# IntelLabs/bayesian-torch

Hardware: AMD Instinct MI355X
Metric: MC-samples/sec (Bayesian-ResNet18, 224^2, bs=64) (higher is better)
Workload: dtype bf16

## Files before the change

### bayesian_torch_amd/_lib.py

```python
import ctypes
import os

_HERE = os.path.dirname(os.path.abspath(__file__))
_LIB = None

KIND_REPARAM, KIND_FLIPOUT = 0, 1
ACT_F32, ACT_BF16 = 0, 1
PREC_F32, PREC_BF16, PREC_BF16X3 = 0, 1, 2
PREC_CODE = {"f32": 0, "bf16": 1, "bf16x3": 2}
FLAG_TRANSPOSED, FLAG_KL_ACCUM, FLAG_ROWFUSE, FLAG_OUT_F32, FLAG_OUT_BF16, FLAG_GATHER, FLAG_SWAP_SIGNS, FLAG_CONCURRENT = 1, 2, 4, 8, 16, 32, 64, 128
FLAG_REVERSE = 256
E_UNSUPPORTED = -3
STREAM_EPS_W, STREAM_EPS_B, STREAM_SIGN_IN, STREAM_SIGN_OUT = 0, 1, 2, 3
ABI_VERSION = 9
FLAG_LANES_SHIFT = 16
FLAG_LANES_MASK = 0xff << FLAG_LANES_SHIFT
SAMPLE_SKIP_MU = 1


class BtxError(RuntimeError):
    pass


class Geom(ctypes.Structure):
    _fields_ = [(n, ctypes.c_int32) for n in (
        "NB", "D", "H", "W", "C", "N", "KD", "KH", "KW", "sd", "sh", "sw", "pd", "ph", "pw",
        "dd", "dh", "dw", "od", "oh", "ow", "groups")]


class Rng(ctypes.Structure):
    _fields_ = [("seed", ctypes.c_uint64), ("sample_idx", ctypes.c_uint32), ("layer_id", ctypes.c_uint32),
                ("sample_idx_dev", ctypes.c_void_p)]


class BnFuse(ctypes.Structure):
    _fields_ = [("residual", ctypes.c_void_p), ("relu", ctypes.c_int32), ("mask", ctypes.c_void_p), ("dres", ctypes.c_void_p)]


class Epilogue(ctypes.Structure):
    _fields_ = [("scale", ctypes.c_void_p), ("shift", ctypes.c_void_p), ("residual", ctypes.c_void_p),
                ("relu", ctypes.c_int32), ("pool", ctypes.c_int32)]


class Lanes(ctypes.Structure):
    _fields_ = [("n", ctypes.c_int32), ("x_stride", ctypes.c_int64), ("out_stride", ctypes.c_int64),
                ("res_stride", ctypes.c_int64)]


class PlanInfo(ctypes.Structure):
    _fields_ = [(n, ctypes.c_int32) for n in ("family", "ksplits", "kper", "kgroups", "wide", "tall", "par_major", "pool_band",
                                              "nwg", "lanes")] + [("ws_bytes", ctypes.c_uint64)]


FAMILIES = ("gather", "regstage", "dma", "gemm8", "patch", "taps", "taps2", "stem", "stem_pool")


class Noise(ctypes.Structure):
    _fields_ = [("eps_w", ctypes.c_void_p), ("eps_b", ctypes.c_void_p),
                ("sign_in", ctypes.c_void_p), ("sign_out", ctypes.c_void_p), ("sampled_w", ctypes.c_void_p)]


class SampleItem(ctypes.Structure):
    _fields_ = [("geom", ctypes.POINTER(Geom)), ("mu_w", ctypes.c_void_p), ("rho_w", ctypes.c_void_p),
                ("out", ctypes.c_void_p), ("kind", ctypes.c_int32), ("layer_id", ctypes.c_uint32),
                ("src_KW", ctypes.c_int32), ("src_C", ctypes.c_int32)]


class LstmLayer(ctypes.Structure):
    _fields_ = [("mu_w", ctypes.c_void_p), ("rho_w", ctypes.c_void_p), ("mu_b", ctypes.c_void_p), ("rho_b", ctypes.c_void_p),
                ("layer_id", ctypes.c_uint32), ("sample_idx", ctypes.c_uint32), ("sample_idx_dev", ctypes.c_void_p)]


class LstmGrads(ctypes.Structure):
    _fields_ = [("dmu_w", ctypes.c_void_p), ("drho_w", ctypes.c_void_p), ("dmu_b", ctypes.c_void_p), ("drho_b", ctypes.c_void_p)]


class KlItem(ctypes.Structure):
    _fields_ = [("mu", ctypes.c_void_p), ("rho", ctypes.c_void_p), ("prior_mu_t", ctypes.c_void_p),
                ("prior_sigma_t", ctypes.c_void_p), ("dmu", ctypes.c_void_p), ("drho", ctypes.c_void_p),
                ("prior_mu", ctypes.c_float), ("prior_sigma", ctypes.c_float), ("n", ctypes.c_size_t)]


class Q8Chain(ctypes.Structure):
    _fields_ = [(n, ctypes.c_float) for n in ("s_sigma", "s_mu", "s_eps", "inv_s_eps", "s_d", "inv_s_d", "inv_s_w")] + \
               [("bias_div", ctypes.c_double)]


class Q8Add(ctypes.Structure):
    _fields_ = [(n, ctypes.c_float) for n in ("s_a", "pre_a", "s_b", "pre_b", "inv_s")] + \
               [("zero_point", ctypes.c_int32), ("relu", ctypes.c_int32)]


class Q8Delta(ctypes.Structure):
    _fields_ = [("inv_s_eps", ctypes.c_float), ("mult", ctypes.c_float), ("mean_bias", ctypes.c_int32), ("pert_bias", ctypes.c_int32),
                ("div_mean", ctypes.c_double), ("div_pert", ctypes.c_double)]


class Q8Flipout(ctypes.Structure):
    _fields_ = [(n, ctypes.c_int32) for n in ("z_x", "z_xp", "z_mean", "z_pert", "z_p2", "sin_pos", "sin_neg", "sout_pos", "sout_neg")] + \
               [(n, ctypes.c_float) for n in ("mult_xp", "mult_mean", "mult_pert", "mult_p2", "out_scale")]


Q8_BIAS_NONE, Q8_BIAS_MU, Q8_BIAS_SIGMA_EPS = 0, 1, 2

EXPORTS = ("btx_abi_version", "btx_strerror", "btx_kl_workspace_bytes", "btx_kl_gauss", "btx_kl_model_workspace_bytes",
           "btx_kl_gauss_model", "btx_kl_gauss_model_bwd", "btx_contract_wgrad",
           "btx_contract_workspace_bytes", "btx_contract_fwd", "btx_contract_fwd_ex", "btx_contract_fwd_lanes", "btx_contract_pool_shape", "btx_contract_plan_info", "btx_out_shape", "btx_fill_eps", "btx_fill_sign", "btx_rho_grad",
           "btx_mc_packed_floats", "btx_mc_accumulate", "btx_mc_accumulate_lanes", "btx_sampled_w_bytes", "btx_sample_weights", "btx_sampled_w_bytes_lanes", "btx_sample_weights_lanes", "btx_rowfuse_pack", "btx_maxpool2d_cl", "btx_avgpool_global_cl",
           "btx_bn_workspace_bytes", "btx_bn_train_fwd", "btx_bn_train_bwd", "btx_dgrad_weights",
           "btx_wgrad_workspace_bytes", "btx_contract_wgrad_ws", "btx_maxpool2d_cl_train", "btx_maxpool2d_cl_bwd",
           "btx_lstm_workspace_bytes", "btx_lstm_fwd", "btx_lstm_train_saved_bytes", "btx_lstm_train_workspace_bytes",
           "btx_lstm_fwd_train", "btx_lstm_bwd",
           "btx_calib_workspace_bytes", "btx_avu_fwd", "btx_avu_bwd", "btx_eau_fwd", "btx_eau_bwd",
           "btx_q8_weight_row_bytes", "btx_q8_quantize_act", "btx_q8_sample_weights", "btx_q8_contract",
           "btx_q8_add", "btx_q8_contract_res", "btx_q8_maxpool2d_cl", "btx_q8_avgpool2d_cl",
           "btx_q8_sample_delta", "btx_q8_contract_flipout")


def lib_path():
    return os.environ.get("BTX_LIB") or os.path.join(_HERE, "libbtx.so")


def lib():
    global _LIB
    if _LIB is not None:
        return _LIB
    path = lib_path()
    if not os.path.exists(path):
        raise BtxError("libbtx.so not found at %s — build it with `python __graft_entry__.py build` "
                       "(hipcc --offload-arch=gfx950); there is no fallback path." % path)
    L = ctypes.CDLL(path)
    vp, sz, u32, i32, f32 = ctypes.c_void_p, ctypes.c_size_t, ctypes.c_uint32, ctypes.c_int, ctypes.c_float
    L.btx_abi_version.restype = i32
    L.btx_abi_version.argtypes = []
    L.btx_strerror.restype = ctypes.c_char_p
    L.btx_strerror.argtypes = [i32]
    L.btx_kl_workspace_bytes.restype = sz
    L.btx_kl_workspace_bytes.argtypes = [sz]
    L.btx_kl_gauss.restype = i32
    L.btx_kl_gauss.argtypes = [vp, vp, sz, vp, vp, f32, f32, vp, u32, vp, sz, vp]
    L.btx_kl_model_workspace_bytes.restype = sz
    L.btx_kl_model_workspace_bytes.argtypes = [i32]
    L.btx_kl_gauss_model.restype = i32
    L.btx_kl_gauss_model.argtypes = [ctypes.POINTER(KlItem), i32, vp, vp, sz, vp]
    L.btx_kl_gauss_model_bwd.restype = i32
    L.btx_kl_gauss_model_bwd.argtypes = [ctypes.POINTER(KlItem), i32, vp, vp]
    L.btx_contract_wgrad.restype = i32
    L.btx_contract_wgrad.argtypes = [i32, ctypes.POINTER(Geom), vp, vp, vp, vp, vp, vp, ctypes.POINTER(Rng),
                                     ctypes.POINTER(Noise), i32, u32, vp]
    L.btx_contract_wgrad_ws.restype = i32
    L.btx_contract_wgrad_ws.argtypes = [i32, ctypes.POINTER(Geom), vp, vp, vp, vp, vp, vp, ctypes.POINTER(Rng),
                                        ctypes.POINTER(Noise), i32, u32, vp, sz, vp, vp, vp]
    L.btx_wgrad_workspace_bytes.restype = sz
    L.btx_wgrad_workspace_bytes.argtypes = [i32, ctypes.POINTER(Geom), i32, u32]
    L.btx_contract_workspace_bytes.restype = sz
    L.btx_contract_workspace_bytes.argtypes = [ctypes.POINTER(Geom), i32, i32, i32, u32]
    L.btx_contract_fwd.restype = i32
    L.btx_contract_fwd.argtypes = [i32, ctypes.POINTER(Geom), vp, vp, vp, vp, vp, vp, ctypes.POINTER(Rng),
                                   ctypes.POINTER(Noise), i32, i32, u32, vp, sz, vp]
    L.btx_contract_fwd_ex.restype = i32
    L.btx_contract_fwd_ex.argtypes = L.btx_contract_fwd.argtypes + [ctypes.POINTER(Epilogue)]
    L.btx_contract_fwd_lanes.restype = i32
    L.btx_contract_fwd_lanes.argtypes = L.btx_contract_fwd_ex.argtypes + [ctypes.POINTER(Lanes)]
    L.btx_contract_plan_info.restype = i32
    L.btx_contract_plan_info.argtypes = [i32, ctypes.POINTER(Geom), i32, i32, u32, ctypes.POINTER(Epilogue), ctypes.POINTER(PlanInfo)]
    L.btx_contract_pool_shape.restype = i32
    L.btx_contract_pool_shape.argtypes = [ctypes.POINTER(Geom), i32, i32, u32] + [ctypes.POINTER(ctypes.c_int32)] * 2
    L.btx_out_shape.restype = i32
    L.btx_out_shape.argtypes = [ctypes.POINTER(Geom), u32] + [ctypes.POINTER(ctypes.c_int32)] * 3
    L.btx_fill_eps.restype = i32
    L.btx_fill_eps.argtypes = [vp, sz, ctypes.POINTER(Rng), u32, vp]
    L.btx_rho_grad.restype = i32
    L.btx_rho_grad.argtypes = [vp, vp, vp, sz, ctypes.POINTER(Rng), u32, vp]
    L.btx_fill_sign.restype = i32
    L.btx_fill_sign.argtypes = [vp, sz, ctypes.POINTER(Rng), u32, vp]
    L.btx_mc_packed_floats.restype = sz
    L.btx_mc_packed_floats.argtypes = [i32, i32]
    L.btx_sampled_w_bytes.restype = sz
    L.btx_sampled_w_bytes.argtypes = [ctypes.POINTER(Geom), i32, i32]
    L.btx_sample_weights.restype = i32
    L.btx_sample_weights.argtypes = [ctypes.POINTER(SampleItem), i32, ctypes.POINTER(Rng), i32, vp]
    L.btx_sampled_w_bytes_lanes.restype = sz
    L.btx_sampled_w_bytes_lanes.argtypes = [ctypes.POINTER(Geom), i32, i32, i32]
    L.btx_sample_weights_lanes.restype = i32
    L.btx_sample_weights_lanes.argtypes = [ctypes.POINTER(SampleItem), i32, ctypes.POINTER(Rng), i32, vp, i32, u32]
    L.btx_rowfuse_pack.restype = i32
    L.btx_rowfuse_pack.argtypes = [vp, i32, ctypes.POINTER(ctypes.c_int64), i32, i32, i32, i32, vp, i32, i32, i32, i32, i32,
                                   i32, vp]
    L.btx_maxpool2d_cl.restype = i32
    L.btx_maxpool2d_cl.argtypes = [vp, vp, i32, i32, i32, i32, i32, i32, i32, i32, vp]
    L.btx_maxpool2d_cl_train.restype = i32
    L.btx_maxpool2d_cl_train.argtypes = [vp, vp, vp, i32, i32, i32, i32, i32, i32, i32, i32, vp]
    L.btx_maxpool2d_cl_bwd.restype = i32
    L.btx_maxpool2d_cl_bwd.argtypes = [vp, vp, vp, i32, i32, i32, i32, i32, i32, i32, i32, vp]
    L.btx_avgpool_global_cl.restype = i32
    L.btx_avgpool_global_cl.argtypes = [vp, vp, i32, i32, i32, i32, vp]
    L.btx_mc_accumulate.restype = i32
    L.btx_mc_accumulate.argtypes = [vp, i32, i32, i32, f32, vp, vp]
# ... 70 lines not shown
```

### bayesian_torch_amd/csrc/btx_api.hip

```cpp
#include <hip/hip_runtime.h>
#include <math.h>
#include <string.h>
#include "../../include/btx.h"
#include <stdlib.h>
#include "btx_contract.h"
#include "btx_rng.h"
#include "btx_presample.h"

using namespace btx;

static int contract_fwd_impl(int kind, const BtxGeom* g, const void* x, const float* mu_w, const float* rho_w,
                             const float* mu_b, const float* rho_b, void* out, const BtxRng* rng, const BtxNoise* noise,
                             int act_dtype, int prec, uint32_t flags, void* ws, size_t ws_bytes, void* stream,
                             const BtxEpilogue* ep, const BtxLanes* ln) {
  if (!g || !x || !mu_w || !rho_w || !out || !rng) return BTX_E_NULL;
  const int lanes = ln ? ln->n : 1;
  if ((mu_b == nullptr) != (rho_b == nullptr)) return BTX_E_NULL;
  const uintptr_t al = (uintptr_t)x | (uintptr_t)mu_w | (uintptr_t)rho_w | (uintptr_t)out |
                       (uintptr_t)(noise && noise->eps_w ? noise->eps_w : nullptr);
  FwdSel sel;
  int rc = select_fwd(kind, g, act_dtype, prec, flags, (al & 15) != 0, noise, ep, &sel);
  if (rc) return rc;
  const Plan& pl = sel.pl;
  const void* sampled_w = (noise && noise->sampled_w) ? noise->sampled_w : nullptr;
  if (sel.need && (!ws || ws_bytes < sel.need)) return BTX_E_WORKSPACE;
  if (sel.need && (((uintptr_t)ws) & 15)) return BTX_E_ALIGN;

  ContractParams p;
  memset(&p, 0, sizeof(p));
  p.x = x; p.mu = mu_w; p.rho = rho_w; p.mu_b = mu_b; p.rho_b = rho_b; p.out = out;
  p.partial = pl.ksplits > 1 ? (float*)ws : nullptr;
  p.lanes = lanes; p.lane_nwg = pl.nwg; p.fd_lane_nwg = make_fastdiv((uint32_t)(pl.nwg > 0 ? pl.nwg : 1));
  if (lanes > 1) {
    p.lane_x = ln->x_stride; p.lane_out = ln->out_stride; p.lane_res = ln->res_stride;
    p.lane_partial = (long long)(plan_ws(pl, g, 1));
  }
  if (noise) {
    p.eps_w = noise->eps_w; p.eps_b = noise->eps_b;
    p.sign_in = noise->sign_in; p.sign_out = noise->sign_out;
  }
  p.NB = g->NB; p.D = g->D; p.H = g->H; p.W = g->W; p.C = g->C; p.Cg = pl.Cg;
  p.Do = pl.Do; p.Ho = pl.Ho; p.Wo = pl.Wo; p.N = g->N; p.Ng = pl.Ng;
  p.KD = g->KD; p.KH = g->KH; p.KW = g->KW;
  p.sd = g->sd; p.sh = g->sh; p.sw = g->sw; p.pd = g->pd; p.ph = g->ph; p.pw = g->pw;
  p.dd = g->dd; p.dh = g->dh; p.dw = g->dw;
  p.M = pl.M; p.K = pl.K;
  p.mtiles = pl.mtiles; p.ntiles = pl.ntiles; p.groups = g->groups; p.ksplits = pl.ksplits; p.kper = pl.kper;
  p.transposed = (flags & BTX_FLAG_TRANSPOSED) ? 1 : 0;
  p.pointwise = (!p.transposed && g->KD == 1 && g->KH == 1 && g->KW == 1 && g->sd == 1 && g->sh == 1 && g->sw == 1 &&
                 g->pd == 0 && g->ph == 0 && g->pw == 0) ? 1 : 0;
  p.out_bf16 = sel.out_bf16;
  if (ep) { p.ep_scale = ep->scale; p.ep_shift = ep->shift; p.ep_res = ep->residual; p.ep_relu = ep->relu; }
  if (flags & BTX_FLAG_ROWFUSE) {
    p.Cg = g->KW * g->C;
    p.KW = 1;
    p.sign_unaligned = 1;
  }
  p.fd_Cg = make_fastdiv((uint32_t)p.Cg); p.fd_KW = make_fastdiv((uint32_t)p.KW); p.fd_KH = make_fastdiv((uint32_t)p.KH);
  p.seed_lo = (uint32_t)rng->seed; p.seed_hi = (uint32_t)(rng->seed >> 32);
  p.sample = rng->sample_idx; p.layer = rng->layer_id;
  p.sample_ptr = rng->sample_idx_dev;
  p.fd_sd = make_fastdiv((uint32_t)g->sd); p.fd_sh = make_fastdiv((uint32_t)g->sh); p.fd_sw = make_fastdiv((uint32_t)g->sw);
  if (sel.par_major) {
    p.par_major = 1; p.par_Hh = pl.Ho / 2; p.par_Wh = pl.Wo / 2; p.par_Mq = g->NB * p.par_Hh * p.par_Wh; p.par_Mqp = sel.par_mqp;
    p.fd_par_Mqp = make_fastdiv((uint32_t)p.par_Mqp); p.fd_par_Hh = make_fastdiv((uint32_t)p.par_Hh);
    p.fd_par_Wh = make_fastdiv((uint32_t)p.par_Wh);
  }
  p.swap_signs = (flags & BTX_FLAG_SWAP_SIGNS) ? 1 : 0;
  p.reverse = (flags & BTX_FLAG_REVERSE) ? 1 : 0;
  sign_keys(rng, p.swap_signs ? BTX_STREAM_SIGN_OUT : BTX_STREAM_SIGN_IN, &p.kin_a, &p.kin_b);
  sign_keys(rng, p.swap_signs ? BTX_STREAM_SIGN_IN : BTX_STREAM_SIGN_OUT, &p.kout_a, &p.kout_b);
  {
    const long long in_elems = (long long)g->NB * g->D * g->H * g->W * g->C;
    const long long xb = in_elems * (act_dtype == BTX_ACT_BF16 ? 2 : 4), wb = (long long)g->N * pl.K * 4;
    p.x_bytes = xb < 0xffffffffLL ? (uint32_t)xb : 0xffffffffu;
    p.w_bytes = wb < 0xffffffffLL ? (uint32_t)wb : 0xffffffffu;
  }

  p.fd_inner = make_fastdiv((uint32_t)(pl.ntiles * g->groups * pl.ksplits)); p.fd_ksplits = make_fastdiv((uint32_t)pl.ksplits);
  p.fd_ntiles = make_fastdiv((uint32_t)pl.ntiles); p.fd_rtiles = make_fastdiv(1u);
  p.fd_mtiles = make_fastdiv((uint32_t)(pl.mtiles > 0 ? pl.mtiles : 1));
  {
    const double w_b = (prec == BTX_PREC_BF16 ? 2.0 : 4.0) * (double)g->N * pl.K * (kind == BTX_KIND_FLIPOUT ? 2 : 1);
    p.wg_order = (uses_tiles(sel.family) && pl.mtiles > 1 && w_b >= WG_MAJOR_MIB * 1048576.0) ? 1 : 0;
  }
  p.fd_Wo = make_fastdiv((uint32_t)pl.Wo); p.fd_Ho = make_fastdiv((uint32_t)pl.Ho); p.fd_Do = make_fastdiv((uint32_t)pl.Do);
  if (uses_tiles(sel.family)) {
    p.wt = sampled_w ? (void*)sampled_w : (void*)((unsigned char*)ws + sel.wt_off);
    p.wt_ready = sampled_w ? 1 : 0;
    p.wt_bytes = (uint32_t)sel.wt_all;
    p.wt_delta_off = (uint32_t)sel.wt_one;
    p.lane_wt = (long long)sel.wt_one;
    p.lane_wt_delta = (kind == BTX_KIND_FLIPOUT) ? 1 : 0;
  }
  hipStream_t st = (hipStream_t)stream;
  typedef int (*LaunchFn)(int, const ContractParams&, int, hipStream_t);
  auto launch = [&](LaunchFn f32, LaunchFn bf16, LaunchFn x3) {
    return (prec == BTX_PREC_BF16 ? bf16 : prec == BTX_PREC_BF16X3 ? x3 : f32)(kind, p, pl.nwg * lanes, st);
  };
  switch (sel.family) {
    case BTX_FAMILY_STEM_POOL: {
      const StemPoolPlan& spp = sel.spp;
// ... 79 lines not shown
    case BTX_E_UNSUPPORTED: return "btx: unsupported configuration";
    case BTX_E_WORKSPACE: return "btx: workspace too small";
    case BTX_E_DTYPE: return "btx: unknown dtype / precision code";
    case BTX_E_ALIGN: return "btx: pointer not 16-byte aligned";
    default: return code > 0 ? hipGetErrorString((hipError_t)code) : "btx: unknown error";
  }
}

int btx_contract_fwd(int kind, const BtxGeom* g, const void* x, const float* mu_w, const float* rho_w,
                     const float* mu_b, const float* rho_b, void* out, const BtxRng* rng, const BtxNoise* noise,
                     int act_dtype, int prec, uint32_t flags, void* ws, size_t ws_bytes, void* stream) {
  return btx_contract_fwd_ex(kind, g, x, mu_w, rho_w, mu_b, rho_b, out, rng, noise, act_dtype, prec, flags, ws,
                             ws_bytes, stream, nullptr);
}

int btx_contract_fwd_ex(int kind, const BtxGeom* g, const void* x, const float* mu_w, const float* rho_w,
                        const float* mu_b, const float* rho_b, void* out, const BtxRng* rng, const BtxNoise* noise,
                        int act_dtype, int prec, uint32_t flags, void* ws, size_t ws_bytes, void* stream,
                        const BtxEpilogue* ep) {
  return contract_fwd_impl(kind, g, x, mu_w, rho_w, mu_b, rho_b, out, rng, noise, act_dtype, prec,
                           flags & ~BTX_FLAG_LANES_MASK, ws, ws_bytes, stream, ep, nullptr);
}

int btx_contract_fwd_lanes(int kind, const BtxGeom* g, const void* x, const float* mu_w, const float* rho_w,
                           const float* mu_b, const float* rho_b, void* out, const BtxRng* rng, const BtxNoise* noise,
                           int act_dtype, int prec, uint32_t flags, void* ws, size_t ws_bytes, void* stream,
                           const BtxEpilogue* ep, const BtxLanes* lanes) {
  if (!lanes) return BTX_E_NULL;
  if (lanes->n < 1 || lanes->n > 255) return BTX_E_SHAPE;
  if ((lanes->x_stride | lanes->out_stride | lanes->res_stride) & 15) return BTX_E_ALIGN;
  if (noise && lanes->n > 1 && (noise->eps_w || noise->eps_b || noise->sign_in || noise->sign_out)) return BTX_E_UNSUPPORTED;
  return contract_fwd_impl(kind, g, x, mu_w, rho_w, mu_b, rho_b, out, rng, noise, act_dtype, prec,
                           (flags & ~BTX_FLAG_LANES_MASK) | BTX_FLAG_LANES(lanes->n), ws, ws_bytes, stream, ep, lanes);
}

int btx_sample_weights(const BtxSampleItem* items, int n_items, const BtxRng* rng, int prec, void* stream) {
  return btx_sample_weights_lanes(items, n_items, rng, prec, stream, 1, 0);
}

int btx_sample_weights_lanes(const BtxSampleItem* items, int n_items, const BtxRng* rng, int prec, void* stream, int lanes,
                             uint32_t sflags) {
  if (!items || !rng) return BTX_E_NULL;
  if (lanes < 1 || lanes > 255) return BTX_E_SHAPE;
  const uint64_t seed = rng->seed;
  const uint32_t sample_idx = rng->sample_idx;
  if (n_items <= 0) return n_items == 0 ? 0 : BTX_E_SHAPE;
  if (prec != BTX_PREC_F32 && prec != BTX_PREC_BF16 && prec != BTX_PREC_BF16X3) return BTX_E_DTYPE;
  for (int base = 0; base < n_items; base += PRESAMPLE_MAX_ITEMS) {
    PresampleBatch b;
    memset(&b, 0, sizeof(b));
    b.n = n_items - base < PRESAMPLE_MAX_ITEMS ? n_items - base : PRESAMPLE_MAX_ITEMS;
    b.seed_lo = (uint32_t)seed; b.seed_hi = (uint32_t)(seed >> 32); b.sample = sample_idx; b.sample_ptr = rng->sample_idx_dev;
    b.lanes = lanes; b.skip_mu = (sflags & BTX_SAMPLE_SKIP_MU) ? 1 : 0;
    uint32_t blocks = 0;
    for (int i = 0; i < b.n; ++i) {
      const BtxSampleItem& s = items[base + i];
      if (!s.geom || !s.mu_w || !s.rho_w || !s.out) return BTX_E_NULL;
      if (s.kind != BTX_KIND_REPARAM && s.kind != BTX_KIND_FLIPOUT) return BTX_E_UNSUPPORTED;
      const bool remap = s.src_C != 0 || s.src_KW != 0;
      if ((((uintptr_t)s.out) & 15) || (!remap && (((uintptr_t)s.mu_w | (uintptr_t)s.rho_w) & 15))) return BTX_E_ALIGN;
      Plan pl;
      int rc = make_plan(s.geom, prec, 0, DBM, &pl);
      if (rc) return rc;
      if (pl.K % (prec == BTX_PREC_BF16 ? 8 : 4)) return BTX_E_UNSUPPORTED;
      size_t one = 0;
      if (patch_wt_bytes(pl, s.geom, s.kind, prec, &one, lanes) >= 0xfff00000ULL) return BTX_E_UNSUPPORTED;
// ... 29 lines not shown
```

### bayesian_torch_amd/csrc/btx_contract.h

```cpp
#pragma once
#include <hip/hip_runtime.h>
#include <stdint.h>
#include "btx_rng.h"
#include "btx_plan.h"

typedef __attribute__((ext_vector_type(8))) __bf16 bf16x8;
typedef __attribute__((ext_vector_type(4))) __bf16 bf16x4;
typedef __attribute__((ext_vector_type(4))) float f32x4;
typedef __attribute__((ext_vector_type(8))) float f32x8;
typedef __attribute__((ext_vector_type(16))) float f32x16;
typedef __attribute__((ext_vector_type(4))) uint32_t u32x4;
typedef __attribute__((ext_vector_type(2))) uint32_t u32x2;

namespace btx {

constexpr int NTHREADS = 512;
constexpr int ACTS_OFF = 0;
constexpr int SIGN_OFF = NG * BM * 16;
constexpr int WMU_OFF = SIGN_OFF + NG * BM * 4;
constexpr int WDL_OFF = WMU_OFF + NG * BN * 16;
constexpr int STAGE_BYTES = WDL_OFF + NG * BN * 16;
constexpr int LDS_BYTES = 2 * STAGE_BYTES;

struct FastDiv {
// ... 48 lines not shown
  const float* ep_scale;
  const float* ep_shift;
  const void* ep_res;
  int ep_relu;
  int out_bf16;
  int sign_unaligned;
  uint32_t x_bytes, w_bytes;
  int pt_G, pt_R, pt_Rp, pt_Wp, pt_PP, pt_NI, pt_rtiles;
  FastDiv fd_Wo, fd_Ho, fd_Do, fd_ptWp, fd_ptRp, fd_ptR;
  FastDiv fd_inner, fd_ksplits, fd_ntiles, fd_Cg, fd_KW, fd_KH, fd_rtiles;
  FastDiv fd_mtiles;
  int swap_signs;
  int par_major, par_Mq, par_Mqp, par_Hh, par_Wh;
  FastDiv fd_par_Mqp, fd_par_Hh, fd_par_Wh;
  FastDiv fd_sd, fd_sh, fd_sw;
  int wg_order;
  int pt_nw, pt_astage, pt_lds;
  int pt_kg;
  int pt_lds_g;
  int pt_taps;
  int pt_wide;
  int sp_Hq, sp_Wq;
  int st_sbytes;
  void* wt;
  uint32_t wt_bytes, wt_delta_off;
  int wt_ready;
  int pt_tall, pt_P, pt_Wt, pt_ncs;
  FastDiv fd_P, fd_Wt, fd_ncs;
  int lanes, lane_nwg;
  FastDiv fd_lane_nwg;
  long long lane_x, lane_out, lane_res, lane_wt, lane_partial;
  int lane_wt_delta;
  int reverse;
};

__device__ __forceinline__ uint32_t sample_word_scalar(const uint32_t* ptr) {
  return *(const __attribute__((address_space(4))) uint32_t*)(uintptr_t)ptr;
}

__device__ __forceinline__ int xcd_logical() {
  const int nwg = gridDim.x, L = blockIdx.x;
  const int q = nwg >> 3, r = nwg & 7, xcd = L & 7, slot = L >> 3;
  return (xcd < r ? xcd * (q + 1) : r * (q + 1) + (xcd - r) * q) + slot;
}

__device__ __forceinline__ ContractParams lane_view(const ContractParams& q, int& logical) {
  ContractParams p = q;
  if (q.reverse) logical = (int)gridDim.x - 1 - logical;
  if (q.lanes > 1) {
    uint32_t lane, loc;
    fdivmod((uint32_t)logical, q.fd_lane_nwg, (uint32_t)q.lane_nwg, lane, loc);
    logical = (int)loc;
    const long long l = (long long)lane;
    p.x = (const unsigned char*)q.x + l * q.lane_x;
    p.out = (unsigned char*)q.out + l * q.lane_out;
    if (q.ep_res) p.ep_res = (const unsigned char*)q.ep_res + l * q.lane_res;
    if (q.wt) {
      if (q.lane_wt_delta) p.wt_delta_off = q.wt_delta_off + (uint32_t)(l * q.lane_wt);
      else p.wt = (unsigned char*)q.wt + l * q.lane_wt;
    }
    if (q.partial) p.partial = (float*)((unsigned char*)q.partial + l * q.lane_partial);
    if (q.sample_ptr) p.sample_ptr = q.sample_ptr + lane;
    p.sample = q.sample + lane;
  }
  return p;
}
// ... 601 lines not shown
      for (int r = 0; r < nv; ++r)
        for (int s = 0; s < ksplits; ++s) a[r] += partial[(long long)s * total + i + r];
    }
    for (int r = 0; r < nv; ++r) {
      const int col = (int)((i + r) % N);
      float v = a[r];
      v = __builtin_fmaf(v, scale ? scale[col] : 1.f, shift ? shift[col] : 0.f);
      if (res) v += (float)res[i + r];
      if (relu) v = v > 0.f ? v : 0.f;
      if (relu == 2) v = v < 6.f ? v : 6.f;
      a[r] = v;
    }
    if (nv == 4) {
      if constexpr (sizeof(ACT) == 4) *(f32x4*)(out + i) = (f32x4){a[0], a[1], a[2], a[3]};
      else *(bf16x4*)(out + i) = __builtin_convertvector((f32x4){a[0], a[1], a[2], a[3]}, bf16x4);
    } else {
      for (int r = 0; r < nv; ++r) out[i + r] = (ACT)a[r];
    }
  }
}

int launch_contract_f32(int kind, int act_bf16, bool gen, const ContractParams& p, int nwg, hipStream_t st);
int launch_contract_bf16(int kind, int act_bf16, bool gen, const ContractParams& p, int nwg, hipStream_t st);
int launch_contract_dma_f32(int kind, const ContractParams& p, int nwg, hipStream_t st);
int launch_contract_dma_bf16(int kind, const ContractParams& p, int nwg, hipStream_t st);
int launch_contract_patch_f32(int kind, const ContractParams& p, int nwg, hipStream_t st);
int launch_contract_stem_f32(int kind, const ContractParams& p, int nwg, hipStream_t st);
int launch_contract_stem_bf16(int kind, const ContractParams& p, int nwg, hipStream_t st);
int launch_stem_pool_bf16(int kind, const ContractParams& p, int nwg, hipStream_t st);
struct PresampleBatch;
int launch_presample_batch_f32(const PresampleBatch& b, hipStream_t st);
int launch_presample_batch_bf16(const PresampleBatch& b, hipStream_t st);
int launch_contract_patch_bf16(int kind, const ContractParams& p, int nwg, hipStream_t st);
int launch_contract_patch_x3(int kind, const ContractParams& p, int nwg, hipStream_t st);
int launch_contract_stem_x3(int kind, const ContractParams& p, int nwg, hipStream_t st);
int launch_contract_dma_x3(int kind, const ContractParams& p, int nwg, hipStream_t st);
int launch_contract_gemm8_bf16(int kind, const ContractParams& p, int nwg, hipStream_t st);
int launch_contract_gemm8_f32(int kind, const ContractParams& p, int nwg, hipStream_t st);
int launch_contract_gemm8_x3(int kind, const ContractParams& p, int nwg, hipStream_t st);
int launch_presample_batch_x3(const PresampleBatch& b, hipStream_t st);

template <int PREC>
static int launch_contract_impl(int kind, int act_bf16, bool gen, const ContractParams& p, int nwg, hipStream_t st) {
#define BTX_LAUNCH(ACT, KIND, GENF)                                                                              \
  do {                                                                                                            \
    auto kfn = contract_kernel<PREC, ACT, KIND, GENF>;                                                            \
    static bool attr_done = false;                                                                                \
    if (!attr_done) {                                                                                             \
      hipError_t e = hipFuncSetAttribute((const void*)kfn, hipFuncAttributeMaxDynamicSharedMemorySize, LDS_BYTES); \
      if (e != hipSuccess) return (int)e;                                                                         \
      attr_done = true;                                                                                           \
    }                                                                                                             \
    hipLaunchKernelGGL(kfn, dim3(nwg), dim3(NTHREADS), LDS_BYTES, st, p);                                         \
  } while (0)
  if (!act_bf16) {
    if (kind == 0) { if (gen) BTX_LAUNCH(float, 0, true); else BTX_LAUNCH(float, 0, false); }
    else           { if (gen) BTX_LAUNCH(float, 1, true); else BTX_LAUNCH(float, 1, false); }
  } else {
    if (kind == 0) { if (gen) BTX_LAUNCH(__bf16, 0, true); else BTX_LAUNCH(__bf16, 0, false); }
    else           { if (gen) BTX_LAUNCH(__bf16, 1, true); else BTX_LAUNCH(__bf16, 1, false); }
  }
#undef BTX_LAUNCH
  return (int)hipGetLastError();
}

}
// ... 1 lines not shown
```

### bayesian_torch_amd/csrc/btx_contract_patch.h

```cpp
#pragma once
#include <type_traits>
#include "btx_contract.h"
#include "btx_contract_dma.h"
#include "btx_epilogue.h"
#include "btx_presample.h"
#include "btx_mma.h"
#include "btx_contract_taps.h"
#include "btx_contract_taps2.h"

namespace btx {



template <int PREC, int KIND, int NW, int MI>
__global__ __launch_bounds__(64 * NW, (MI == 4) ? 1 : 2) void contract_patch_kernel(const ContractParams) {
  BTX_SECTION_PARAMS(p, logical);
  const RngLive rl = rng_live<KIND>(p);
  constexpr int NT = 64 * NW;
  constexpr int WPX = 32 * MI;
  constexpr int MAXNI = (MI == 4) ? 16 : PT_MAXNI;
  constexpr int SJ = (MI == 4) ? 4 : 2;
  using ACT = typename std::conditional<PREC == 1, __bf16, float>::type;
  constexpr int G = (PREC == 1) ? 8 : 4;
  constexpr int BK = NG * G;
// ... 196 lines not shown
    BTX_SECTION_PARAMS(pe, logical2);
    const int nimg = min(pe.pt_G, pe.NB - img0), nrow = min(pe.pt_R, pe.Ho - row0);
    const int nvalid = nimg * nrow * pe.Wo;
    const uint32_t m0 = (uint32_t)(img0 * pe.Ho + row0) * (uint32_t)pe.Wo;
    if constexpr (MI == 2) {
      staged_epilogue<KIND, NW>(pe, rl, accm, accd, smem, tid, wave, lane, ntile, group, split, m0, nvalid);
    } else {
#pragma unroll
      for (int hf = 0; hf < MI / 2; ++hf) {
        __builtin_amdgcn_sched_barrier(0);
        staged_epilogue<KIND, NW>(pe, rl, reinterpret_cast<const f32x16(&)[2][2]>(accm[2 * hf]),
                                  reinterpret_cast<const f32x16(&)[2][2]>(accd[2 * hf]), smem, tid, wave, lane, ntile,
                                  group, split, m0, nvalid, wave * (MI / 2) + hf, hf == 0);
      }
    }
  }
}

template <int PREC>
static int launch_contract_patch_impl(int kind, const ContractParams& p, int nwg, hipStream_t st) {
#define BTX_LAUNCH_PT(KIND, NW, MI)                                                                                 \
  do {                                                                                                            \
    auto kfn = contract_patch_kernel<PREC, KIND, NW, MI>;                                                           \
    static bool attr_done = false;                                                                                \
    if (!attr_done) {                                                                                             \
      hipError_t e = hipFuncSetAttribute((const void*)kfn, hipFuncAttributeMaxDynamicSharedMemorySize, 163840);   \
      if (e != hipSuccess) return (int)e;                                                                         \
      attr_done = true;                                                                                           \
    }                                                                                                             \
    hipLaunchKernelGGL(kfn, dim3(nwg), dim3(64 * NW), p.pt_lds, st, p);                                           \
  } while (0)
  int rc = launch_presample_impl<PREC>(kind, p, st);
  if (rc) return rc;
  if (p.pt_taps == 332) {
#define BTX_LAUNCH_T2(KIND, ...)                                                                                  \
  do {                                                                                                            \
    auto kfn = contract_taps2_kernel<PREC, KIND, ##__VA_ARGS__>;                                                  \
    static bool attr_done = false;                                                                                \
    if (!attr_done) {                                                                                             \
      hipError_t e = hipFuncSetAttribute((const void*)kfn, hipFuncAttributeMaxDynamicSharedMemorySize, 163840);   \
      if (e != hipSuccess) return (int)e;                                                                         \
      attr_done = true;                                                                                           \
    }                                                                                                             \
    hipLaunchKernelGGL(kfn, dim3(nwg), dim3(256), p.pt_lds, st, p);                                               \
  } while (0)
    if constexpr (PREC == 1) {
      if (p.pt_wide && kind == 0) {
        BTX_LAUNCH_T2(0, true);
        return (int)hipGetLastError();
      }
    }
    if (kind == 0) BTX_LAUNCH_T2(0); else BTX_LAUNCH_T2(1);
#undef BTX_LAUNCH_T2
    return (int)hipGetLastError();
  }
  if (p.pt_taps == 33) {
#define BTX_LAUNCH_TP(KIND, KG, ...)                                                                               \
  do {                                                                                                            \
    auto kfn = contract_taps_kernel<PREC, KIND, 3, 3, KG, ##__VA_ARGS__>;                                           \
    static bool attr_done = false;                                                                                \
    if (!attr_done) {                                                                                             \
      hipError_t e = hipFuncSetAttribute((const void*)kfn, hipFuncAttributeMaxDynamicSharedMemorySize, 163840);   \
      if (e != hipSuccess) return (int)e;                                                                         \
      attr_done = true;                                                                                           \
    }                                                                                                             \
    hipLaunchKernelGGL(kfn, dim3(nwg), dim3(256 * KG), p.pt_lds, st, p);                                          \
// ... 22 lines not shown
```

### bayesian_torch_amd/csrc/btx_contract_taps.h

```cpp
#pragma once
#include <type_traits>
#include "btx_contract.h"
#include "btx_contract_dma.h"
#include "btx_epilogue.h"
#include "btx_mma.h"

namespace btx {

__device__ __forceinline__ void dma16s(__amdgpu_buffer_rsrc_t rsrc, uint32_t voff, uint32_t soff,
                                       unsigned char* lds_wave_base) {
  __builtin_amdgcn_raw_ptr_buffer_load_lds(rsrc, (__attribute__((address_space(3))) void*)lds_wave_base, 16, voff, soff,
                                           0, 0);
}

template <int N>
__device__ __forceinline__ void end_stage() {
  asm volatile("s_waitcnt vmcnt(%0)\n\ts_waitcnt lgkmcnt(0)\n\ts_barrier" ::"n"(N) : "memory");
}

template <int I, int N, class F>
__device__ __forceinline__ void static_for(F&& f) {
  if constexpr (I < N) {
    f(std::integral_constant<int, I>{});
    static_for<I + 1, N>(f);
  }
}

constexpr int TP_MAXNI = 6;

template <int T>
constexpr int tp_pieces(int t) {
  constexpr int PST = T - 3;
  constexpr int PPS = (TP_MAXNI + PST - 1) / PST;
  if (t < 0) t += T;
  if (t >= PST) return 0;
  int n = 0;
  for (int i = 0; i < PPS; ++i)
    if (t + PST * i < TP_MAXNI) ++n;
  return n;
}

template <int PREC, int KIND, int KH, int KW, int KG, bool WIDE = false>
__global__ __launch_bounds__(256 * KG, 2) void contract_taps_kernel(const ContractParams) {
  static_assert(!WIDE || (PREC == 1 && KG == 1 && KIND == 0), "wide tile: bf16 Reparameterization, one K-group");
  constexpr int K2 = (KIND == 1 || WIDE) ? 1 : 0;
  BTX_SECTION_PARAMS(p, logical);
  constexpr int NW = 4, NT = 256, MI = 2, T = KH * KW;
  static_assert(T >= 5 && T <= 32, "tap-unrolled kernel: 5..32 taps");
  constexpr int MAXNI = TP_MAXNI;
  constexpr int PST = T - 3;
  constexpr int WOPS = K2 ? 2 : 1;
  using ACT = typename std::conditional<PREC == 1, __bf16, float>::type;
  constexpr int G = (PREC == 1) ? 8 : 4;
  constexpr int BK = NG * G;
  constexpr int ESZ = (int)sizeof(ACT);
  extern __shared__ __attribute__((aligned(16))) unsigned char smem_all[];

  uint32_t smp = p.sample;
  if (p.sample_ptr) smp = sample_word_scalar(p.sample_ptr);

  const int tid = threadIdx.x & 255;
  const int lane = tid & 63;
  const int l31 = lane & 31;
  const int h = lane >> 5;
  const int wave_all = __builtin_amdgcn_readfirstlane((int)(threadIdx.x >> 6));
  const int wave = wave_all & 3;
  const int kg = (KG == 1) ? 0 : (wave_all >> 2);
  unsigned char* const smem = smem_all + kg * p.pt_lds_g;

  uint32_t u_mtile, u_rem, u_split, u_ntile, u_group, u_t;
  const uint32_t ntg = (uint32_t)(WIDE ? p.ntiles >> 1 : p.ntiles);
  if (p.wg_order) fdivmod((uint32_t)logical, p.fd_mtiles, (uint32_t)p.mtiles, u_rem, u_mtile);
  else fdivmod((uint32_t)logical, p.fd_inner, ntg * (uint32_t)(p.groups * p.ksplits), u_mtile, u_rem);
  fdivmod(u_rem, p.fd_ksplits, (uint32_t)p.ksplits, u_t, u_split);
  fdivmod(u_t, p.fd_ntiles, ntg, u_group, u_ntile);
  const int mtile = (int)u_mtile, split = (int)u_split, ntile = (int)u_ntile, group = (int)u_group;

  const bool tall = p.pt_tall != 0;
  uint32_t u_ig, u_rt;
  if (tall) fdivmod((uint32_t)mtile, p.fd_ncs, (uint32_t)p.pt_ncs, u_rt, u_ig);
  else fdivmod((uint32_t)mtile, p.fd_rtiles, (uint32_t)p.pt_rtiles, u_ig, u_rt);
  const int img0 = tall ? 0 : (int)u_ig * p.pt_G, row0 = (int)u_rt * p.pt_R, col0 = tall ? (int)u_ig * p.pt_Wt : 0;
  auto patch_src = [&](int q, bool& ok) __attribute__((always_inline)) -> uint32_t {
    uint32_t ut, upc, ugi, upr;
    fdivmod((uint32_t)q, p.fd_ptWp, (uint32_t)p.pt_Wp, ut, upc);
    int img, ih, iw;
    if (tall) {
      fdivmod((uint32_t)row0 + ut, p.fd_P, (uint32_t)p.pt_P, ugi, upr);
      img = (int)ugi; ih = (int)upr - p.ph; iw = col0 + (int)upc - p.pw;
      ok = (int)ut < p.pt_Rp;
    } else {
      fdivmod(ut, p.fd_ptRp, (uint32_t)p.pt_Rp, ugi, upr);
      img = img0 + (int)ugi; ih = row0 + (int)upr - p.ph; iw = (int)upc - p.pw;
      ok = true;
    }
    ok = ok && img < p.NB && (unsigned)ih < (unsigned)p.H && (unsigned)iw < (unsigned)p.W;
    return (uint32_t)((img * p.H + ih) * p.W + iw);
  };
  const int ncb_total = p.Cg / BK;
  const int cb_per = p.kper / BK;
  const int cb0 = split * cb_per + kg * (cb_per / KG);
  const int ncb = (KG == 1) ? min(ncb_total, cb0 + cb_per) - cb0 : cb_per / KG;
  const int a_stage = p.pt_astage, s_stage = p.pt_astage >> 4;
  const int PT_A_OFF = 0, PT_S_OFF = 2 * a_stage, PT_W_OFF = 2 * a_stage + 2 * s_stage;
  const int PT_X_OFF = PT_W_OFF + PT_WD * DW_STAGE;

  const __amdgpu_buffer_rsrc_t x_rsrc = __builtin_amdgcn_make_buffer_rsrc((void*)p.x, 0, p.x_bytes, 0x00020000);
  const __amdgpu_buffer_rsrc_t wt_rsrc = __builtin_amdgcn_make_buffer_rsrc((void*)p.wt, 0, p.wt_bytes, 0x00020000);

  const uint32_t w_voff = (uint32_t)lane * 16u + (uint32_t)wave * 1024u;
  const uint32_t w_sbase = (uint32_t)(group * p.ntiles + (WIDE ? 2 * ntile : ntile)) * (uint32_t)(p.K / G) * 1024u;
  const uint32_t w_second = WIDE ? (uint32_t)(p.K / G) * 1024u : p.wt_delta_off;
  const uint32_t CgG = (uint32_t)(p.Cg / G);
  const int w_lds = PT_W_OFF + wave * 1024;
  int wslot = 0;
  auto issue_w = [&](uint32_t tap, uint32_t cb, int slot) __attribute__((always_inline)) {
    const uint32_t soff = w_sbase + (tap * CgG + cb * (uint32_t)NG) * 1024u;
    unsigned char* ld = smem + w_lds + slot * DW_STAGE;
    dma16s(wt_rsrc, w_voff, soff, ld);
    if constexpr (K2) dma16s(wt_rsrc, w_voff, soff + w_second, ld + 4096);
  };
  if (ncb > 0) issue_w(0u, (uint32_t)cb0, 0);

  uint32_t sg_off[2];
  bool sg_ok[2];
  uint32_t* const pix_tab = (uint32_t*)(smem + PT_S_OFF + s_stage);
#pragma unroll
  for (int j = 0; j < 2; ++j) {
    const int q = tid + NT * j;
    sg_ok[j] = q < p.pt_PP;
    bool inside;
    const uint32_t ipix = patch_src(sg_ok[j] ? q : 0, inside);
    sg_off[j] = ipix * (uint32_t)p.C + (uint32_t)(group * p.Cg);
    if (q * 4 < s_stage) pix_tab[q] = (sg_ok[j] && inside) ? sg_off[j] : 0xffffffffu;
    if (p.sign_in)
      sg_ok[j] = sg_ok[j] && inside;
  }
  asm volatile("s_waitcnt lgkmcnt(0)\n\ts_barrier" ::: "memory");

  const int g_lane = (lane & 3) ^ ((lane >> 4) & 3);
  uint32_t pp_boff[MAXNI];
  uint32_t pmask = 0;
  uint32_t pp_e[MAXNI];
#pragma unroll
  for (int j = 0; j < MAXNI; ++j) {
    const int q = 16 * (wave + NW * j) + (lane >> 2);
    pp_e[j] = pix_tab[q < p.pt_PP ? q : 0];
  }
#pragma unroll
  for (int j = 0; j < MAXNI; ++j) {
    const int q = 16 * (wave + NW * j) + (lane >> 2);
    uint32_t bo = DMA_OOB;
    if (j < p.pt_NI && q < p.pt_PP) {
      const uint32_t e = pp_e[j];
      if (e != 0xffffffffu) bo = (e + (uint32_t)(G * g_lane)) * (uint32_t)ESZ;
    }
    pp_boff[j] = bo;
    if (j < p.pt_NI && 16 * (wave + NW * j) < p.pt_PP) {
      pmask |= 1u << j;
      if (ncb > 0)
        dma16(x_rsrc, bo == DMA_OOB ? DMA_OOB : bo + (uint32_t)(cb0 * BK * ESZ), smem + PT_A_OFF + (wave + NW * j) * 1024);
    }
  }
  pmask = __builtin_amdgcn_readfirstlane(pmask);
  if (ncb > 0) {
    issue_w(1u, (uint32_t)cb0, 1);
    issue_w(2u, (uint32_t)cb0, 2);
  }

  RngLive rl = {smp, p.kin_a, p.kin_b, p.kout_a, p.kout_b};
  if (p.sample_ptr || p.lanes > 1) {
    rl.sample = __builtin_amdgcn_readfirstlane(smp);
    if constexpr (KIND == 1) {
      const uint32_t si = p.swap_signs ? 3u : 2u, so = p.swap_signs ? 2u : 3u;
      const BtxPhilox4 ki = btx_philox4x32_10(0u, rl.sample, p.layer, si, p.seed_lo, p.seed_hi);
      const BtxPhilox4 ko = btx_philox4x32_10(0u, rl.sample, p.layer, so, p.seed_lo, p.seed_hi);
      rl.kin_a = __builtin_amdgcn_readfirstlane(ki.x[0]); rl.kin_b = __builtin_amdgcn_readfirstlane(ki.x[1]);
      rl.kout_a = __builtin_amdgcn_readfirstlane(ko.x[0]); rl.kout_b = __builtin_amdgcn_readfirstlane(ko.x[1]);
    }
  }

  auto write_signs = [&](int slot, int cb) __attribute__((always_inline)) {
    if constexpr (KIND == 1) {
      unsigned char* ss = smem + PT_S_OFF + slot * s_stage;
#pragma unroll
      for (int j = 0; j < 2; ++j) {
        if (sg_ok[j]) {
          const uint32_t off = sg_off[j] + (uint32_t)(cb * BK);
          uint32_t w;
          if (p.sign_in) w = sign_word_explicit(p.sign_in, off, p.x_bytes / (uint32_t)ESZ);
          else w = btx_sign_word(off >> 5, rl.kin_a, rl.kin_b);
          if constexpr (G == 4) w <<= 8 * ((off >> 4) & 1);
          *(uint32_t*)(ss + (tid + NT * j) * 4) = w;
        }
      }
    }
  };

  int q0[MI];
#pragma unroll
  for (int mi = 0; mi < MI; ++mi) {
    const int pl = wave * 64 + mi * 32 + l31;
    uint32_t ut, uc, ugi, ur;
    if (tall) {
      fdivmod((uint32_t)pl, p.fd_Wt, (uint32_t)p.pt_Wt, ur, uc);
      q0[mi] = ((int)ur < p.pt_R) ? (int)ur * p.pt_Wp + (int)uc : 0;
    } else {
      fdivmod((uint32_t)pl, p.fd_Wo, (uint32_t)p.Wo, ut, uc);
      fdivmod(ut, p.fd_ptR, (uint32_t)p.pt_R, ugi, ur);
      const int c = (int)uc, r = (int)ur, gi = (int)ugi;
      const bool ok = (gi < p.pt_G) && (img0 + gi < p.NB) && (row0 + r < p.Ho);
      q0[mi] = ok ? (gi * p.pt_Rp + r) * p.pt_Wp + c : 0;
    }
  }
  const int row_step = p.dh * p.pt_Wp;

  constexpr bool ZI = (PREC == 1 && KG == 1);
  f32x16 accm[MI][2], accd[MI][2];
  auto clear_acc = [&](int a0) __attribute__((always_inline)) {
#pragma unroll
    for (int a = 0; a < MI; ++a)
#pragma unroll
      for (int b = 0; b < 2; ++b)
#pragma unroll
        for (int r = 0; r < 16; ++r)
          if (a >= a0) { accm[a][b][r] = 0.f; accd[a][b][r] = 0.f; }
  };
  if (!ZI || ncb <= 0) clear_acc(0);

  using Frag = StageFragT<MI>;
  auto load_frag = [&](Frag& f, int aslot, int toffv, int wsl, auto mia_tag) __attribute__((always_inline)) {
    constexpr int MIA = decltype(mia_tag)::value;
    const unsigned char* as = smem + PT_A_OFF + aslot * a_stage;
    const unsigned char* ss = smem + PT_S_OFF + aslot * s_stage;
    const unsigned char* ws = smem + PT_W_OFF + wsl * DW_STAGE;
    int q[MI];
#pragma unroll
    for (int mi = 0; mi < MI; ++mi) q[mi] = q0[mi] + toffv;
#pragma unroll
    for (int kk = 0; kk < NG / 2; ++kk) {
      const int row = 2 * kk + h;
#pragma unroll
      for (int mi = 0; mi < MIA; ++mi) f.a[kk][mi] = *(const u32x4*)(as + q[mi] * 64 + ((row ^ ((q[mi] >> 2) & 3)) * 16));
#pragma unroll
      for (int ni = 0; ni < 2; ++ni) f.wm[kk][ni] = *(const u32x4*)(ws + (row * BN + ni * 32 + l31) * 16);
    }
    if constexpr (KIND == 1) {
#pragma unroll
      for (int mi = 0; mi < MIA; ++mi) f.sw[mi] = *(const uint32_t*)(ss + q[mi] * 4);
    }
  };

  if (ncb > 0) {
    write_signs(0, cb0);
    asm volatile("s_waitcnt vmcnt(%0)\n\ts_waitcnt lgkmcnt(0)\n\ts_barrier" ::"n"(KG == 1 ? WOPS : 2 * WOPS) : "memory");
    Frag fa, fb;
    const int nvalid_px = tall ? p.pt_R * p.pt_Wt : min(p.pt_G, p.NB - img0) * min(p.pt_R, p.Ho - row0) * p.Wo;
    const bool mi1_dead = wave * 64 + 32 >= nvalid_px;
    auto kloop = [&](auto mia_tag) __attribute__((always_inline)) {
    constexpr int MIA = decltype(mia_tag)::value;
    if constexpr (KG == 1) load_frag(fa, 0, 0, 0, mia_tag);
    auto block = [&](auto par_tag, auto first_tag, int cbi, bool last) __attribute__((always_inline)) {
      constexpr int PAR = decltype(par_tag)::value;
      constexpr bool FIRST = decltype(first_tag)::value;
      static_for<0, T>([&](auto t_tag) __attribute__((always_inline)) {
        constexpr int t = decltype(t_tag)::value;
        constexpr int sp = (PAR * T + t) & 1;
        Frag& cur = (KG == 1 && sp) ? fb : fa;
        Frag& nxt = (KG == 1 && sp) ? fa : fb;
        asm volatile("" : "+v"(q0[0]), "+v"(q0[1]));
        constexpr int t3 = (t + 3) % T, c3 = (t + 3) / T;
        if constexpr (c3 == 0) {
          issue_w((uint32_t)t3, (uint32_t)(cb0 + cbi), (wslot + 3) & 3);
        } else {
          if (!last) issue_w((uint32_t)t3, (uint32_t)(cb0 + cbi + 1), (wslot + 3) & 3);
        }
        constexpr int KP = tp_pieces<T>(t);
        if constexpr (t < PST) {
          if (!last) {
            const uint32_t cboff = (uint32_t)((cb0 + cbi + 1) * BK * ESZ);
#pragma unroll
            for (int i = 0; i < KP; ++i) {
              const int j = t + PST * i;
              const uint32_t bo = pp_boff[j];
              unsigned char* dst = ((pmask >> j) & 1u) ? smem + PT_A_OFF + (PAR ^ 1) * a_stage + (wave + NW * j) * 1024
                                                        : smem + PT_X_OFF;
              dma16(x_rsrc, bo == DMA_OOB ? DMA_OOB : bo + cboff, dst);
            }
            if constexpr (t == 0) write_signs(PAR ^ 1, cb0 + cbi + 1);
          }
        }
        DeltaFrag df;
        if constexpr (KG == 1) {
          load_delta<K2>(df, smem + PT_W_OFF + wslot * DW_STAGE, l31, h);
          constexpr int t1 = (t + 1) % T, c1 = (t + 1) / T;
          load_frag(nxt, PAR ^ c1, (t1 / KW) * row_step + (t1 % KW) * p.dw, (wslot + 1) & 3, mia_tag);
          if constexpr (FIRST && t == 0) stage_mma<PREC, K2, MI, MIA, true, KIND == 1>(cur, df, accm, accd, l31, h);
          else stage_mma<PREC, K2, MI, MIA, false, KIND == 1>(cur, df, accm, accd, l31, h);
          if (!last) end_stage<WOPS + KP>();
          else end_stage<(c3 == 0) ? WOPS : 0>();
        } else {
          load_delta<KIND>(df, smem + PT_W_OFF + wslot * DW_STAGE, l31, h);
          load_frag(cur, PAR, (t / KW) * row_step + (t % KW) * p.dw, wslot, mia_tag);
          __builtin_amdgcn_sched_barrier(0);
          asm volatile("s_barrier" ::: "memory");
          __builtin_amdgcn_sched_barrier(0);
          stage_mma<PREC, KIND, MI, MIA>(cur, df, accm, accd, l31, h);
          __builtin_amdgcn_sched_barrier(0);
          if (!last) {
            end_stage<2 * WOPS + KP + tp_pieces<T>(t - 1) + tp_pieces<T>(t - 2)>();
          } else {
            constexpr int a_ = (t + 3 < T) ? 1 : 0, b_ = (t == 0) ? 1 : ((t + 2 < T) ? 1 : 0);
            end_stage<WOPS * (a_ + b_)>();
          }
        }
        wslot = (wslot + 1) & 3;
      });
    };
    if (KG == 2 && kg == 1) asm volatile("s_barrier" ::: "memory");
    using P0 = std::integral_constant<int, 0>;
    using P1 = std::integral_constant<int, 1>;
    if constexpr (ZI) {
      if constexpr (MIA < MI) clear_acc(MIA);
      block(P0{}, std::true_type{}, 0, ncb == 1);
      int cbi = 1;
      for (; cbi + 2 <= ncb; cbi += 2) {
        block(P1{}, std::false_type{}, cbi, false);
        block(P0{}, std::false_type{}, cbi + 1, cbi + 2 == ncb);
      }
      if (cbi < ncb) block(P1{}, std::false_type{}, cbi, true);
    } else {
      int cbi = 0;
      for (; cbi + 2 <= ncb; cbi += 2) {
        block(P0{}, std::false_type{}, cbi, false);
        block(P1{}, std::false_type{}, cbi + 1, cbi + 2 == ncb);
      }
      if (cbi < ncb) block(P0{}, std::false_type{}, cbi, true);
    }
    if (KG == 2 && kg == 0) asm volatile("s_barrier" ::: "memory");
    };
    if (mi1_dead) kloop(std::integral_constant<int, 1>{});
    else kloop(std::integral_constant<int, 2>{});
  }

  {
    BTX_SECTION_PARAMS(pe, logical2);
    const int nimg = min(pe.pt_G, pe.NB - img0), nrow = min(pe.pt_R, pe.Ho - row0);
    const int nvalid = nimg * nrow * pe.Wo;
    const uint32_t m0 = (uint32_t)(img0 * pe.Ho + row0) * (uint32_t)pe.Wo;
    const PixTall pmt = {pe, row0, col0};
    if constexpr (KG == 1) {
      if constexpr (WIDE) {
        float* const ba0 = (float*)(smem + NW * PT_EP_WAVE);
        float* const ba1 = ba0 + 4 * BN;
        {
          const bool has_bias = (split == 0) && (pe.mu_b != nullptr);
          const bool has_aff = (pe.ksplits == 1) && ((pe.ep_scale != nullptr) || (pe.ep_shift != nullptr));
          if (has_bias || has_aff) {
            if (tid < 64) ep_fill_constants<0>(pe, rl, ba0, tid, 2 * ntile, group, has_bias, has_aff);
            else if (tid < 128) ep_fill_constants<0>(pe, rl, ba1, tid - 64, 2 * ntile + 1, group, has_bias, has_aff);
          }
          __syncthreads();
        }
        if (tall) {
          staged_epilogue_pm<0, NW, PixTall>(pe, rl, accm, accm, smem, tid, wave, lane, 2 * ntile, group, split, pmt, -1, true, ba0);
          staged_epilogue_pm<0, NW, PixTall>(pe, rl, accd, accd, smem, tid, wave, lane, 2 * ntile + 1, group, split, pmt, -1, true, ba1);
        } else {
          staged_epilogue<0, NW>(pe, rl, accm, accm, smem, tid, wave, lane, 2 * ntile, group, split, m0, nvalid, -1, true, ba0);
          staged_epilogue<0, NW>(pe, rl, accd, accd, smem, tid, wave, lane, 2 * ntile + 1, group, split, m0, nvalid, -1, true, ba1);
        }
      } else
      if (tall) staged_epilogue_pm<KIND, NW, PixTall>(pe, rl, accm, accd, smem, tid, wave, lane, ntile, group, split, pmt);
      else staged_epilogue<KIND, NW>(pe, rl, accm, accd, smem, tid, wave, lane, ntile, group, split, m0, nvalid);
    } else {
      float* ba_lds = (float*)(smem_all + 131072);
      const bool to_partial = pe.ksplits > 1;
      const bool has_bias = (split == 0) && (pe.mu_b != nullptr);
      const bool has_aff = !to_partial && ((pe.ep_scale != nullptr) || (pe.ep_shift != nullptr));
      if (kg == 1) {
#pragma unroll
        for (int mi = 0; mi < MI; ++mi)
#pragma unroll
          for (int ni = 0; ni < 2; ++ni)
// ... 44 lines not shown
```

### bayesian_torch_amd/csrc/btx_contract_taps2.h

```cpp
#pragma once
#include <type_traits>
#include "btx_contract.h"
#include "btx_contract_dma.h"
#include "btx_contract_taps.h"
#include "btx_epilogue.h"
#include "btx_mma.h"

namespace btx {

constexpr int T2_MAXNI = 5;
constexpr int T2_WD = 3;
constexpr int T2_T = 9;

constexpr int t2_seq(int s) { return s < 4 ? 0 : (s == 4 ? 1 : (s < 7 ? 2 : 3)); }
constexpr int t2_tap(int s) {
  return s == 0 ? 0 : s == 1 ? 2 : s == 2 ? 6 : s == 3 ? 8 : s == 4 ? 4 : s == 5 ? 1 : s == 6 ? 7 : s == 7 ? 3 : 5;
}
constexpr int t2_a(int k) { return (k == 0 || k == 2) ? 1 : 0; }
constexpr int t2_b(int k) { return (k == 0 || k == 3) ? 1 : 0; }
constexpr int t2_np(int s) { return (s == 0 || s == 5 || s == 7) ? 3 : ((s == 1 || s == 6 || s == 8) ? 2 : (s == 4 ? 5 : 0)); }
constexpr int t2_p0(int s) { return (s == 1 || s == 6 || s == 8) ? 3 : 0; }
constexpr int t2_fseq(int s) { return s < 2 ? 2 : (s == 4 ? 3 : (s < 7 ? 4 : 5)); }

template <int PREC, int KIND, bool WIDE = false>
__global__ __launch_bounds__(256, 2) void contract_taps2_kernel(const ContractParams) {
  static_assert(!WIDE || (PREC == 1 && KIND == 0), "wide tile: bf16 Reparameterization");
  BTX_SECTION_PARAMS(p, logical);
  constexpr int NW = 4, NT = 256, MI = 2, T = T2_T, MAXNI = T2_MAXNI, WD = T2_WD;
  constexpr int K2 = (KIND == 1 || WIDE) ? 1 : 0;
  constexpr int WOPS = K2 ? 2 : 1;
  using ACT = typename std::conditional<PREC == 1, __bf16, float>::type;
  constexpr int G = (PREC == 1) ? 8 : 4;
  constexpr int BK = NG * G;
  constexpr int ESZ = (int)sizeof(ACT);
  extern __shared__ __attribute__((aligned(16))) unsigned char smem[];

  uint32_t smp = p.sample;
  if (p.sample_ptr) smp = sample_word_scalar(p.sample_ptr);

  const int tid = threadIdx.x;
  const int lane = tid & 63;
  const int l31 = lane & 31;
  const int h = lane >> 5;
  const int wave = __builtin_amdgcn_readfirstlane(tid >> 6);

  uint32_t u_mtile, u_rem, u_split, u_ntile, u_group, u_t;
  const uint32_t ntg = (uint32_t)(WIDE ? p.ntiles >> 1 : p.ntiles);
  if (p.wg_order) fdivmod((uint32_t)logical, p.fd_mtiles, (uint32_t)p.mtiles, u_rem, u_mtile);
  else fdivmod((uint32_t)logical, p.fd_inner, ntg * (uint32_t)(p.groups * p.ksplits), u_mtile, u_rem);
  fdivmod(u_rem, p.fd_ksplits, (uint32_t)p.ksplits, u_t, u_split);
  fdivmod(u_t, p.fd_ntiles, ntg, u_group, u_ntile);
  const int mtile = (int)u_mtile, split = (int)u_split, ntile = (int)u_ntile, group = (int)u_group;

  uint32_t u_ig, u_rt;
  fdivmod((uint32_t)mtile, p.fd_rtiles, (uint32_t)p.pt_rtiles, u_ig, u_rt);
  const int img0 = (int)u_ig * p.pt_G, row0 = (int)u_rt * p.pt_R;
  const int ncb_total = p.Cg / BK;
  const int cb_per = p.kper / BK;
  const int cb0 = split * cb_per;
  const int ncb = min(ncb_total, cb0 + cb_per) - cb0;
  const int a_stage = p.pt_astage, s_stage = p.pt_astage >> 4;
  const int PT_A_OFF = 0, PT_S_OFF = 3 * a_stage, PT_W_OFF = 3 * a_stage + 3 * s_stage;
  const int PT_X_OFF = PT_W_OFF + WD * DW_STAGE;

  const __amdgpu_buffer_rsrc_t x_rsrc = __builtin_amdgcn_make_buffer_rsrc((void*)p.x, 0, p.x_bytes, 0x00020000);
  const __amdgpu_buffer_rsrc_t wt_rsrc = __builtin_amdgcn_make_buffer_rsrc((void*)p.wt, 0, p.wt_bytes, 0x00020000);

  const uint32_t w_voff = (uint32_t)lane * 16u + (uint32_t)wave * 1024u;
  const uint32_t w_sbase = (uint32_t)(group * p.ntiles + (WIDE ? 2 * ntile : ntile)) * (uint32_t)(p.K / G) * 1024u;
  const uint32_t w_second = WIDE ? (uint32_t)(p.K / G) * 1024u : p.wt_delta_off;
  const uint32_t CgG = (uint32_t)(p.Cg / G);
  const int w_lds = PT_W_OFF + wave * 1024;
  int wslot = 0;
  auto issue_w = [&](uint32_t tap, uint32_t cb, int slot) __attribute__((always_inline)) {
    const uint32_t soff = w_sbase + (tap * CgG + cb * (uint32_t)NG) * 1024u;
    unsigned char* ld = smem + w_lds + slot * DW_STAGE;
    dma16s(wt_rsrc, w_voff, soff, ld);
    if constexpr (K2) dma16s(wt_rsrc, w_voff, soff + w_second, ld + 4096);
  };
  if (ncb > 0) issue_w((uint32_t)t2_tap(0), (uint32_t)cb0, 0);

  const int g_lane = (lane & 3) ^ ((lane >> 4) & 3);
  uint32_t pp_base[MAXNI];
  uint32_t pvalid = 0, pmask = 0;
#pragma unroll
  for (int j = 0; j < MAXNI; ++j) {
    const int q = 16 * (wave + NW * j) + (lane >> 2);
    uint32_t bo = 0;
    if (j < p.pt_NI && q < p.pt_PP) {
      uint32_t ut, ujj, ugi, ui;
      fdivmod((uint32_t)q, p.fd_ptWp, (uint32_t)p.pt_Wp, ut, ujj);
      fdivmod(ut, p.fd_ptRp, (uint32_t)p.pt_Rp, ugi, ui);
      const int img = img0 + (int)ugi, ih0 = 2 * (row0 + (int)ui), iw0 = 2 * (int)ujj;
      bo = ((uint32_t)((img * p.H + ih0) * p.W + iw0) * (uint32_t)p.C + (uint32_t)(group * p.Cg + G * g_lane)) * (uint32_t)ESZ;
// ... 24 lines not shown
  };

  RngLive rl = {smp, p.kin_a, p.kin_b, p.kout_a, p.kout_b};
  if (p.sample_ptr || p.lanes > 1) {
    rl.sample = __builtin_amdgcn_readfirstlane(smp);
    if constexpr (KIND == 1) {
      const uint32_t si = p.swap_signs ? 3u : 2u, so = p.swap_signs ? 2u : 3u;
      const BtxPhilox4 ki = btx_philox4x32_10(0u, rl.sample, p.layer, si, p.seed_lo, p.seed_hi);
      const BtxPhilox4 ko = btx_philox4x32_10(0u, rl.sample, p.layer, so, p.seed_lo, p.seed_hi);
      rl.kin_a = __builtin_amdgcn_readfirstlane(ki.x[0]); rl.kin_b = __builtin_amdgcn_readfirstlane(ki.x[1]);
      rl.kout_a = __builtin_amdgcn_readfirstlane(ko.x[0]); rl.kout_b = __builtin_amdgcn_readfirstlane(ko.x[1]);
    }
  }
  uint32_t sg_base[2];
  uint32_t sg_v = 0;
#pragma unroll
  for (int j = 0; j < 2; ++j) {
    const int q = tid + NT * j;
    const int qq = q < p.pt_PP ? q : 0;
    uint32_t ut, ujj, ugi, ui;
    fdivmod((uint32_t)qq, p.fd_ptWp, (uint32_t)p.pt_Wp, ut, ujj);
    fdivmod(ut, p.fd_ptRp, (uint32_t)p.pt_Rp, ugi, ui);
    const int img = img0 + (int)ugi, ih0 = 2 * (row0 + (int)ui), iw0 = 2 * (int)ujj;
    sg_base[j] = (uint32_t)((img * p.H + ih0) * p.W + iw0) * (uint32_t)p.C + (uint32_t)(group * p.Cg);
    if (q < p.pt_PP && img < p.NB) {
#pragma unroll
      for (int a = 0; a < 2; ++a)
#pragma unroll
        for (int b = 0; b < 2; ++b)
          if ((unsigned)(ih0 - a) < (unsigned)p.H && (unsigned)(iw0 - b) < (unsigned)p.W) sg_v |= 1u << (4 * j + 2 * a + b);
    }
  }
  auto write_signs = [&](int a, int b, int cb, int sslot_off) __attribute__((always_inline)) {
    if constexpr (KIND == 1) {
      unsigned char* ss = smem + PT_S_OFF + sslot_off;
#pragma unroll
      for (int j = 0; j < 2; ++j) {
        if ((sg_v >> (4 * j + 2 * a + b)) & 1u) {
          const uint32_t off = sg_base[j] - (uint32_t)((a * p.W + b) * p.C) + (uint32_t)(cb * BK);
          uint32_t w;
          if (p.sign_in) w = sign_word_explicit(p.sign_in, off, p.x_bytes / (uint32_t)ESZ);
          else w = btx_sign_word(off >> 5, rl.kin_a, rl.kin_b);
          if constexpr (G == 4) w <<= 8 * ((off >> 4) & 1);
          *(uint32_t*)(ss + (tid + NT * j) * 4) = w;
        }
      }
    }
  };

  int q0[MI];
#pragma unroll
  for (int mi = 0; mi < MI; ++mi) {
    const int pl = wave * 64 + mi * 32 + l31;
    uint32_t ut, uc, ugi, ur;
    fdivmod((uint32_t)pl, p.fd_Wo, (uint32_t)p.Wo, ut, uc);
    fdivmod(ut, p.fd_ptR, (uint32_t)p.pt_R, ugi, ur);
    const int c = (int)uc, r = (int)ur, gi = (int)ugi;
    const bool ok = (gi < p.pt_G) && (img0 + gi < p.NB) && (row0 + r < p.Ho);
    q0[mi] = ok ? (gi * p.pt_Rp + r) * p.pt_Wp + c : 0;
  }
  const int Wp = p.pt_Wp;

  f32x16 accm[MI][2], accd[MI][2];
#pragma unroll
  for (int a = 0; a < MI; ++a)
#pragma unroll
    for (int b = 0; b < 2; ++b)
#pragma unroll
      for (int r = 0; r < 16; ++r) { accm[a][b][r] = 0.f; accd[a][b][r] = 0.f; }

  using Frag = StageFragT<MI>;
  auto load_frag = [&](Frag& f, int aoff, int soff, int toffv, int wsl, auto mia_tag) __attribute__((always_inline)) {
    constexpr int MIA = decltype(mia_tag)::value;
    const unsigned char* as = smem + PT_A_OFF + aoff;
    const unsigned char* ss = smem + PT_S_OFF + soff;
    const unsigned char* ws = smem + PT_W_OFF + wsl * DW_STAGE;
    int q[MI];
#pragma unroll
    for (int mi = 0; mi < MI; ++mi) q[mi] = q0[mi] + toffv;
#pragma unroll
    for (int kk = 0; kk < NG / 2; ++kk) {
      const int row = 2 * kk + h;
#pragma unroll
      for (int mi = 0; mi < MIA; ++mi) f.a[kk][mi] = *(const u32x4*)(as + q[mi] * 64 + ((row ^ ((q[mi] >> 2) & 3)) * 16));
#pragma unroll
      for (int ni = 0; ni < 2; ++ni) f.wm[kk][ni] = *(const u32x4*)(ws + (row * BN + ni * 32 + l31) * 16);
    }
    if constexpr (KIND == 1) {
#pragma unroll
      for (int mi = 0; mi < MIA; ++mi) f.sw[mi] = *(const uint32_t*)(ss + q[mi] * 4);
    }
  };

  if (ncb > 0) {
    int sl0 = 0, sl1 = 1, sl2 = 2;
    issue_plane(0, MAXNI, 1, 1, cb0, sl0 * a_stage);
    issue_w((uint32_t)t2_tap(1), (uint32_t)cb0, 1);
    issue_plane(0, MAXNI, 0, 0, cb0, sl1 * a_stage);
    write_signs(1, 1, cb0, sl0 * s_stage);
    write_signs(0, 0, cb0, sl1 * s_stage);
    asm volatile("s_waitcnt vmcnt(%0)\n\ts_waitcnt lgkmcnt(0)\n\ts_barrier" ::"n"(MAXNI + WOPS) : "memory");
    Frag fa;
    const int nvalid_px = min(p.pt_G, p.NB - img0) * min(p.pt_R, p.Ho - row0) * p.Wo;
    const bool mi1_dead = wave * 64 + 32 >= nvalid_px;
    auto kloop = [&](auto mia_tag) __attribute__((always_inline)) {
      constexpr int MIA = decltype(mia_tag)::value;
      auto block = [&](int cbi, bool last) __attribute__((always_inline)) {
        static_for<0, T>([&](auto t_tag) __attribute__((always_inline)) {
          constexpr int s = decltype(t_tag)::value;
          asm volatile("" : "+v"(q0[0]), "+v"(q0[1]), "+v"(pvalid), "+v"(sg_v), "+v"(sg_base[0]), "+v"(sg_base[1]));
          asm volatile("" : "+v"(pp_base[0]), "+v"(pp_base[1]), "+v"(pp_base[2]), "+v"(pp_base[3]), "+v"(pp_base[4]));
          auto slot_of = [&](int k) __attribute__((always_inline)) { return (k % 3) == 0 ? sl0 : ((k % 3) == 1 ? sl1 : sl2); };
          constexpr int s2 = (s + 2) % T, c2 = (s + 2) / T;
          if constexpr (c2 == 0) issue_w((uint32_t)t2_tap(s2), (uint32_t)(cb0 + cbi), (wslot + 2) % WD);
          else { if (!last) issue_w((uint32_t)t2_tap(s2), (uint32_t)(cb0 + cbi + 1), (wslot + 2) % WD); }
          constexpr int NP = t2_np(s);
          if constexpr (NP > 0) {
            constexpr int FS = t2_fseq(s), FK = FS % 4, FC = FS / 4;
            if (FC == 0 || !last) {
              const int so = slot_of(FS);
              issue_plane(t2_p0(s), NP, t2_a(FK), t2_b(FK), cb0 + cbi + FC, so * a_stage);
              if constexpr (t2_p0(s) == 0) write_signs(t2_a(FK), t2_b(FK), cb0 + cbi + FC, so * s_stage);
            }
          }
          DeltaFrag df;
          load_delta<K2>(df, smem + PT_W_OFF + wslot * DW_STAGE, l31, h);
          {
            constexpr int TP = t2_tap(s);
            const int so = slot_of(t2_seq(s));
            load_frag(fa, so * a_stage, so * s_stage, ((TP / 3) == 2 ? Wp : 0) + ((TP % 3) == 2 ? 1 : 0), wslot, mia_tag);
          }
          stage_mma<PREC, K2, MI, MIA, false, KIND == 1>(fa, df, accm, accd, l31, h);
          if (!last) end_stage<WOPS + NP>();
          else end_stage<((s + 2 < T) ? WOPS : 0) + ((t2_fseq(s) < 4) ? NP : 0)>();
          wslot = (wslot + 1) % WD;
        });
        const int t0 = sl0; sl0 = sl1; sl1 = sl2; sl2 = t0;
      };
      for (int cbi = 0; cbi + 1 < ncb; ++cbi) block(cbi, false);
      block(ncb - 1, true);
    };
    if (mi1_dead) kloop(std::integral_constant<int, 1>{});
    else kloop(std::integral_constant<int, 2>{});
  }

  {
    BTX_SECTION_PARAMS(pe, logical2);
    const int nimg = min(pe.pt_G, pe.NB - img0), nrow = min(pe.pt_R, pe.Ho - row0);
    const int nvalid = nimg * nrow * pe.Wo;
    const uint32_t m0 = (uint32_t)(img0 * pe.Ho + row0) * (uint32_t)pe.Wo;
    if constexpr (WIDE) {
      float* const ba0 = (float*)(smem + NW * PT_EP_WAVE);
      float* const ba1 = ba0 + 4 * BN;
      const bool has_bias = (split == 0) && (pe.mu_b != nullptr);
      const bool has_aff = (pe.ksplits == 1) && ((pe.ep_scale != nullptr) || (pe.ep_shift != nullptr));
      if (has_bias || has_aff) {
        if (tid < 64) ep_fill_constants<0>(pe, rl, ba0, tid, 2 * ntile, group, has_bias, has_aff);
        else if (tid < 128) ep_fill_constants<0>(pe, rl, ba1, tid - 64, 2 * ntile + 1, group, has_bias, has_aff);
      }
      __syncthreads();
      staged_epilogue<0, NW>(pe, rl, accm, accm, smem, tid, wave, lane, 2 * ntile, group, split, m0, nvalid, -1, true, ba0);
      staged_epilogue<0, NW>(pe, rl, accd, accd, smem, tid, wave, lane, 2 * ntile + 1, group, split, m0, nvalid, -1, true, ba1);
    } else
    staged_epilogue<KIND, NW>(pe, rl, accm, accd, smem, tid, wave, lane, ntile, group, split, m0, nvalid);
  }
}

}
```

### bayesian_torch_amd/csrc/btx_epilogue.h

```cpp
#pragma once
#include <type_traits>
#include "btx_contract.h"

namespace btx {

template <int I, int N, class F>
__device__ __forceinline__ void static_for_ep(F&& f) {
  if constexpr (I < N) {
    f(std::integral_constant<int, I>{});
    static_for_ep<I + 1, N>(f);
  }
}

struct EpRaw {
  float mu, rho, eps, sc, sh;
};
__device__ __forceinline__ EpRaw ep_load_constants(const ContractParams& p, int t, int ntile, int group, bool has_bias,
                                                   bool has_aff) {
  EpRaw r = {0.f, 0.f, 0.f, 1.f, 0.f};
  if (t < BN) {
    const int col = ntile * BN + t;
    const int gcol = group * p.Ng + (col < p.Ng ? col : 0);
    if (has_bias && col < p.Ng) {
      r.mu = p.mu_b[gcol];
// ... 75 lines not shown
    fdivmod((uint32_t)pl, p.fd_Wt, (uint32_t)p.pt_Wt, r, c);
    fdivmod((uint32_t)row0 + r, p.fd_P, (uint32_t)p.pt_P, img, oh);
    const int ow = col0 + (int)c;
    ok = (int)r < p.pt_R && (int)oh < p.Ho && (int)img < p.NB && ow < p.Wo;
    return ok ? ((img * (uint32_t)p.Ho + oh) * (uint32_t)p.Wo + (uint32_t)ow) : 0u;
  }
  __device__ __forceinline__ uint32_t first() const { return 0u; }
  struct Walk {
    const ContractParams& p;
    int r, c, oh, img, col0;
    __device__ __forceinline__ uint32_t get(bool& ok) const {
      const int ow = col0 + c;
      ok = r < p.pt_R && oh < p.Ho && img < p.NB && ow < p.Wo;
      return ok ? (uint32_t)((img * p.Ho + oh) * p.Wo + ow) : 0u;
    }
    __device__ __forceinline__ void step8() {
      c += 8;
#pragma unroll
      for (int i = 0; i < 2; ++i)
        if (c >= p.pt_Wt) { c -= p.pt_Wt; ++r; if (++oh >= p.pt_P) { oh -= p.pt_P; ++img; } }
    }
  };
  __device__ __forceinline__ Walk walk(int pl) const {
    uint32_t r, c, img, oh;
    fdivmod((uint32_t)pl, p.fd_Wt, (uint32_t)p.pt_Wt, r, c);
    fdivmod((uint32_t)row0 + r, p.fd_P, (uint32_t)p.pt_P, img, oh);
    return Walk{p, (int)r, (int)c, (int)oh, (int)img, col0};
  }
};

struct EpNoHook {
  __device__ __forceinline__ void operator()() const {}
};
template <int KIND, int NW, class PM = PixContig, bool RES_PRE = false, class HOOK = EpNoHook>
__device__ __forceinline__ void staged_epilogue_pm(const ContractParams& p, const RngLive& rl, const f32x16 (&accm)[2][2],
                                                   const f32x16 (&accd)[2][2], unsigned char* smem, int tid, int wave,
                                                   int lane, int ntile, int group, int split, const PM& pm,
                                                   int pwave = -1, bool first = true,
                                                   float* ba_ext = nullptr, const HOOK& hook = HOOK{},
                                                   const uint32_t* wsh_ext = nullptr) {
  if (pwave < 0) pwave = wave;
  constexpr int EP_ROW = PT_EP_ROW;
  constexpr int EP_WAVE = PT_EP_WAVE;
  const int l31 = lane & 31, h = lane >> 5;
  const bool to_partial = p.ksplits > 1;
  const bool has_bias = (split == 0) && (p.mu_b != nullptr);
  const bool has_aff = !to_partial && ((p.ep_scale != nullptr) || (p.ep_shift != nullptr));
  const bool has_ba = has_bias || has_aff;
  float* ba_lds = ba_ext ? ba_ext : (float*)(smem + NW * EP_WAVE);
  if (has_ba && first && !ba_ext) {
    ep_fill_constants<KIND>(p, rl, ba_lds, tid, ntile, group, has_bias, has_aff);
    __syncthreads();
  }
  unsigned char* ep = smem + wave * EP_WAVE;

  constexpr bool BUFIO = RES_PRE && std::is_same<PM, PixContig>::value;
  u32x4 rpre[8];
  auto io_off = [&](int lane_) __attribute__((always_inline)) -> uint32_t {
    return ((pm.first() + (uint32_t)(pwave * 64 + (lane_ >> 3))) * (uint32_t)p.N + (uint32_t)(group * p.Ng + ntile * BN + (lane_ & 7) * 8)) * 2u;
  };
  const uint32_t io_step = 8u * (uint32_t)p.N * 2u, io_bytes = (uint32_t)p.M * (uint32_t)p.N * 2u;
  if constexpr (RES_PRE) {
    const bool all_vec = ((p.N & 7) == 0) && (((group * p.Ng) & 7) == 0) && (ntile * BN + BN <= p.Ng);
    if (all_vec && !to_partial && p.ep_res != nullptr && p.out_bf16 && p.ep_relu != 2) {
      if constexpr (BUFIO) {
        const __amdgpu_buffer_rsrc_t res_rsrc = __builtin_amdgcn_make_buffer_rsrc((void*)p.ep_res, 0, io_bytes, 0x00020000);
        const uint32_t io_voff = io_off(lane);
#pragma unroll
        for (int i = 0; i < 8; ++i) rpre[i] = __builtin_amdgcn_raw_buffer_load_b128(res_rsrc, io_voff, io_step * (uint32_t)i, 0);
      } else {
        const uint32_t cbase = (uint32_t)(group * p.Ng + ntile * BN + (lane & 7) * 8);
        auto wk = pm.walk(pwave * 64 + (lane >> 3));
#pragma unroll
// ... 127 lines not shown
    const bool all_vec = ((p.N & 7) == 0) && (((group * p.Ng) & 7) == 0) && (ntile * BN + BN <= p.Ng) && p.ep_relu != 2;
    const bool res = !to_partial && p.ep_res != nullptr, relu = !to_partial && p.ep_relu;
    const bool relu6 = relu && p.ep_relu == 2;
    auto fast = [&](auto outk_tag, auto res_tag, auto relu_tag) __attribute__((always_inline)) {
      constexpr int OUTK = decltype(outk_tag)::value;
      constexpr bool RES = decltype(res_tag)::value, RELU = decltype(relu_tag)::value;
      auto wk = pm.walk(pwave * 64 + (lane >> 3));
      int lane_s2 = lane;
      asm volatile("" : "+v"(lane_s2));
      const uint32_t io_voff = BUFIO ? io_off(lane_s2) : 0u;
      constexpr int NP = RES_PRE ? 8 : 4;
#pragma unroll
      for (int hf = 0; hf < 8 / NP; ++hf) {
        uint32_t idx[NP];
        bool pk[NP];
        u32x4 r0[NP], r1[NP];
#pragma unroll
        for (int i = 0; i < NP; ++i) {
          if constexpr (BUFIO && OUTK == 1) {
            pk[i] = true; idx[i] = 0;
            if constexpr (RES) r0[i] = rpre[hf * NP + i];
            continue;
          }
          const uint32_t gp = wk.get(pk[i]);
          wk.step8();
          idx[i] = gp * (uint32_t)p.N + cbase;
          if constexpr (RES) {
            const uint32_t li = pk[i] ? idx[i] : cbase + pm.first() * (uint32_t)p.N;
            if constexpr (OUTK == 1 && RES_PRE) r0[i] = rpre[hf * NP + i];
            else if constexpr (OUTK == 1) r0[i] = *(const u32x4*)((const __bf16*)p.ep_res + li);
            else { r0[i] = *(const u32x4*)((const float*)p.ep_res + li); r1[i] = *(const u32x4*)((const float*)p.ep_res + li + 4); }
          }
        }
        f32x4 lo[NP], hi[NP];
#pragma unroll
        for (int i = 0; i < NP; ++i) {
          const int pix = (hf * NP + i) * 8 + (lane >> 3);
          lo[i] = *(const f32x4*)(ep + pix * EP_ROW + cg * 32);
          hi[i] = *(const f32x4*)(ep + pix * EP_ROW + cg * 32 + 16);
        }
#pragma unroll
        for (int i = 0; i < NP; ++i) {
          float v[8] = {lo[i][0], lo[i][1], lo[i][2], lo[i][3], hi[i][0], hi[i][1], hi[i][2], hi[i][3]};
          if constexpr (RES) {
            if constexpr (OUTK == 1) {
#pragma unroll
              for (int j = 0; j < 4; ++j) { v[2 * j] += u2f(r0[i][j] << 16); v[2 * j + 1] += u2f(r0[i][j] & 0xffff0000u); }
            } else {
#pragma unroll
              for (int j = 0; j < 4; ++j) { v[j] += u2f(r0[i][j]); v[4 + j] += u2f(r1[i][j]); }
            }
          }
          if constexpr (RELU) {
#pragma unroll
            for (int j = 0; j < 8; ++j) v[j] = fmaxf(v[j], 0.f);
          }
          if constexpr (OUTK == 1 && !BUFIO) {
            const f32x4 x0 = {v[0], v[1], v[2], v[3]}, x1 = {v[4], v[5], v[6], v[7]};
            const u32x2 p0 = __builtin_bit_cast(u32x2, __builtin_convertvector(x0, bf16x4));
            const u32x2 p1 = __builtin_bit_cast(u32x2, __builtin_convertvector(x1, bf16x4));
            const __amdgpu_buffer_rsrc_t out_rsrc = __builtin_amdgcn_make_buffer_rsrc((void*)p.out, 0, io_bytes, 0x00020000);
            __builtin_amdgcn_raw_buffer_store_b128((u32x4){p0[0], p0[1], p1[0], p1[1]}, out_rsrc, pk[i] ? idx[i] * 2u : 0xfffffff0u, 0, 0);
          } else
          if (pk[i]) {
            if constexpr (OUTK == 0) {
              float* dst = p.partial + (size_t)split * p.M * p.N + idx[i];
              *(f32x4*)dst = (f32x4){v[0], v[1], v[2], v[3]};
              *(f32x4*)(dst + 4) = (f32x4){v[4], v[5], v[6], v[7]};
            } else if constexpr (OUTK == 1) {
              const f32x4 x0 = {v[0], v[1], v[2], v[3]}, x1 = {v[4], v[5], v[6], v[7]};
              const u32x2 p0 = __builtin_bit_cast(u32x2, __builtin_convertvector(x0, bf16x4));
              const u32x2 p1 = __builtin_bit_cast(u32x2, __builtin_convertvector(x1, bf16x4));
              if constexpr (BUFIO) {
                const __amdgpu_buffer_rsrc_t out_rsrc = __builtin_amdgcn_make_buffer_rsrc((void*)p.out, 0, io_bytes, 0x00020000);
                __builtin_amdgcn_raw_buffer_store_b128((u32x4){p0[0], p0[1], p1[0], p1[1]}, out_rsrc, io_voff,
                                                       io_step * (uint32_t)(hf * NP + i), 0);
              } else {
                *(u32x4*)((__bf16*)p.out + idx[i]) = (u32x4){p0[0], p0[1], p1[0], p1[1]};
              }
            } else {
              float* dst = (float*)p.out + idx[i];
              *(f32x4*)dst = (f32x4){v[0], v[1], v[2], v[3]};
              *(f32x4*)(dst + 4) = (f32x4){v[4], v[5], v[6], v[7]};
            }
          }
        }
      }
    };
    using T = std::true_type;
    using F = std::false_type;
    if (all_vec) {
      if (to_partial) fast(std::integral_constant<int, 0>{}, F{}, F{});
      else if (p.out_bf16) {
        if (res) { if (relu) fast(std::integral_constant<int, 1>{}, T{}, T{}); else fast(std::integral_constant<int, 1>{}, T{}, F{}); }
        else { if (relu) fast(std::integral_constant<int, 1>{}, F{}, T{}); else fast(std::integral_constant<int, 1>{}, F{}, F{}); }
      } else {
        if (res) { if (relu) fast(std::integral_constant<int, 2>{}, T{}, T{}); else fast(std::integral_constant<int, 2>{}, T{}, F{}); }
        else { if (relu) fast(std::integral_constant<int, 2>{}, F{}, T{}); else fast(std::integral_constant<int, 2>{}, F{}, F{}); }
      }
    } else {
      auto wk = pm.walk(pwave * 64 + (lane >> 3));
#pragma unroll 1
      for (int r8 = 0; r8 < 8; ++r8) {
        const int pix = r8 * 8 + (lane >> 3);
        bool pok;
        const uint32_t gp = wk.get(pok);
        wk.step8();
        if (pok && nv > 0) {
          const uint32_t idx = gp * (uint32_t)p.N + cbase;
          const float* row = (const float*)(ep + pix * EP_ROW + cg * 32);
#pragma unroll 1
          for (int j = 0; j < nv; ++j) {
            float y = row[j];
            if (to_partial) { p.partial[(size_t)split * p.M * p.N + idx + j] = y; continue; }
            if (res) y += p.out_bf16 ? (float)((const __bf16*)p.ep_res)[idx + j] : ((const float*)p.ep_res)[idx + j];
            if (relu) y = fmaxf(y, 0.f);
            if (relu6) y = fminf(y, 6.f);
            if (p.out_bf16) ((__bf16*)p.out)[idx + j] = (__bf16)y;
            else ((float*)p.out)[idx + j] = y;
          }
        }
      }
    }
  }
}

template <int KIND, int NW, bool RES_PRE = false>
__device__ __forceinline__ void staged_epilogue(const ContractParams& p, const RngLive& rl, const f32x16 (&accm)[2][2],
                                                const f32x16 (&accd)[2][2], unsigned char* smem, int tid, int wave,
                                                int lane, int ntile, int group, int split, uint32_t m0, int nvalid,
                                                int pwave = -1, bool first = true, float* ba_ext = nullptr) {
  const PixContig pm = {m0, nvalid};
  staged_epilogue_pm<KIND, NW, PixContig, RES_PRE>(p, rl, accm, accd, smem, tid, wave, lane, ntile, group, split, pm, pwave, first,
                                                   ba_ext);
}

}
```

### bayesian_torch_amd/csrc/btx_mma.h

```cpp
#pragma once
#include "btx_contract.h"

namespace btx {

typedef __attribute__((ext_vector_type(2))) float f32x2;
typedef __attribute__((ext_vector_type(2))) __bf16 bf16x2;

__device__ __forceinline__ void split_bf16_pair(uint32_t x0, uint32_t x1, uint32_t& hi, uint32_t& lo) {
#pragma clang fp contract(off)
  const f32x2 v = {u2f(x0), u2f(x1)};
  hi = __builtin_bit_cast(uint32_t, __builtin_convertvector(v, bf16x2));
  const f32x2 r = {v[0] - u2f(hi << 16), v[1] - u2f(hi & 0xffff0000u)};
  lo = __builtin_bit_cast(uint32_t, __builtin_convertvector(r, bf16x2));
}
__device__ __forceinline__ void split_bf16_granules(const u32x4& g0, const u32x4& g1, u32x4& hi, u32x4& lo) {
  uint32_t h_, l_;
  split_bf16_pair(g0[0], g0[1], h_, l_); hi[0] = h_; lo[0] = l_;
  split_bf16_pair(g0[2], g0[3], h_, l_); hi[1] = h_; lo[1] = l_;
  split_bf16_pair(g1[0], g1[1], h_, l_); hi[2] = h_; lo[2] = l_;
  split_bf16_pair(g1[2], g1[3], h_, l_); hi[3] = h_; lo[3] = l_;
}
__device__ __forceinline__ f32x16 mfma3(const u32x4& wh, const u32x4& wl, const u32x4& ah, const u32x4& al, f32x16 c) {
  c = __builtin_amdgcn_mfma_f32_32x32x16_bf16(__builtin_bit_cast(bf16x8, wl), __builtin_bit_cast(bf16x8, ah), c, 0, 0, 0);
  c = __builtin_amdgcn_mfma_f32_32x32x16_bf16(__builtin_bit_cast(bf16x8, wh), __builtin_bit_cast(bf16x8, al), c, 0, 0, 0);
  return __builtin_amdgcn_mfma_f32_32x32x16_bf16(__builtin_bit_cast(bf16x8, wh), __builtin_bit_cast(bf16x8, ah), c, 0, 0, 0);
}

template <int MI>
struct StageFragT {
  u32x4 a[NG / 2][MI], wm[NG / 2][2];
  uint32_t sw[MI];
};
using StageFrag = StageFragT<2>;

struct DeltaFrag {
  u32x4 w[NG / 2][2];
};
template <int KIND>
__device__ __forceinline__ void load_delta(DeltaFrag& d, const unsigned char* ws, int l31, int h) {
  if constexpr (KIND == 1) {
#pragma unroll
    for (int kk = 0; kk < NG / 2; ++kk)
#pragma unroll
      for (int ni = 0; ni < 2; ++ni)
        d.w[kk][ni] = *(const u32x4*)(ws + NG * BN * 16 + ((2 * kk + h) * BN + ni * 32 + l31) * 16);
  }
}

template <int PREC, int KIND, int MI = 2, int MIA = MI, bool ZERO = false, bool MASK = true>
__device__ __forceinline__ void stage_mma(StageFragT<MI>& f, const DeltaFrag& dfrag, f32x16 (&accm)[MI][2],
                                          f32x16 (&accd)[MI][2], int l31, int h) {
    const u32x4 (&wd)[NG / 2][2] = dfrag.w;
    if constexpr (PREC == 2) {
      static_assert(NG == 4, "split-bf16: one 32x32x16 K-step per 16-k stage");
      u32x4 ah[MI], al[MI];
#pragma unroll
      for (int mi = 0; mi < MIA; ++mi) split_bf16_granules(f.a[0][mi], f.a[1][mi], ah[mi], al[mi]);
#pragma unroll
      for (int ni = 0; ni < 2; ++ni) {
        const u32x4 wh = {f.wm[0][ni][0], f.wm[0][ni][1], f.wm[1][ni][0], f.wm[1][ni][1]};
        const u32x4 wl = {f.wm[0][ni][2], f.wm[0][ni][3], f.wm[1][ni][2], f.wm[1][ni][3]};
#pragma unroll
        for (int mi = 0; mi < MIA; ++mi) accm[mi][ni] = mfma3(wh, wl, ah[mi], al[mi], accm[mi][ni]);
      }
      if constexpr (KIND == 1) {
#pragma unroll
        for (int mi = 0; mi < MIA; ++mi) {
#pragma unroll
          for (int r = 0; r < 4; ++r) {
            const uint32_t m = (f.sw[mi] << (2 * ((r >> 1) * 2 + h) + (r & 1))) & 0x80008000u;
            ah[mi][r] ^= m;
            al[mi][r] ^= m;
          }
        }
#pragma unroll
        for (int ni = 0; ni < 2; ++ni) {
          const u32x4 dh = {wd[0][ni][0], wd[0][ni][1], wd[1][ni][0], wd[1][ni][1]};
          const u32x4 dl = {wd[0][ni][2], wd[0][ni][3], wd[1][ni][2], wd[1][ni][3]};
#pragma unroll
          for (int mi = 0; mi < MIA; ++mi) accd[mi][ni] = mfma3(dh, dl, ah[mi], al[mi], accd[mi][ni]);
        }
      }
      return;
    }
#pragma unroll
// ... 68 lines not shown
```

### bayesian_torch_amd/csrc/btx_plan.cpp

```cpp
#include <string.h>
#include "btx_plan.h"

namespace btx {

static inline long long plan_lanes(uint32_t flags) {
  const long long n = (flags >> BTX_FLAG_LANES_SHIFT) & 0xffu;
  return n > 1 ? n : 1;
}

static inline bool throughput_plan(uint32_t flags) { return (flags & BTX_FLAG_CONCURRENT) || plan_lanes(flags) > 1; }

static int split_k(long long base1, int units, int unit_cost, int max_split, bool full_splits, bool throughput, bool short_exit) {
  int ks = 1;
  long long best = -1;
  for (int c = 1; c <= max_split; ++c) {
    if (full_splits && units % c) continue;
    const int per = (units + c - 1) / c;
    const long long rounds = (base1 * c + SLOTS - 1) / SLOTS;
    const long long cost = rounds * (per * unit_cost + 4) + (c > 1 ? 1 : 0);
    if (best < 0 || cost < best) { best = cost; ks = c; }
    if (throughput && (base1 * c >= 64 || (short_exit && base1 * c >= 16 && per <= 16))) { ks = c; break; }
  }
  return ks;
}
// ... 72 lines not shown
    if (Rp * Wp > ppcap) return false;
    G = tp / (Ho * Wo);
    if (G > ppcap / (Rp * Wp)) G = ppcap / (Rp * Wp);
    if (G > g->NB) G = g->NB;
    if (G < 1) return false;
  } else {
    int rmax = tp / Wo;
    const int rfit = ppcap / Wp - halo_r;
    if (rfit < rmax) rmax = rfit;
    if (rmax > Ho) rmax = Ho;
    if (rmax < 1) return false;
    const int nrt = (Ho + rmax - 1) / rmax;
    R = (Ho + nrt - 1) / nrt;
    auto mfma_tiles = [&](int r) {
      long long n = 0;
      for (int row = 0; row < Ho; row += r) n += ((long long)((Ho - row < r) ? Ho - row : r) * Wo + 31) / 32;
      return n;
    };
    if (rmax > R && (Ho % rmax == 0 || 2 * (Ho % rmax) >= rmax) && mfma_tiles(rmax) < mfma_tiles(R)) R = rmax;
  }
  pt->G = G; pt->R = R; pt->Rp = R + halo_r; pt->Wp = Wp; pt->PP = G * pt->Rp * Wp;
  pt->rtiles = (Ho + R - 1) / R;
  return pt->PP <= ppcap && G * R * Wo <= tp;
}


static bool patch_base_ok(const BtxGeom* g, int act_dtype, int prec, uint32_t flags, Plan* pl, PatchPlan* pt) {
  if (flags & (BTX_FLAG_TRANSPOSED | BTX_FLAG_ROWFUSE)) return false;
  pt->wide = 0;
  if (make_plan(g, prec, flags, DBM, pl)) return false;
  if (!dma_shape_ok(g, act_dtype, prec, *pl)) return false;
  return g->D == 1 && g->KD == 1 && pl->Do == 1;
}
static bool patch_lds(PatchPlan* pt, int slots, int wd, int max_ni) {
  const int pieces = (pt->PP + 15) / 16;
  pt->NI = (pieces + pt->nw - 1) / pt->nw;
  if (pt->NI > max_ni) return false;
  pt->astage = pieces * 1024;
  int lds = slots * pt->astage + slots * (pt->astage / 16) + wd * 8192 + 1024;
  const int ep = pt->nw * PT_EP_WAVE + 1024;
  if (lds < ep) lds = ep;
  if (lds > (pt->nw == 4 ? 81920 : 163840)) return false;
  pt->lds = lds;
  pt->lds_g = (lds + 15) & ~15;
  return true;
}
static void wide_tile(const BtxGeom* g, int kind, int act_dtype, int prec, uint32_t flags, const Plan& pl, PatchPlan* pt) {
  if (kind == BTX_KIND_REPARAM && prec == BTX_PREC_BF16 && act_dtype == BTX_ACT_BF16 && (pl.Ng % 128) == 0 &&
      (long long)pl.mtiles * (pl.ntiles / 2) * g->groups * plan_lanes(flags) >= SLOTS) {
    pt->wide = 1;
    if (pt->lds < pt->nw * PT_EP_WAVE + 2048) {
      pt->lds = pt->nw * PT_EP_WAVE + 2048;
      pt->lds_g = (pt->lds + 15) & ~15;
    }
  }
}
static long long patch_base1(const BtxGeom* g, const Plan& pl, const PatchPlan& pt) {
  return (long long)pl.mtiles * (pt.wide ? pl.ntiles / 2 : pl.ntiles) * g->groups;
}
static bool patch_split_k(const BtxGeom* g, int prec, uint32_t flags, int T, Plan* pl, const PatchPlan& pt) {
  const int bk = NG * (prec == BTX_PREC_BF16 ? 8 : 4);
  const int units = pl->Cg / bk / pt.kg;
  const long long base1 = patch_base1(g, *pl, pt);
  const long long base1n = throughput_plan(flags) ? (long long)pl->mtiles * pl->ntiles * g->groups : base1;
  int max_ks = 1;
  while (max_ks < units && max_ks < 32 && (units + max_ks) / (max_ks + 1) * T >= 4) ++max_ks;
  const int ks = split_k(base1n, units, T, max_ks, pt.kg == 2, throughput_plan(flags), false);
  const int per = (units + ks - 1) / ks;
  pl->kper = per * pt.kg * bk;
  pl->ksplits = (units + per - 1) / per;
  const long long nwg = base1 * pl->ksplits;
  if (nwg > 0x7fffffffLL) return false;
  pl->nwg = (int)nwg;
  return true;
}

static bool make_patch_plan(const BtxGeom* g, int act_dtype, int prec, uint32_t flags, Plan* pl, PatchPlan* pt, int kind = -1) {
  if (!patch_base_ok(g, act_dtype, prec, flags, pl, pt) || g->sh != 1 || g->sw != 1) return false;
  const int T = g->KH * g->KW;
  if (T < 2 || T > 64) return false;
  pt->tall = 0; pt->P = 1; pt->Wt = 1; pt->ncs = 1;
  if (patch_tile(g, *pl, 256, 352, pt)) pt->nw = 4;
  else if (patch_tile(g, *pl, 512, 960, pt)) pt->nw = 8;
  else return false;
  if (pt->nw == 4 && g->KH == 3 && g->KW == 3) {
    const long long mt_old = (long long)((g->NB + pt->G - 1) / pt->G) * pt->rtiles;
    const double eff_old = (double)pl->M / ((double)mt_old * 256.0);
    PatchPlan tp = *pt;
    const double eff_tall = tall_tile(g, *pl, 256, 352, &tp);
    if (eff_tall > eff_old * TALL_MIN_GAIN) *pt = tp;
  }
  if (!patch_lds(pt, 2, PT_WD, PT_MAXNI)) return false;
  pl->mtiles = pt->tall ? pt->rtiles * pt->ncs : ((g->NB + pt->G - 1) / pt->G) * pt->rtiles;
  pt->taps = (pt->nw == 4 && pt->NI <= 6 && g->KH == 3 && g->KW == 3) ? 33 : 0;
  if (pt->taps == 33) wide_tile(g, kind, act_dtype, prec, flags, *pl, pt);
  const int ncb = pl->Cg / (NG * (prec == BTX_PREC_BF16 ? 8 : 4));
  pt->kg = (pt->taps && !throughput_plan(flags) && patch_base1(g, *pl, *pt) * plan_lanes(flags) <= 256 && ncb >= 2 && (ncb % 2) == 0 &&
            2 * pt->lds_g <= 163840) ? 2 : 1;
  if (!patch_split_k(g, prec, flags, T, pl, *pt)) return false;
  if (pt->kg == 2) pt->lds = 2 * pt->lds_g;
  return true;
}

static bool make_patch2_plan(const BtxGeom* g, int act_dtype, int prec, uint32_t flags, Plan* pl, PatchPlan* pt, int kind = -1) {
  if (!patch_base_ok(g, act_dtype, prec, flags, pl, pt)) return false;
  if (g->KH != 3 || g->KW != 3 || g->sh != 2 || g->sw != 2 || g->ph != 1 || g->pw != 1 || g->dh != 1 || g->dw != 1) return false;
  BtxGeom gp = *g;
  gp.KH = 2; gp.KW = 2;
  if (!patch_tile(&gp, *pl, 256, 272, pt)) return false;
  pt->nw = 4;
  pt->tall = 0; pt->P = 1; pt->Wt = 1; pt->ncs = 1;
  if (!patch_lds(pt, 3, 3, 5)) return false;
  pl->mtiles = ((g->NB + pt->G - 1) / pt->G) * pt->rtiles;
  wide_tile(g, kind, act_dtype, prec, flags, *pl, pt);
  pt->taps = 332;
  pt->kg = 1;
  return patch_split_k(g, prec, flags, 9, pl, *pt);
}

static bool make_stem_plan(const BtxGeom* g, int act_dtype, int prec, const Plan& pl, StemPlan* st) {
  if (g->D != 1 || g->KD != 1 || pl.Do != 1 || g->groups != 1) return false;
  const int esz = (act_dtype == BTX_ACT_BF16) ? 2 : 4;
  const int bk = NG * (prec == BTX_PREC_BF16 ? 8 : 4);
  if ((g->KW * g->C) % bk || pl.K % bk) return false;
  const long long rowB = (long long)g->W * g->C * esz;
  for (int nw = 4; nw <= 8; nw += 4) {
    const int tp = 64 * nw;
    if (pl.Wo > tp) continue;
    int R = tp / pl.Wo;
    if (R > pl.Ho) R = pl.Ho;
    const long long cap = (nw == 4 ? 81920 : 163840) - PT_WD * 8192;
    for (; R >= 1; --R) {
      const long long Rp = (long long)(R - 1) * g->sh + g->KH;
      const long long pb = Rp * rowB;
      const long long astage = (pb + 1023) / 1024 * 1024;
      const long long sbytes = ((pb / esz + 31) / 32 + 3) * 4;
      const long long sb16 = (sbytes + 15) / 16 * 16;
      if (astage + sb16 > cap) continue;
      long long lds = astage + sb16 + PT_WD * 8192;
      const long long ep = (long long)nw * PT_EP_WAVE + 1024;
      if (lds < ep) lds = ep;
      st->R = R; st->Rp = (int)Rp; st->rtiles = (pl.Ho + R - 1) / R; st->nw = nw; st->astage = (int)astage;
      st->sbytes = (int)sb16; st->lds = (int)lds; st->patch_bytes = (int)pb;
      const long long nwg = (long long)g->NB * st->rtiles * pl.ntiles;
      if (nwg > 0x7fffffffLL) return false;
      st->nwg = (int)nwg;
      return true;
    }
  }
  return false;
// ... 10 lines not shown
  const int Hq = (pl.Ho - 1) / 2 + 1, Wq = (pl.Wo - 1) / 2 + 1;
  const long long rowB = (long long)g->W * g->C * 2;
  const long long Rp = (long long)g->sh + g->KH;
  const long long pb = Rp * rowB;
  const long long astage = (pb + 1023) / 1024 * 1024;
  const long long sbytes = ((pb / 2 + 31) / 32 + 3) * 4;
  const long long sb16 = (sbytes + 127) / 128 * 128;
  const long long lds = (long long)nstages * 8192 + 3 * astage + 2 * sb16 + 3LL * pl.Wo * 128 + 1024 + 64;
  if (lds > 163840) return false;
  const long long units = (long long)g->NB * pl.ntiles;
  long long PB = ((long long)Hq * units * (lanes > 1 ? lanes : 1)) / 256;
  if (PB < 4) PB = 4;
  if (PB > Hq) PB = Hq;
  const int bands = (Hq + (int)PB - 1) / (int)PB;
  const long long nwg = units * bands;
  if (nwg > 0x7fffffffLL) return false;
  sp->PB = (int)PB; sp->bands = bands; sp->Rp = (int)Rp; sp->astage = (int)astage; sp->sbytes = (int)sb16;
  sp->lds = (int)lds; sp->patch_bytes = (int)pb; sp->nwg = (int)nwg; sp->Hq = Hq; sp->Wq = Wq;
  return true;
}

size_t patch_wt_bytes(const Plan& pl, const BtxGeom* g, int kind, int prec, size_t* one, int lanes) {
  const size_t arr = (size_t)g->groups * pl.ntiles * 64 * (size_t)pl.K * (prec == BTX_PREC_BF16 ? 2 : 4);
  if (one) *one = arr;
  return arr * (size_t)(kind == BTX_KIND_FLIPOUT ? 1 + lanes : lanes);
}
static size_t pad256(size_t v) { return (v + 255) & ~(size_t)255; }

size_t plan_ws(const Plan& pl, const BtxGeom* g, int lanes) {
  return pl.ksplits > 1 ? (size_t)lanes * (size_t)pl.ksplits * (size_t)pl.M * (size_t)g->N * sizeof(float) : 0;
}

int select_fwd(int kind, const BtxGeom* g, int act_dtype, int prec, uint32_t flags, bool unaligned, const BtxNoise* noise,
               const BtxEpilogue* ep, FwdSel* s) {
  if (kind != BTX_KIND_REPARAM && kind != BTX_KIND_FLIPOUT) return BTX_E_UNSUPPORTED;
  if (act_dtype != BTX_ACT_F32 && act_dtype != BTX_ACT_BF16) return BTX_E_DTYPE;
  memset(s, 0, sizeof(*s));
  const int lanes = (int)plan_lanes(flags);
  Plan& pl = s->pl;
  int rc = make_plan(g, prec, flags, BM, &pl);
  if (rc) return rc;

  const int G = (prec == BTX_PREC_BF16) ? 8 : 4;
  const bool explicit_kloop = (flags & BTX_FLAG_GATHER) != 0;
  const bool gen = (pl.Cg % G != 0) || unaligned || explicit_kloop;
  const bool rowfuse = (flags & BTX_FLAG_ROWFUSE) != 0;
  bool dma = !gen && dma_shape_ok(g, act_dtype, prec, pl);
  {
    const bool pointwise_geom = !(flags & BTX_FLAG_TRANSPOSED) && g->KD == 1 && g->KH == 1 && g->KW == 1 && g->sd == 1 && g->sh == 1 &&
                                g->sw == 1 && g->pd == 0 && g->ph == 0 && g->pw == 0;
    if (dma && !rowfuse && pointwise_geom && lanes == 1 && !(flags & BTX_FLAG_CONCURRENT) && pl.M <= 256 && prec != BTX_PREC_BF16X3 &&
        !(noise && (noise->sampled_w || noise->eps_w || noise->sign_in || noise->sign_out)) &&
        !(flags & (BTX_FLAG_OUT_F32 | BTX_FLAG_OUT_BF16)))
      dma = false;
  }
  if (rowfuse) {
    const int esz = (act_dtype == BTX_ACT_BF16) ? 2 : 4;
    const int bk = NG * G;
    const bool ok = !unaligned && !explicit_kloop && !(noise && noise->sign_in) && (prec == BTX_PREC_BF16) == (act_dtype == BTX_ACT_BF16) &&
                    g->groups == 1 && g->dw == 1 && g->pw == 0 && !(flags & BTX_FLAG_TRANSPOSED) &&
                    ((g->KW * g->C) % bk == 0) && ((g->sw * g->C * esz) % 16 == 0) && ((g->W * g->C * esz) % 16 == 0) &&
                    (g->C % G == 0 || G % g->C == 0);
    if (!ok) return BTX_E_UNSUPPORTED;
    dma = true;
  }
  if (dma) {
    rc = make_plan(g, prec, flags, 256, &pl);
// ... 63 lines not shown
      }
    }
  }
  size_t need = plan_ws(pl, g, lanes);
  size_t wt_off = 0, wt_one = 0, wt_all = 0;
  const void* sampled_w = (noise && noise->sampled_w) ? noise->sampled_w : nullptr;
  if (sampled_w && (((uintptr_t)sampled_w) & 15)) return BTX_E_ALIGN;
  if (dma) {
    wt_off = pad256(need);
    wt_all = patch_wt_bytes(pl, g, kind, prec, &wt_one, lanes);
    if (sampled_w && wt_all < 0xfff00000ULL) wt_off = need;
    if (wt_off + wt_all >= 0xfff00000ULL) {
      if (rowfuse || (flags & (BTX_FLAG_OUT_F32 | BTX_FLAG_OUT_BF16)) || lanes > 1) return BTX_E_UNSUPPORTED;
      dma = false;
      rc = make_plan(g, prec, flags, BM, &pl);
      if (rc) return rc;
      need = plan_ws(pl, g, lanes);
    } else if (!sampled_w) {
      need = wt_off + wt_all;
    }
  }
  if ((long long)pl.nwg * lanes > 0x7fffffffLL) return BTX_E_UNSUPPORTED;
  if (!dma) s->family = gen ? BTX_FAMILY_GATHER : BTX_FAMILY_REGSTAGE;
  else if (want_pool) s->family = BTX_FAMILY_STEM_POOL;
  else if (stem) s->family = BTX_FAMILY_STEM;
  else if (patch) s->family = pt.taps == 33 ? BTX_FAMILY_TAPS : pt.taps == 332 ? BTX_FAMILY_TAPS2 : BTX_FAMILY_PATCH;
  else s->family = gemm8 ? BTX_FAMILY_GEMM8 : BTX_FAMILY_DMA;
  s->par_major = (par_major && s->family == BTX_FAMILY_DMA) ? 1 : 0;
  s->par_mqp = par_mqp; s->g8_pairs = g8_pairs; s->out_bf16 = out_bf16;
  s->stp = stp; s->spp = spp;
  if (dma && patch) s->pt = pt;
  else s->pt.kg = 1;
  s->need = need; s->wt_off = wt_off; s->wt_one = wt_one; s->wt_all = wt_all;
  return 0;
}

}

using namespace btx;

extern "C" {

int btx_out_shape(const BtxGeom* g, uint32_t flags, int32_t* Do, int32_t* Ho, int32_t* Wo) {
  if (!g || !Do || !Ho || !Wo) return BTX_E_NULL;
  if (g->NB <= 0 || g->D <= 0 || g->H <= 0 || g->W <= 0 || g->C <= 0 || g->N <= 0 || g->KD <= 0 || g->KH <= 0 ||
      g->KW <= 0 || g->sd <= 0 || g->sh <= 0 || g->sw <= 0 || g->dd <= 0 || g->dh <= 0 || g->dw <= 0 ||
      g->pd < 0 || g->ph < 0 || g->pw < 0 || g->groups <= 0)
    return BTX_E_SHAPE;
  if (g->C % g->groups || g->N % g->groups) return BTX_E_SHAPE;
  if (flags & BTX_FLAG_TRANSPOSED) {
    *Do = (g->D - 1) * g->sd - 2 * g->pd + g->dd * (g->KD - 1) + g->od + 1;
    *Ho = (g->H - 1) * g->sh - 2 * g->ph + g->dh * (g->KH - 1) + g->oh + 1;
    *Wo = (g->W - 1) * g->sw - 2 * g->pw + g->dw * (g->KW - 1) + g->ow + 1;
  } else {
    *Do = (g->D + 2 * g->pd - g->dd * (g->KD - 1) - 1) / g->sd + 1;
    *Ho = (g->H + 2 * g->ph - g->dh * (g->KH - 1) - 1) / g->sh + 1;
    *Wo = (g->W + 2 * g->pw - g->dw * (g->KW - 1) - 1) / g->sw + 1;
  }
  if (*Do <= 0 || *Ho <= 0 || *Wo <= 0) return BTX_E_SHAPE;
  return 0;
}

int btx_contract_pool_shape(const BtxGeom* g, int act_dtype, int prec, uint32_t flags, int32_t* Hq, int32_t* Wq) {
  if (!g || !(flags & BTX_FLAG_ROWFUSE) || (flags & (BTX_FLAG_TRANSPOSED | BTX_FLAG_OUT_F32 | BTX_FLAG_SWAP_SIGNS | BTX_FLAG_GATHER)))
    return 0;
  Plan sp;
// ... 1 lines not shown
  StemPoolPlan spp;
  if (make_plan(g, prec, flags, DBM, &sp) || !make_stem_plan(g, act_dtype, prec, sp, &stp) ||
      !make_stem_pool_plan(g, act_dtype, prec, sp, &spp))
    return 0;
  if (Hq) *Hq = spp.Hq;
  if (Wq) *Wq = spp.Wq;
  return 1;
}

size_t btx_contract_workspace_bytes(const BtxGeom* g, int kind, int act_dtype, int prec, uint32_t flags) {
  Plan a, b;
  if (!g || make_plan(g, prec, flags, BM, &a) || make_plan(g, prec, flags, DBM, &b)) return 0;
  (void)kind;
  const int lanes = (int)plan_lanes(flags);
  auto with_tiles = [&](const Plan& pl) {
    return pad256(plan_ws(pl, g, lanes)) + patch_wt_bytes(pl, g, BTX_KIND_FLIPOUT, prec, nullptr, lanes);
  };
  auto raise = [](size_t& w, size_t v) { if (v > w) w = v; };
  size_t wa = plan_ws(a, g, lanes);
  raise(wa, with_tiles(b));
  Plan b4;
  if (!make_plan(g, prec, flags, 256, &b4)) raise(wa, with_tiles(b4));
  Plan c;
  PatchPlan pt;
  if (make_patch_plan(g, act_dtype, prec, flags, &c, &pt) || make_patch2_plan(g, act_dtype, prec, flags, &c, &pt)) {
    raise(wa, with_tiles(c));
    if ((make_patch_plan(g, act_dtype, prec, flags, &c, &pt, BTX_KIND_REPARAM) ||
         make_patch2_plan(g, act_dtype, prec, flags, &c, &pt, BTX_KIND_REPARAM)) && pt.wide)
      raise(wa, with_tiles(c));
  }
  return wa;
}

int btx_contract_plan_info(int kind, const BtxGeom* g, int act_dtype, int prec, uint32_t flags, const BtxEpilogue* ep,
                           BtxPlanInfo* out) {
  if (!g || !out) return BTX_E_NULL;
  memset(out, 0, sizeof(*out));
  FwdSel s;
  const int rc = select_fwd(kind, g, act_dtype, prec, flags, false, nullptr, ep, &s);
  if (rc) return rc;
  out->family = s.family;
  out->ksplits = s.pl.ksplits;
  out->kper = s.pl.kper;
  out->kgroups = s.pt.kg;
  out->wide = s.pt.wide;
  out->tall = s.pt.tall;
  out->par_major = s.par_major;
  out->pool_band = s.spp.PB;
  out->nwg = s.pl.nwg;
  out->lanes = (int32_t)plan_lanes(flags);
  out->ws_bytes = (uint64_t)s.need;
  return 0;
}

size_t btx_sampled_w_bytes(const BtxGeom* g, int kind, int prec) { return btx_sampled_w_bytes_lanes(g, kind, prec, 1); }

size_t btx_sampled_w_bytes_lanes(const BtxGeom* g, int kind, int prec, int lanes) {
  Plan pl;
  if (!g || lanes < 1 || lanes > 255 || make_plan(g, prec, 0, DBM, &pl)) return 0;
  size_t one = 0;
  const size_t tiles = patch_wt_bytes(pl, g, kind, prec, &one, lanes);
  return tiles + (kind == BTX_KIND_FLIPOUT ? one * (prec == BTX_PREC_BF16 ? 2 : 1) : 0);
}

}
```

### bayesian_torch_amd/csrc/btx_plan.h

```cpp
#pragma once
#include <stddef.h>
#include <stdint.h>
#include "../../include/btx.h"

namespace btx {

constexpr int BM = 256;
constexpr int BN = 64;
constexpr int NG = 4;
constexpr int DBM = 512;

constexpr int PT_WD = 4;
constexpr int PT_EP_ROW = 272;
constexpr int PT_EP_WAVE = 64 * PT_EP_ROW;
constexpr int PT_MAXNI = 8;

constexpr long long SLOTS = 256;
constexpr double TALL_MIN_GAIN = 1.15;
constexpr int GEMM8_MIN_K = 128;
constexpr double WG_MAJOR_MIB = 3.0;

struct Plan {
  int Do, Ho, Wo, Cg, Ng, M, K, mtiles, ntiles, ksplits, kper, nwg;
};

struct PatchPlan {
  int G, R, Rp, Wp, PP, NI, rtiles, nw, astage, lds;
  int taps, kg, lds_g;
  int wide;
  int tall, P, Wt, ncs;
};

struct StemPlan {
  int R, Rp, rtiles, nw, astage, sbytes, lds, patch_bytes, nwg;
};

struct StemPoolPlan {
  int PB, bands, Rp, astage, sbytes, lds, patch_bytes, nwg, Hq, Wq;
};

struct FwdSel {
  int family;
  Plan pl;
  int par_major;
  int par_mqp, g8_pairs, out_bf16;
  StemPlan stp;
  StemPoolPlan spp;
  PatchPlan pt;
  size_t need, wt_off, wt_one, wt_all;
};
static inline bool uses_tiles(int family) { return family >= BTX_FAMILY_DMA; }

int select_fwd(int kind, const BtxGeom* g, int act_dtype, int prec, uint32_t flags, bool unaligned, const BtxNoise* noise,
               const BtxEpilogue* ep, FwdSel* s);

int make_plan(const BtxGeom* g, int prec, uint32_t flags, int bm, Plan* pl);
size_t plan_ws(const Plan& pl, const BtxGeom* g, int lanes = 1);
size_t patch_wt_bytes(const Plan& pl, const BtxGeom* g, int kind, int prec, size_t* one, int lanes = 1);

}
```

### bayesian_torch_amd/functional.py

```python
import ctypes
import os

import torch
import torch.nn.functional as F

from . import _lib
from . import rng as _rng

_PRECISION = os.environ.get("BTX_PRECISION", "f32")
PRECISIONS = ("f32", "bf16", "bf16x3")


def set_precision(prec):
    global _PRECISION
    if prec not in PRECISIONS:
        raise ValueError("precision must be one of %s" % (PRECISIONS,))
    _PRECISION = prec


def get_precision():
    return _PRECISION


_ALT_ORDER = True
# ... 200 lines not shown
    r = _lib.Rng(int(seed), int(sample_idx) & 0xFFFFFFFF, 0, sample_dev.data_ptr() if sample_dev is not None else None)
    _lib.check(L.btx_sample_weights_lanes(arr, len(items), ctypes.byref(r), prec_c, stream, int(lanes),
                                          _lib.SAMPLE_SKIP_MU if skip_mu else 0))
    return outs


_REFUSED_CACHE = {}


def _lanes_refused(kind, op, nb, spatial, dtype, out_dtype, prec_c, extra_flags, lanes):
    flags = (_lib.FLAG_TRANSPOSED if op.transposed else 0) | extra_flags | (lanes << _lib.FLAG_LANES_SHIFT)
    if out_dtype is not None and out_dtype != dtype:
        flags |= _lib.FLAG_OUT_BF16 if out_dtype == torch.bfloat16 else _lib.FLAG_OUT_F32
    act = _lib.ACT_BF16 if dtype == torch.bfloat16 else _lib.ACT_F32
    key = (id(op), nb, spatial, kind, act, prec_c, flags)
    hit = _REFUSED_CACHE.get(key)
    if hit is None or hit[1] is not op:
        L = _lib.lib()
        g = _lib.Geom()
        g.NB, (g.D, g.H, g.W), g.C, g.N = nb, spatial, op.in_channels, op.out_channels
        g.KD, g.KH, g.KW = op.kernel
        g.sd, g.sh, g.sw = op.stride
        g.pd, g.ph, g.pw = op.padding
        g.dd, g.dh, g.dw = op.dilation
        g.od, g.oh, g.ow = op.output_padding
        g.groups = op.groups
        info = _lib.PlanInfo()
        rc = L.btx_contract_plan_info(kind, ctypes.byref(g), act, prec_c, flags, None, ctypes.byref(info))
        if len(_REFUSED_CACHE) > 4096:
            _REFUSED_CACHE.clear()
        hit = _REFUSED_CACHE[key] = (rc == _lib.E_UNSUPPORTED and
                                     L.btx_contract_plan_info(kind, ctypes.byref(g), act, prec_c, flags & ~_lib.FLAG_LANES_MASK,
                                                              None, ctypes.byref(info)) == 0, op)
    return hit[0]


def act_code(act):
    if isinstance(act, str):
        codes = {"none": 0, "relu": 1, "relu6": 2}
        if act not in codes:
            raise ValueError("epilogue activation must be one of %s, got %r" % (sorted(codes), act))
        return codes[act]
    if act is None or isinstance(act, bool):
        return int(bool(act))
    if act in (0, 1, 2):
        return int(act)
    raise ValueError("epilogue activation code must be 0, 1 or 2, got %r" % (act,))


def apply_act_aten(out, act):
    code = act_code(act)
    if code == 1:
        return torch.relu(out)
    if code == 2:
        return torch.clamp(out, 0.0, 6.0)
    return out


def contract_hip(kind, x, mu_p, rho_p, mu_b, rho_b, op, seed, sample_idx, layer_id, prec=None, noise=None,
                 extra_flags=0, out_dtype=None, epilogue=None, sampled_w=None, sample_dev=None, lanes=1, lane_batch=None,
                 self_sampling_weights=None):
    L = _lib.lib()
    if not x.is_cuda:
        raise _lib.BtxError("contract_hip needs a CUDA (ROCm) tensor")
    if x.dtype == torch.float32:
        act = _lib.ACT_F32
# ... 99 lines not shown
            t = _sign_to_int8_cl(noise["sign_in"].to(x.device), op)
            keep.append(t); nz.sign_in = t.data_ptr()
        if noise.get("sign_out") is not None:
            so = noise["sign_out"].to(x.device)
            if op.nd == 0:
                so = so.reshape(-1, op.out_channels)
            t = _sign_to_int8_cl(so, op)
            keep.append(t); nz.sign_out = t.data_ptr()
    ev0 = None
    if _LAUNCH_LOG is not None:
        ev0 = torch.cuda.Event(enable_timing=True)
        ev0.record(torch.cuda.current_stream(x.device))
    ep = None
    if epilogue is not None:
        ep = _lib.Epilogue()
        for name in ("scale", "shift"):
            t = epilogue.get(name)
            if t is not None:
                if t.dtype != torch.float32 or t.numel() != op.out_channels or not t.is_contiguous():
                    raise ValueError("epilogue %s must be a contiguous float32 [out_channels] tensor" % name)
                keep.append(t)
                setattr(ep, name, t.data_ptr())
        res = epilogue.get("residual")
        if res is not None:
            if op.nd == 0:
                res = res.reshape(-1, op.out_channels)
            rp, _, _, _ = _to_channels_last(res, OpDesc(op.nd, op.out_channels, op.out_channels))
            if rp.dtype != out.dtype or rp.numel() != out.numel():
                raise ValueError("epilogue residual must match the output shape and dtype")
            keep.append(rp)
            ep.residual = rp.data_ptr()
        ep.relu = act_code(epilogue.get("relu"))
        ep.pool = 1 if epilogue.get("pool") else 0
    args = (kind, ctypes.byref(g), xp.data_ptr(), mu_p.data_ptr(), rho_p.data_ptr(),
            mu_b.data_ptr() if mu_b is not None else None, rho_b.data_ptr() if rho_b is not None else None,
            out.data_ptr(), ctypes.byref(r), ctypes.byref(nz) if nz is not None else None,
            act, prec_c, flags | rev, ws.data_ptr() if ws is not None else None,
            ws.numel() if ws is not None else 0, stream, ctypes.byref(ep) if ep is not None else None)
    if lanes > 1:
        ln = _lib.Lanes()
        ln.n = lanes
        ln.x_stride = 0 if x_shared else (xp.numel() // lanes) * xp.element_size()
        ln.out_stride = (out.numel() // lanes) * out.element_size()
        ln.res_stride = ln.out_stride
        rc = L.btx_contract_fwd_lanes(*args, ctypes.byref(ln))
    else:
        rc = L.btx_contract_fwd_ex(*args)
    if rc == _lib.E_UNSUPPORTED and ep is not None and ep.relu == 2:
        ep.relu = 1
        rc = L.btx_contract_fwd_lanes(*args, ctypes.byref(ln)) if lanes > 1 else L.btx_contract_fwd_ex(*args)
        _lib.check(rc)
        out.clamp_(max=6.0)
    _lib.check(rc)
    if ev0 is not None:
        ev1 = torch.cuda.Event(enable_timing=True)
        ev1.record(torch.cuda.current_stream(x.device))
        m_rows = nb_out * out_sp[0] * out_sp[1] * out_sp[2]
        k_red = op.kernel[0] * op.kernel[1] * op.kernel[2] * (op.in_channels // op.groups)
        flops = 2.0 * m_rows * op.out_channels * k_red * (2 if kind == _lib.KIND_FLIPOUT else 1)
        tag = "%s/%s/%s k%dx%dx%d cin%d cout%d M%d" % ("flipout" if kind else "reparam", prec,
                                                     "bf16" if act == _lib.ACT_BF16 else "f32", op.kernel[0],
                                                     op.kernel[1], op.kernel[2], op.in_channels, op.out_channels, m_rows)
        _LAUNCH_LOG.append((tag, flops, ev0, ev1))
    if op.nd == 0 and x_shared:
        res = out.reshape((lanes * x.shape[0],) + tuple(x.shape[1:-1]) + (op.out_channels,))
    else:
        res = restore(out, out_sp)
    return res.contiguous() if (_OUT_LAYOUT == "contiguous" and op.nd > 0) else res


WGRAD_ATOMICS = False


def wgrad_hip(kind, x, dy, op, seed, sample_idx, layer_id, w_shape, signs=None, swap=False, bias=False, rowfuse=None,
              _flags=0, raw=False, sample_dev=None, rho_flat=None):
    L = _lib.lib()
    if op.transposed:
        raise _lib.BtxError("wgrad_hip wants the plain-convolution geometry (exchange x and dy for transposed layers)")
    if rowfuse is not None:
        plan, fop = rowfuse, rowfuse["op"]
        xin = rowfuse_input(x, plan, dy.dtype)
# ... 483 lines not shown
```

### bayesian_torch_amd/layers/base_variational_layer.py

```python
import collections
import warnings
from itertools import repeat

import torch
import torch.nn as nn
from torch.nn import Parameter

from .. import _lib
from .. import functional as BF
from .. import rng as _rng

_BACKEND = "auto"


def set_backend(name):
    global _BACKEND
    if name not in ("auto", "hip", "torch"):
        raise ValueError("backend must be auto|hip|torch")
    _BACKEND = name


def get_kernel_size(x, n):
    if isinstance(x, collections.abc.Iterable):
        return tuple(x)
# ... 264 lines not shown
        else:
            tag, op, src = ("plain",), op0, ()
        if src and op0.transposed:
            return None
        if op0.nd == 0 and (self.precision or prec) != "bf16x3" and self._lanes()[0] == 1 and not BF._CONCURRENT:
            rows = 1
            for v in shape[:-1]:
                rows *= int(v)
            if rows <= 256:
                return None
        bk = 32 if (self.precision or prec) == "bf16" else 16
        cg = op.in_channels // op.groups
        if plan is None and cg % bk != 0:
            return None
        kind = _lib.KIND_FLIPOUT if self._family == "flipout" else _lib.KIND_REPARAM
        key = (_rng.seed(), self._sample_key(sample_idx), self._btx_layer_id, self.precision or prec, tag)
        return key, (kind, op, mu_p, rho_p, self._btx_layer_id) + tuple(src)

    def _lanes(self):
        return self.__dict__.get("_btx_lanes", 1), self.__dict__.get("_btx_lane_batch")

    def _sample_key(self, sample_idx):
        sdev = getattr(self, "_btx_sample_dev", None)
        n = self.__dict__.get("_btx_lanes", 1)
        return ("dev", sdev.data_ptr(), n) if sdev is not None else (int(sample_idx), n)

    def _take_presampled(self, sample_idx, prec, tag):
        pre = self.__dict__.get("_btx_pre")
        self.__dict__["_btx_pre"] = None
        if pre is not None and pre[0] == (_rng.seed(), self._sample_key(sample_idx), self._btx_layer_id, prec, tag):
            return pre[1]
        return None

    def _forward_hip(self, x, noise=None, sample_idx=None, epilogue=None, gather=False):
        if self._op.nd > 0 and x.dim() == self._op.nd + 1:
            if epilogue is not None and epilogue.get("residual") is not None:
                epilogue = dict(epilogue, residual=epilogue["residual"].unsqueeze(0))
            return self._forward_hip(x.unsqueeze(0), noise, sample_idx, epilogue, gather).squeeze(0)
        mu, rho = self._w()
        mu_p, rho_p = BF.gemm_major_view(mu, self._op), BF.gemm_major_view(rho, self._op)
        lanes, lane_batch = self._lanes()
        if lanes > 1 and noise is not None:
            raise _lib.BtxError("explicit noise is single-sample: clear the sample lanes first (rng.set_sample_lanes)")
        if sample_idx is None:
            sample_idx = self._btx_sample
            self.__dict__["_btx_sample"] = sample_idx + lanes
        kind = _lib.KIND_FLIPOUT if self._family == "flipout" else _lib.KIND_REPARAM
        mb = self.mu_bias.detach() if self.mu_bias is not None else None
        rb = self.rho_bias.detach() if self.rho_bias is not None else None
        op = self._op
        self.__dict__["_btx_last_xshape"] = tuple(x.shape)
        plan = self._rowfuse_plan(x) if noise is None else None
        if plan is not None:
            prec = self.precision or BF.get_precision()
            pre = self._take_presampled(sample_idx, prec, ("rowfuse", plan["cp"], plan["kwp"]))
            mu_f, rho_f = BF.rowfuse_weights(mu_p, rho_p, plan) if pre is None else (mu_p, rho_p)
            xin = self._rowfuse_packed(x, plan, torch.bfloat16 if prec == "bf16" else torch.float32)
            fo = plan["op"].out_spatial((1, plan["Hp"], plan["Wp"]))
            if epilogue is not None and epilogue.get("residual") is not None and fo[2] != plan["Wo"]:
                raise _lib.BtxError("residual epilogue is not available for this row-fused stem geometry")
            out = BF.contract_hip(kind, xin, mu_f, rho_f, mb, rb, plan["op"], _rng.seed(), sample_idx,
                                  self._btx_layer_id, prec=prec, extra_flags=_lib.FLAG_ROWFUSE, out_dtype=x.dtype,
                                  epilogue=epilogue, sampled_w=pre, sample_dev=getattr(self, "_btx_sample_dev", None),
                                  lanes=lanes, lane_batch=lane_batch,
                                  self_sampling_weights=(lambda: BF.rowfuse_weights(mu_p, rho_p, plan)) if pre is not None else None)
            if epilogue is not None and epilogue.get("pool"):
                return out
            return out[:, :, :plan["Ho"], :plan["Wo"]]
        if epilogue is not None and epilogue.get("pool"):
            raise _lib.BtxError("the fused max-pool needs the row-fused stem path (pool_fusable)")
        if self._btx_cpad is not None and noise is None:
            extra = self._btx_cpad - op.in_channels
            x = BF.pad_channels(x, op, extra)
            mu_p = torch.nn.functional.pad(mu_p, (0, extra))
            rho_p = torch.nn.functional.pad(rho_p, (0, extra))
            op = self._op_pad
        pre = None
        if noise is None:
            tag = ("cpad", self._btx_cpad) if self._btx_cpad is not None else ("plain",)
            pre = self._take_presampled(sample_idx, self.precision or BF.get_precision(), tag)
        return BF.contract_hip(kind, x, mu_p, rho_p, mb, rb, op, _rng.seed(), sample_idx,
                               self._btx_layer_id, prec=self.precision, noise=noise, epilogue=epilogue, sampled_w=pre,
                               sample_dev=getattr(self, "_btx_sample_dev", None),
                               extra_flags=_lib.FLAG_GATHER if gather else 0, lanes=lanes, lane_batch=lane_batch)

    def _rowfuse_packed(self, x, plan, dtype):
        store = self.__dict__.get("_btx_static_x")
        if store is None or store is False:
            return BF.rowfuse_input(x, plan, dtype)
        key = (x.data_ptr(), tuple(x.shape), x.dtype, dtype)
        st = store.get(id(self))
        if st is None or st[0] != key:
            if torch.cuda.is_current_stream_capturing():
                raise _lib.BtxError("static_input: the stem input must be packed before the capture starts")
            st = (key, BF.rowfuse_input(x, plan, dtype))
            store[id(self)] = st
        return st[1]

    def _static_repack(self, x, store):
        st = store.get(id(self))
        if st is None or st[0][0] != x.data_ptr():
            return
        plan = self._rowfuse_plan(x)
        st[1].copy_(BF.rowfuse_input(x, plan, st[1].dtype))

    def pool_fusable(self, x):
        if not self._use_hip(x) or x.dtype != torch.bfloat16 or (self.precision or BF.get_precision()) != "bf16":
            return False
        plan = self._rowfuse_plan(x)
        if plan is None:
            return False
        fo = plan["op"].out_spatial((1, plan["Hp"], plan["Wp"]))
        if (fo[1], fo[2]) != (plan["Ho"], plan["Wo"]):
            return False
        return BF.contract_pool_ok(plan["op"], x.shape[0], (1, plan["Hp"], plan["Wp"]), torch.bfloat16, "bf16",
                                   _lib.FLAG_ROWFUSE)

    def forward_fused(self, x, scale=None, shift=None, residual=None, relu=False, pool=False, act=None):
        relu = BF.act_code(act if act is not None else relu)
        if self._use_hip(x) and not self._needs_grad(x):
            return self._forward_hip(x, epilogue=dict(scale=scale, shift=shift, residual=residual, relu=relu, pool=pool))
        if pool:
            raise _lib.BtxError("forward_fused(pool=True) is an inference-only GPU path (pool_fusable)")
        out = self.forward(x, return_kl=False) if self._use_hip(x) else self._forward_aten(x, False)
        shape = (1, -1) + (1,) * self._op.nd if self._op.nd else (1, -1)
        if scale is not None:
            out = out * scale.view(shape).to(out.dtype)
        if shift is not None:
            out = out + shift.view(shape).to(out.dtype)
        if residual is not None:
            out = out + residual
        return BF.apply_act_aten(out, relu)

    def _rowfuse_plan(self, x):
        if self._op.nd != 2 or self._op.in_channels > 4 or not x.is_cuda:
            return None
        cache = self.__dict__.setdefault("_btx_plans", {})
        key = tuple(x.shape)
        if key not in cache:
            if len(cache) > 64:
                cache.clear()
            cache[key] = BF.rowfuse_plan(self._op, key)
        return cache[key]

    def materialize_noise(self, sample_idx, x_shape=None, out_shape=None, x_dtype=None, signs=True, sample_dev=None):
        mu, _ = self._w()
        op, seed, lid = self._op, _rng.seed(), self._btx_layer_id
        cin, cpad = op.in_channels, self._btx_cpad
        if sample_dev is not None and signs and self._family == "flipout" and x_shape is not None:
            raise _lib.BtxError("sign tensors of padded layouts need a host-side sample index: this layer cannot run in a captured step")
        _fill_eps = BF.fill_eps_hip
        if sample_dev is not None:
            _fill_eps = lambda n, dev, sd, si, li, st: BF.fill_eps_hip(n, dev, sd, si, li, st, sample_dev=sample_dev)
        plan = None
# ... 295 lines not shown
```

### bayesian_torch_amd/models/fuse.py

```python
import types

import torch
import torch.nn as nn


STEM_POOL_FUSION = True


def fold_bn(bn):
    with torch.no_grad():
        w = bn.weight.float() if bn.weight is not None else torch.ones_like(bn.running_var, dtype=torch.float32)
        b = bn.bias.float() if bn.bias is not None else torch.zeros_like(bn.running_var, dtype=torch.float32)
        scale = w / torch.sqrt(bn.running_var.float() + bn.eps)
        shift = b - bn.running_mean.float() * scale
    return scale.contiguous(), shift.contiguous()


def _is_var(m):
    return hasattr(m, "forward_fused")


def _is_q8(m):
    return getattr(m, "_btx_q8", False)


def _is_lstm(m):
    return hasattr(m, "fused_sequence") and hasattr(m, "ih") and hasattr(m, "hh")


def _out(o):
    return o[0] if isinstance(o, tuple) else o


def _textbook_block(m, x):
    y = torch.relu(m.bn1(_out(m.conv1(x))))
    y = m.bn2(_out(m.conv2(y)))
    if hasattr(m, "conv3") and hasattr(m, "bn3"):
        y = m.bn3(_out(m.conv3(torch.relu(y))))
    idt = x if m.downsample is None else m.downsample(x)
# ... 66 lines not shown
            import warnings
            warnings.warn("bayesian_torch_amd.models.fuse: %s has a ResNet's attributes but not its forward: stem / head left unfused"
                          % type(model).__name__)
    object.__setattr__(model, "_btx_textbook", bool(ok))
    return bool(ok)


class _Folded:

    def __init__(self, conv, bn):
        self.conv, self.bn = conv, bn
        self._key, self._ss = None, None

    def _scale_shift(self):
        bn = self.bn
        ts = [t for t in (bn.weight, bn.bias, bn.running_mean, bn.running_var) if t is not None]
        key = tuple((t.data_ptr(), t._version) for t in ts)
        if key != self._key:
            self._ss, self._key = fold_bn(bn), key
        return self._ss

    def __call__(self, x, residual=None, relu=False, pool=False):
        scale, shift = self._scale_shift()
        return self.conv.forward_fused(x, scale, shift, residual, relu, pool=pool)


def _downsample(self, x):
    f = self.__dict__.get("_fds")
    if f is not None:
        return f(x)
    return x if self.downsample is None else self.downsample(x)


def _basic_forward(self, x):
    idt = _downsample(self, x)
    y = self._f1(x, None, True)
    return self._f2(y, idt, True)


def _bottleneck_forward(self, x):
    idt = _downsample(self, x)
    y = self._f1(x, None, True)
    y = self._f2(y, None, True)
    return self._f3(y, idt, True)


def fuse_resnet(model):
    n = 0
    for m in model.modules():
        names = [k for k in ("conv1", "bn1", "conv2", "bn2") if hasattr(m, k)]
        if (len(names) == 4 and hasattr(m, "downsample") and _is_var(m.conv1) and _is_var(m.conv2)
                and ("_f1" in m.__dict__ or block_is_textbook(m))):
            object.__setattr__(m, "_f1", _Folded(m.conv1, m.bn1))
            object.__setattr__(m, "_f2", _Folded(m.conv2, m.bn2))
            if hasattr(m, "conv3") and _is_var(m.conv3):
                object.__setattr__(m, "_f3", _Folded(m.conv3, m.bn3))
                m.forward = types.MethodType(_bottleneck_forward, m)
            else:
                m.forward = types.MethodType(_basic_forward, m)
            ds = m.downsample
            if isinstance(ds, nn.Sequential) and len(ds) == 2 and _is_var(ds[0]) and isinstance(ds[1], nn.BatchNorm2d):
                object.__setattr__(m, "_fds", _Folded(ds[0], ds[1]))
            n += 1
    if (hasattr(model, "conv1") and hasattr(model, "bn1") and hasattr(model, "maxpool") and _is_var(model.conv1)
            and ("_stem" in model.__dict__ or resnet_is_textbook(model))):
        object.__setattr__(model, "_stem", _Folded(model.conv1, model.bn1))

        def pool(mp, y):
            ints = all(isinstance(v, int) for v in (mp.kernel_size, mp.stride, mp.padding, mp.dilation))
            if (y.is_cuda and isinstance(mp, nn.MaxPool2d) and ints and mp.dilation == 1 and not mp.ceil_mode
# ... 469 lines not shown
```

### include/btx.h

```cpp
#ifndef BTX_H_
#define BTX_H_

#include <stddef.h>
#include <stdint.h>

#ifdef __cplusplus
extern "C" {
#endif

#define BTX_ABI_VERSION 9

#define BTX_E_NULL        (-1)
#define BTX_E_SHAPE       (-2)
#define BTX_E_UNSUPPORTED (-3)
#define BTX_E_WORKSPACE   (-4)
#define BTX_E_DTYPE       (-5)
#define BTX_E_ALIGN       (-6)

#define BTX_KIND_REPARAM 0
#define BTX_KIND_FLIPOUT 1
#define BTX_ACT_F32  0
#define BTX_ACT_BF16 1
#define BTX_PREC_F32  0
#define BTX_PREC_BF16 1
#define BTX_PREC_BF16X3 2
#define BTX_FLAG_TRANSPOSED   1u
#define BTX_FLAG_KL_ACCUM     2u
#define BTX_FLAG_ROWFUSE      4u
#define BTX_FLAG_OUT_F32      8u
#define BTX_FLAG_OUT_BF16    16u
#define BTX_FLAG_SWAP_SIGNS  64u
#define BTX_FLAG_CONCURRENT 128u
#define BTX_FLAG_REVERSE    256u
#define BTX_FLAG_GATHER      32u

#define BTX_FLAG_LANES_SHIFT 16
#define BTX_FLAG_LANES_MASK  (0xffu << BTX_FLAG_LANES_SHIFT)
#define BTX_FLAG_LANES(n)    (((uint32_t)(n) & 0xffu) << BTX_FLAG_LANES_SHIFT)

#define BTX_STREAM_EPS_W    0u
#define BTX_STREAM_EPS_B    1u
#define BTX_STREAM_SIGN_IN  2u
#define BTX_STREAM_SIGN_OUT 3u

typedef struct BtxGeom {
  int32_t NB, D, H, W, C;
  int32_t N;
  int32_t KD, KH, KW;
  int32_t sd, sh, sw;
  int32_t pd, ph, pw;
  int32_t dd, dh, dw;
  int32_t od, oh, ow;
  int32_t groups;
} BtxGeom;

typedef struct BtxRng {
  uint64_t seed;
  uint32_t sample_idx;
  uint32_t layer_id;
  const uint32_t* sample_idx_dev;
} BtxRng;

typedef struct BtxNoise {
  const float*  eps_w;
  const float*  eps_b;
  const int8_t* sign_in;
  const int8_t* sign_out;
// ... 57 lines not shown
                           const void* x, const float* mu_w, const float* rho_w,
                           const float* mu_b, const float* rho_b,
                           void* out,
                           const BtxRng* rng, const BtxNoise* noise ,
                           int act_dtype, int prec, uint32_t flags,
                           void* ws, size_t ws_bytes, void* stream,
                           const BtxEpilogue* epilogue , const BtxLanes* lanes);

#define BTX_FAMILY_GATHER    0
#define BTX_FAMILY_REGSTAGE  1
#define BTX_FAMILY_DMA       2
#define BTX_FAMILY_GEMM8     3
#define BTX_FAMILY_PATCH     4
#define BTX_FAMILY_TAPS      5
#define BTX_FAMILY_TAPS2     6
#define BTX_FAMILY_STEM      7
#define BTX_FAMILY_STEM_POOL 8
typedef struct BtxPlanInfo {
  int32_t  family;
  int32_t  ksplits;
  int32_t  kper;
  int32_t  kgroups;
  int32_t  wide;
  int32_t  tall;
  int32_t  par_major;
  int32_t  pool_band;
  int32_t  nwg;
  int32_t  lanes;
  uint64_t ws_bytes;
} BtxPlanInfo;
int btx_contract_plan_info(int kind, const BtxGeom* g, int act_dtype, int prec, uint32_t flags,
                           const BtxEpilogue* ep , BtxPlanInfo* out);

int btx_contract_wgrad(int kind, const BtxGeom* g, const void* x, const void* dy, float* dw_mu, float* dw_delta,
                       float* db_mu, float* db_delta, const BtxRng* rng, const BtxNoise* noise ,
                       int act_dtype, uint32_t flags, void* stream);
size_t btx_wgrad_workspace_bytes(int kind, const BtxGeom* g, int act_dtype, uint32_t flags);
int btx_contract_wgrad_ws(int kind, const BtxGeom* g, const void* x, const void* dy, float* dw_mu, float* dw_delta,
                          float* db_mu, float* db_delta, const BtxRng* rng, const BtxNoise* noise ,
                          int act_dtype, uint32_t flags, void* ws, size_t ws_bytes, const float* rho_w ,
                          float* drho , void* stream);

typedef struct BtxSampleItem {
  const BtxGeom* geom;
  const float*   mu_w;
  const float*   rho_w;
  void*          out;
  int32_t        kind;
  uint32_t       layer_id;
  int32_t        src_KW, src_C;
} BtxSampleItem;
size_t btx_sampled_w_bytes(const BtxGeom* g, int kind, int prec);
int btx_sample_weights(const BtxSampleItem* items_host, int n_items, const BtxRng* rng ,
                       int prec, void* stream);
#define BTX_SAMPLE_SKIP_MU 1u
size_t btx_sampled_w_bytes_lanes(const BtxGeom* g, int kind, int prec, int lanes);
int btx_sample_weights_lanes(const BtxSampleItem* items_host, int n_items, const BtxRng* rng ,
                             int prec, void* stream, int lanes, uint32_t sflags);

int btx_dgrad_weights(const float* mu_w, const float* rho_w, float* out_mu, float* out_rho, float* out_eps, int N, int T, int C,
                      int flip, const BtxRng* rng, void* stream);

int btx_rho_grad(const float* dw, const float* rho, float* drho, size_t n, const BtxRng* rng, uint32_t rng_stream,
                 void* stream);

int btx_rowfuse_pack(const void* x, int in_dtype, const int64_t* strides_ncHW_host, int NB, int C, int H, int W,
// ... 131 lines not shown
```

Before: 1977.

## Fuse next-layer Flipout input signs into producer conv epilogue for ResNet basic blocks

```diff
diff --git a/bayesian_torch_amd/_lib.py b/bayesian_torch_amd/_lib.py
--- a/bayesian_torch_amd/_lib.py
+++ b/bayesian_torch_amd/_lib.py
@@ -10,6 +10,7 @@
 PREC_CODE = {"f32": 0, "bf16": 1, "bf16x3": 2}
 FLAG_TRANSPOSED, FLAG_KL_ACCUM, FLAG_ROWFUSE, FLAG_OUT_F32, FLAG_OUT_BF16, FLAG_GATHER, FLAG_SWAP_SIGNS, FLAG_CONCURRENT = 1, 2, 4, 8, 16, 32, 64, 128
 FLAG_REVERSE = 256
+FLAG_X_SIGNED = 512
 E_UNSUPPORTED = -3
 STREAM_EPS_W, STREAM_EPS_B, STREAM_SIGN_IN, STREAM_SIGN_OUT = 0, 1, 2, 3
 ABI_VERSION = 9
@@ -42,6 +43,10 @@
                 ("relu", ctypes.c_int32), ("pool", ctypes.c_int32)]
 
 
+class Epilogue2(ctypes.Structure):
+    _fields_ = [("base", Epilogue), ("sign_next_layer", ctypes.c_uint32), ("sign_next", ctypes.c_uint32)]
+
+
 class Lanes(ctypes.Structure):
     _fields_ = [("n", ctypes.c_int32), ("x_stride", ctypes.c_int64), ("out_stride", ctypes.c_int64),
                 ("res_stride", ctypes.c_int64)]
@@ -50,6 +55,10 @@
 class PlanInfo(ctypes.Structure):
     _fields_ = [(n, ctypes.c_int32) for n in ("family", "ksplits", "kper", "kgroups", "wide", "tall", "par_major", "pool_band",
                                               "nwg", "lanes")] + [("ws_bytes", ctypes.c_uint64)]
+
+
+class PlanInfo2(ctypes.Structure):
+    _fields_ = [("info", PlanInfo), ("lds_bytes", ctypes.c_int32), ("reserved", ctypes.c_int32)]
 
 
 FAMILIES = ("gather", "regstage", "dma", "gemm8", "patch", "taps", "taps2", "stem", "stem_pool")
@@ -105,7 +114,7 @@
 
 EXPORTS = ("btx_abi_version", "btx_strerror", "btx_kl_workspace_bytes", "btx_kl_gauss", "btx_kl_model_workspace_bytes",
            "btx_kl_gauss_model", "btx_kl_gauss_model_bwd", "btx_contract_wgrad",
-           "btx_contract_workspace_bytes", "btx_contract_fwd", "btx_contract_fwd_ex", "btx_contract_fwd_lanes", "btx_contract_pool_shape", "btx_contract_plan_info", "btx_out_shape", "btx_fill_eps", "btx_fill_sign", "btx_rho_grad",
+           "btx_contract_workspace_bytes", "btx_contract_fwd", "btx_contract_fwd_ex", "btx_contract_fwd_lanes", "btx_contract_fwd2", "btx_contract_pool_shape", "btx_contract_plan_info", "btx_contract_plan_info2", "btx_out_shape", "btx_fill_eps", "btx_fill_sign", "btx_rho_grad",
            "btx_mc_packed_floats", "btx_mc_accumulate", "btx_mc_accumulate_lanes", "btx_sampled_w_bytes", "btx_sample_weights", "btx_sampled_w_bytes_lanes", "btx_sample_weights_lanes", "btx_rowfuse_pack", "btx_maxpool2d_cl", "btx_avgpool_global_cl",
            "btx_bn_workspace_bytes", "btx_bn_train_fwd", "btx_bn_train_bwd", "btx_dgrad_weights",
            "btx_wgrad_workspace_bytes", "btx_contract_wgrad_ws", "btx_maxpool2d_cl_train", "btx_maxpool2d_cl_bwd",
@@ -164,6 +173,10 @@
     L.btx_contract_fwd_lanes.argtypes = L.btx_contract_fwd_ex.argtypes + [ctypes.POINTER(Lanes)]
     L.btx_contract_plan_info.restype = i32
     L.btx_contract_plan_info.argtypes = [i32, ctypes.POINTER(Geom), i32, i32, u32, ctypes.POINTER(Epilogue), ctypes.POINTER(PlanInfo)]
+    L.btx_contract_fwd2.restype = i32
+    L.btx_contract_fwd2.argtypes = L.btx_contract_fwd.argtypes + [ctypes.POINTER(Epilogue2), ctypes.POINTER(Lanes)]
+    L.btx_contract_plan_info2.restype = i32
+    L.btx_contract_plan_info2.argtypes = [i32, ctypes.POINTER(Geom), i32, i32, u32, ctypes.POINTER(Epilogue2), ctypes.POINTER(PlanInfo2)]
     L.btx_contract_pool_shape.restype = i32
     L.btx_contract_pool_shape.argtypes = [ctypes.POINTER(Geom), i32, i32, u32] + [ctypes.POINTER(ctypes.c_int32)] * 2
     L.btx_out_shape.restype = i32
diff --git a/bayesian_torch_amd/csrc/btx_api.hip b/bayesian_torch_amd/csrc/btx_api.hip
--- a/bayesian_torch_amd/csrc/btx_api.hip
+++ b/bayesian_torch_amd/csrc/btx_api.hip
@@ -12,14 +12,16 @@
 static int contract_fwd_impl(int kind, const BtxGeom* g, const void* x, const float* mu_w, const float* rho_w,
                              const float* mu_b, const float* rho_b, void* out, const BtxRng* rng, const BtxNoise* noise,
                              int act_dtype, int prec, uint32_t flags, void* ws, size_t ws_bytes, void* stream,
-                             const BtxEpilogue* ep, const BtxLanes* ln) {
+                             const BtxEpilogue* ep, const BtxLanes* ln, const BtxEpilogue2* ep2 = nullptr) {
   if (!g || !x || !mu_w || !rho_w || !out || !rng) return BTX_E_NULL;
+  if (ep2 && ep2->sign_next > 1u) return BTX_E_UNSUPPORTED;
+  const int sign_next = ep2 ? (int)ep2->sign_next : 0;
   const int lanes = ln ? ln->n : 1;
   if ((mu_b == nullptr) != (rho_b == nullptr)) return BTX_E_NULL;
   const uintptr_t al = (uintptr_t)x | (uintptr_t)mu_w | (uintptr_t)rho_w | (uintptr_t)out |
                        (uintptr_t)(noise && noise->eps_w ? noise->eps_w : nullptr);
   FwdSel sel;
-  int rc = select_fwd(kind, g, act_dtype, prec, flags, (al & 15) != 0, noise, ep, &sel);
+  int rc = select_fwd(kind, g, act_dtype, prec, flags, (al & 15) != 0, noise, ep, &sel, sign_next);
   if (rc) return rc;
   const Plan& pl = sel.pl;
   const void* sampled_w = (noise && noise->sampled_w) ? noise->sampled_w : nullptr;
@@ -68,6 +70,13 @@
   }
   p.swap_signs = (flags & BTX_FLAG_SWAP_SIGNS) ? 1 : 0;
   p.reverse = (flags & BTX_FLAG_REVERSE) ? 1 : 0;
+  p.x_signed = (flags & BTX_FLAG_X_SIGNED) ? 1 : 0;
+  if (sign_next) {
+    BtxRng nr = *rng;
+    nr.layer_id = ep2->sign_next_layer;
+    p.sign_next = 1; p.sn_layer = ep2->sign_next_layer;
+    sign_keys(&nr, BTX_STREAM_SIGN_IN, &p.sn_ka, &p.sn_kb);
+  }
   sign_keys(rng, p.swap_signs ? BTX_STREAM_SIGN_OUT : BTX_STREAM_SIGN_IN, &p.kin_a, &p.kin_b);
   sign_keys(rng, p.swap_signs ? BTX_STREAM_SIGN_IN : BTX_STREAM_SIGN_OUT, &p.kout_a, &p.kout_b);
   {
@@ -213,6 +222,21 @@
   if (noise && lanes->n > 1 && (noise->eps_w || noise->eps_b || noise->sign_in || noise->sign_out)) return BTX_E_UNSUPPORTED;
   return contract_fwd_impl(kind, g, x, mu_w, rho_w, mu_b, rho_b, out, rng, noise, act_dtype, prec,
                            (flags & ~BTX_FLAG_LANES_MASK) | BTX_FLAG_LANES(lanes->n), ws, ws_bytes, stream, ep, lanes);
+}
+
+int btx_contract_fwd2(int kind, const BtxGeom* g, const void* x, const float* mu_w, const float* rho_w,
+                      const float* mu_b, const float* rho_b, void* out, const BtxRng* rng, const BtxNoise* noise,
+                      int act_dtype, int prec, uint32_t flags, void* ws, size_t ws_bytes, void* stream,
+                      const BtxEpilogue2* ep2, const BtxLanes* lanes) {
+  const BtxEpilogue* ep = ep2 ? &ep2->base : nullptr;
+  if (!lanes)
+    return contract_fwd_impl(kind, g, x, mu_w, rho_w, mu_b, rho_b, out, rng, noise, act_dtype, prec,
+                             flags & ~BTX_FLAG_LANES_MASK, ws, ws_bytes, stream, ep, nullptr, ep2);
+  if (lanes->n < 1 || lanes->n > 255) return BTX_E_SHAPE;
+  if ((lanes->x_stride | lanes->out_stride | lanes->res_stride) & 15) return BTX_E_ALIGN;
+  if (noise && lanes->n > 1 && (noise->eps_w || noise->eps_b || noise->sign_in || noise->sign_out)) return BTX_E_UNSUPPORTED;
+  return contract_fwd_impl(kind, g, x, mu_w, rho_w, mu_b, rho_b, out, rng, noise, act_dtype, prec,
+                           (flags & ~BTX_FLAG_LANES_MASK) | BTX_FLAG_LANES(lanes->n), ws, ws_bytes, stream, ep, lanes, ep2);
 }
 
 int btx_sample_weights(const BtxSampleItem* items, int n_items, const BtxRng* rng, int prec, void* stream) {
diff --git a/bayesian_torch_amd/csrc/btx_contract.h b/bayesian_torch_amd/csrc/btx_contract.h
--- a/bayesian_torch_amd/csrc/btx_contract.h
+++ b/bayesian_torch_amd/csrc/btx_contract.h
@@ -104,6 +104,13 @@
   long long lane_x, lane_out, lane_res, lane_wt, lane_partial;
   int lane_wt_delta;
   int reverse;
+  int x_signed;
+  int sign_next;
+  uint32_t sn_layer, sn_ka, sn_kb;
+};
+
+struct SignNext {
+  uint32_t on, ka, kb;
 };
 
 __device__ __forceinline__ uint32_t sample_word_scalar(const uint32_t* ptr) {
@@ -771,6 +778,7 @@
 int launch_presample_batch_f32(const PresampleBatch& b, hipStream_t st);
 int launch_presample_batch_bf16(const PresampleBatch& b, hipStream_t st);
 int launch_contract_patch_bf16(int kind, const ContractParams& p, int nwg, hipStream_t st);
+int launch_contract_taps_presign_bf16(const ContractParams& p, int nwg, hipStream_t st);
 int launch_contract_patch_x3(int kind, const ContractParams& p, int nwg, hipStream_t st);
 int launch_contract_stem_x3(int kind, const ContractParams& p, int nwg, hipStream_t st);
 int launch_contract_dma_x3(int kind, const ContractParams& p, int nwg, hipStream_t st);
diff --git a/bayesian_torch_amd/csrc/btx_contract_patch.h b/bayesian_torch_amd/csrc/btx_contract_patch.h
--- a/bayesian_torch_amd/csrc/btx_contract_patch.h
+++ b/bayesian_torch_amd/csrc/btx_contract_patch.h
@@ -252,6 +252,12 @@
   } while (0)
   int rc = launch_presample_impl<PREC>(kind, p, st);
   if (rc) return rc;
+  if (p.x_signed || p.sign_next) {
+    if constexpr (PREC == 1) {
+      if (kind == 1 && (p.pt_taps == 33 || p.pt_taps == 332) && p.pt_kg == 1) return launch_contract_taps_presign_bf16(p, nwg, st);
+    }
+    return BTX_E_UNSUPPORTED;
+  }
   if (p.pt_taps == 332) {
 #define BTX_LAUNCH_T2(KIND, ...)                                                                                  \
   do {                                                                                                            \
diff --git a/bayesian_torch_amd/csrc/btx_contract_taps.h b/bayesian_torch_amd/csrc/btx_contract_taps.h
--- a/bayesian_torch_amd/csrc/btx_contract_taps.h
+++ b/bayesian_torch_amd/csrc/btx_contract_taps.h
@@ -40,9 +40,11 @@
   return n;
 }
 
-template <int PREC, int KIND, int KH, int KW, int KG, bool WIDE = false>
+template <int PREC, int KIND, int KH, int KW, int KG, bool WIDE = false, int PS = 0>
 __global__ __launch_bounds__(256 * KG, 2) void contract_taps_kernel(const ContractParams) {
   static_assert(!WIDE || (PREC == 1 && KG == 1 && KIND == 0), "wide tile: bf16 Reparameterization, one K-group");
+  static_assert(PS == 0 || (PREC == 1 && KG == 1 && KIND == 1 && !WIDE), "signed stores: bf16 Flipout, one K-group");
+  constexpr bool XS = (PS & 1) != 0, SN = (PS & 2) != 0;
   constexpr int K2 = (KIND == 1 || WIDE) ? 1 : 0;
   BTX_SECTION_PARAMS(p, logical);
   constexpr int NW = 4, NT = 256, MI = 2, T = KH * KW;
@@ -101,7 +103,7 @@
   const int cb_per = p.kper / BK;
   const int cb0 = split * cb_per + kg * (cb_per / KG);
   const int ncb = (KG == 1) ? min(ncb_total, cb0 + cb_per) - cb0 : cb_per / KG;
-  const int a_stage = p.pt_astage, s_stage = p.pt_astage >> 4;
+  const int a_stage = p.pt_astage, s_stage = XS ? 0 : p.pt_astage >> 4;
   const int PT_A_OFF = 0, PT_S_OFF = 2 * a_stage, PT_W_OFF = 2 * a_stage + 2 * s_stage;
   const int PT_X_OFF = PT_W_OFF + PT_WD * DW_STAGE;
 
@@ -124,7 +126,7 @@
 
   uint32_t sg_off[2];
   bool sg_ok[2];
-  uint32_t* const pix_tab = (uint32_t*)(smem + PT_S_OFF + s_stage);
+  uint32_t* const pix_tab = (uint32_t*)(XS ? smem + PT_W_OFF + 3 * DW_STAGE : smem + PT_S_OFF + s_stage);
 #pragma unroll
   for (int j = 0; j < 2; ++j) {
     const int q = tid + NT * j;
@@ -132,7 +134,7 @@
     bool inside;
     const uint32_t ipix = patch_src(sg_ok[j] ? q : 0, inside);
     sg_off[j] = ipix * (uint32_t)p.C + (uint32_t)(group * p.Cg);
-    if (q * 4 < s_stage) pix_tab[q] = (sg_ok[j] && inside) ? sg_off[j] : 0xffffffffu;
+    if (q * 4 < (p.pt_astage >> 4)) pix_tab[q] = (sg_ok[j] && inside) ? sg_off[j] : 0xffffffffu;
     if (p.sign_in)
       sg_ok[j] = sg_ok[j] && inside;
   }
@@ -181,7 +183,7 @@
   }
 
   auto write_signs = [&](int slot, int cb) __attribute__((always_inline)) {
-    if constexpr (KIND == 1) {
+    if constexpr (KIND == 1 && !XS) {
       unsigned char* ss = smem + PT_S_OFF + slot * s_stage;
 #pragma unroll
       for (int j = 0; j < 2; ++j) {
@@ -245,7 +247,7 @@
 #pragma unroll
       for (int ni = 0; ni < 2; ++ni) f.wm[kk][ni] = *(const u32x4*)(ws + (row * BN + ni * 32 + l31) * 16);
     }
-    if constexpr (KIND == 1) {
+    if constexpr (KIND == 1 && !XS) {
 #pragma unroll
       for (int mi = 0; mi < MIA; ++mi) f.sw[mi] = *(const uint32_t*)(ss + q[mi] * 4);
     }
@@ -295,8 +297,8 @@
           load_delta<K2>(df, smem + PT_W_OFF + wslot * DW_STAGE, l31, h);
           constexpr int t1 = (t + 1) % T, c1 = (t + 1) / T;
           load_frag(nxt, PAR ^ c1, (t1 / KW) * row_step + (t1 % KW) * p.dw, (wslot + 1) & 3, mia_tag);
-          if constexpr (FIRST && t == 0) stage_mma<PREC, K2, MI, MIA, true, KIND == 1>(cur, df, accm, accd, l31, h);
-          else stage_mma<PREC, K2, MI, MIA, false, KIND == 1>(cur, df, accm, accd, l31, h);
+          if constexpr (FIRST && t == 0) stage_mma<PREC, K2, MI, MIA, true, KIND == 1, XS>(cur, df, accm, accd, l31, h);
+          else stage_mma<PREC, K2, MI, MIA, false, KIND == 1, XS>(cur, df, accm, accd, l31, h);
           if (!last) end_stage<WOPS + KP>();
           else end_stage<(c3 == 0) ? WOPS : 0>();
         } else {
@@ -349,6 +351,17 @@
     const int nvalid = nimg * nrow * pe.Wo;
     const uint32_t m0 = (uint32_t)(img0 * pe.Ho + row0) * (uint32_t)pe.Wo;
     const PixTall pmt = {pe, row0, col0};
+    if constexpr (SN) {
+      SignNext sn = {1u, pe.sn_ka, pe.sn_kb};
+      if (pe.sample_ptr || pe.lanes > 1) {
+        const BtxPhilox4 kn = btx_philox4x32_10(0u, rl.sample, pe.sn_layer, 2u, pe.seed_lo, pe.seed_hi);
+        sn.ka = __builtin_amdgcn_readfirstlane(kn.x[0]); sn.kb = __builtin_amdgcn_readfirstlane(kn.x[1]);
+      }
+      if (tall) staged_epilogue_pm<KIND, NW, PixTall, false, EpNoHook, true>(pe, rl, accm, accd, smem, tid, wave, lane, ntile, group, split,
+                                                                           pmt, -1, true, nullptr, EpNoHook{}, nullptr, sn);
+      else staged_epilogue<KIND, NW, false, true>(pe, rl, accm, accd, smem, tid, wave, lane, ntile, group, split, m0, nvalid, -1, true,
+                                                  nullptr, sn);
+    } else
     if constexpr (KG == 1) {
       if constexpr (WIDE) {
         float* const ba0 = (float*)(smem + NW * PT_EP_WAVE);
diff --git a/bayesian_torch_amd/csrc/btx_contract_taps2.h b/bayesian_torch_amd/csrc/btx_contract_taps2.h
--- a/bayesian_torch_amd/csrc/btx_contract_taps2.h
+++ b/bayesian_torch_amd/csrc/btx_contract_taps2.h
@@ -22,9 +22,11 @@
 constexpr int t2_p0(int s) { return (s == 1 || s == 6 || s == 8) ? 3 : 0; }
 constexpr int t2_fseq(int s) { return s < 2 ? 2 : (s == 4 ? 3 : (s < 7 ? 4 : 5)); }
 
-template <int PREC, int KIND, bool WIDE = false>
+template <int PREC, int KIND, bool WIDE = false, int PS = 0>
 __global__ __launch_bounds__(256, 2) void contract_taps2_kernel(const ContractParams) {
   static_assert(!WIDE || (PREC == 1 && KIND == 0), "wide tile: bf16 Reparameterization");
+  static_assert(PS == 0 || (PREC == 1 && KIND == 1 && !WIDE), "signed stores: bf16 Flipout");
+  constexpr bool XS = (PS & 1) != 0, SN = (PS & 2) != 0;
   BTX_SECTION_PARAMS(p, logical);
   constexpr int NW = 4, NT = 256, MI = 2, T = T2_T, MAXNI = T2_MAXNI, WD = T2_WD;
   constexpr int K2 = (KIND == 1 || WIDE) ? 1 : 0;
@@ -59,7 +61,7 @@
   const int cb_per = p.kper / BK;
   const int cb0 = split * cb_per;
   const int ncb = min(ncb_total, cb0 + cb_per) - cb0;
-  const int a_stage = p.pt_astage, s_stage = p.pt_astage >> 4;
+  const int a_stage = p.pt_astage, s_stage = XS ? 0 : p.pt_astage >> 4;
   const int PT_A_OFF = 0, PT_S_OFF = 3 * a_stage, PT_W_OFF = 3 * a_stage + 3 * s_stage;
   const int PT_X_OFF = PT_W_OFF + WD * DW_STAGE;
 
@@ -150,7 +152,7 @@
     }
   }
   auto write_signs = [&](int a, int b, int cb, int sslot_off) __attribute__((always_inline)) {
-    if constexpr (KIND == 1) {
+    if constexpr (KIND == 1 && !XS) {
       unsigned char* ss = smem + PT_S_OFF + sslot_off;
 #pragma unroll
       for (int j = 0; j < 2; ++j) {
@@ -204,7 +206,7 @@
 #pragma unroll
       for (int ni = 0; ni < 2; ++ni) f.wm[kk][ni] = *(const u32x4*)(ws + (row * BN + ni * 32 + l31) * 16);
     }
-    if constexpr (KIND == 1) {
+    if constexpr (KIND == 1 && !XS) {
 #pragma unroll
       for (int mi = 0; mi < MIA; ++mi) f.sw[mi] = *(const uint32_t*)(ss + q[mi] * 4);
     }
@@ -248,7 +250,7 @@
             const int so = slot_of(t2_seq(s));
             load_frag(fa, so * a_stage, so * s_stage, ((TP / 3) == 2 ? Wp : 0) + ((TP % 3) == 2 ? 1 : 0), wslot, mia_tag);
           }
-          stage_mma<PREC, K2, MI, MIA, false, KIND == 1>(fa, df, accm, accd, l31, h);
+          stage_mma<PREC, K2, MI, MIA, false, KIND == 1, XS>(fa, df, accm, accd, l31, h);
           if (!last) end_stage<WOPS + NP>();
           else end_stage<((s + 2 < T) ? WOPS : 0) + ((t2_fseq(s) < 4) ? NP : 0)>();
           wslot = (wslot + 1) % WD;
@@ -279,6 +281,13 @@
       __syncthreads();
       staged_epilogue<0, NW>(pe, rl, accm, accm, smem, tid, wave, lane, 2 * ntile, group, split, m0, nvalid, -1, true, ba0);
       staged_epilogue<0, NW>(pe, rl, accd, accd, smem, tid, wave, lane, 2 * ntile + 1, group, split, m0, nvalid, -1, true, ba1);
+    } else if constexpr (SN) {
+      SignNext sn = {1u, pe.sn_ka, pe.sn_kb};
+      if (pe.sample_ptr || pe.lanes > 1) {
+        const BtxPhilox4 kn = btx_philox4x32_10(0u, rl.sample, pe.sn_layer, 2u, pe.seed_lo, pe.seed_hi);
+        sn.ka = __builtin_amdgcn_readfirstlane(kn.x[0]); sn.kb = __builtin_amdgcn_readfirstlane(kn.x[1]);
+      }
+      staged_epilogue<KIND, NW, false, true>(pe, rl, accm, accd, smem, tid, wave, lane, ntile, group, split, m0, nvalid, -1, true, nullptr, sn);
     } else
     staged_epilogue<KIND, NW>(pe, rl, accm, accd, smem, tid, wave, lane, ntile, group, split, m0, nvalid);
   }
diff --git a/bayesian_torch_amd/csrc/btx_epilogue.h b/bayesian_torch_amd/csrc/btx_epilogue.h
--- a/bayesian_torch_amd/csrc/btx_epilogue.h
+++ b/bayesian_torch_amd/csrc/btx_epilogue.h
@@ -131,13 +131,14 @@
 struct EpNoHook {
   __device__ __forceinline__ void operator()() const {}
 };
-template <int KIND, int NW, class PM = PixContig, bool RES_PRE = false, class HOOK = EpNoHook>
+template <int KIND, int NW, class PM = PixContig, bool RES_PRE = false, class HOOK = EpNoHook, bool SIGNX = false>
 __device__ __forceinline__ void staged_epilogue_pm(const ContractParams& p, const RngLive& rl, const f32x16 (&accm)[2][2],
                                                    const f32x16 (&accd)[2][2], unsigned char* smem, int tid, int wave,
                                                    int lane, int ntile, int group, int split, const PM& pm,
                                                    int pwave = -1, bool first = true,
                                                    float* ba_ext = nullptr, const HOOK& hook = HOOK{},
-                                                   const uint32_t* wsh_ext = nullptr) {
+                                                   const uint32_t* wsh_ext = nullptr, const SignNext sn = SignNext{0u, 0u, 0u}) {
+  static_assert(!SIGNX || !RES_PRE, "signed stores: the tap-unrolled kernels' store side");
   if (pwave < 0) pwave = wave;
   constexpr int EP_ROW = PT_EP_ROW;
   constexpr int EP_WAVE = PT_EP_WAVE;
@@ -331,6 +332,22 @@
             else { r0[i] = *(const u32x4*)((const float*)p.ep_res + li); r1[i] = *(const u32x4*)((const float*)p.ep_res + li + 4); }
           }
         }
+        uint32_t sgw[NP];
+        if constexpr (SIGNX && RELU && OUTK == 1) {
+          static_assert(NP == 4, "one pixel of the round per lane of a quad");
+          if (((p.N & 31) == 0) && (((group * p.Ng) & 31) == 0)) {
+            const int k = lane & 3;
+            const uint32_t mine = k == 0 ? idx[0] : (k == 1 ? idx[1] : (k == 2 ? idx[2] : idx[3]));
+            const int w = (int)btx_sign_word(mine >> 5, sn.ka, sn.kb);
+            sgw[0] = (uint32_t)__builtin_amdgcn_mov_dpp(w, 0x00, 0xf, 0xf, true);
+            sgw[1] = (uint32_t)__builtin_amdgcn_mov_dpp(w, 0x55, 0xf, 0xf, true);
+            sgw[2] = (uint32_t)__builtin_amdgcn_mov_dpp(w, 0xaa, 0xf, 0xf, true);
+            sgw[3] = (uint32_t)__builtin_amdgcn_mov_dpp(w, 0xff, 0xf, 0xf, true);
+          } else {
+#pragma unroll
+            for (int i = 0; i < NP; ++i) sgw[i] = btx_sign_word(idx[i] >> 5, sn.ka, sn.kb);
+          }
+        }
         f32x4 lo[NP], hi[NP];
 #pragma unroll
         for (int i = 0; i < NP; ++i) {
@@ -359,7 +376,13 @@
             const u32x2 p0 = __builtin_bit_cast(u32x2, __builtin_convertvector(x0, bf16x4));
             const u32x2 p1 = __builtin_bit_cast(u32x2, __builtin_convertvector(x1, bf16x4));
             const __amdgpu_buffer_rsrc_t out_rsrc = __builtin_amdgcn_make_buffer_rsrc((void*)p.out, 0, io_bytes, 0x00020000);
-            __builtin_amdgcn_raw_buffer_store_b128((u32x4){p0[0], p0[1], p1[0], p1[1]}, out_rsrc, pk[i] ? idx[i] * 2u : 0xfffffff0u, 0, 0);
+            u32x4 pv = {p0[0], p0[1], p1[0], p1[1]};
+            if constexpr (SIGNX && RELU) {
+              const uint32_t ws = sgw[i] << (((idx[i] >> 3) & 3u) * 4u);
+#pragma unroll
+              for (int d = 0; d < 4; ++d) pv[d] = (pv[d] & 0x7fff7fffu) | ((ws << d) & 0x80008000u);
+            }
+            __builtin_amdgcn_raw_buffer_store_b128(pv, out_rsrc, pk[i] ? idx[i] * 2u : 0xfffffff0u, 0, 0);
           } else
           if (pk[i]) {
             if constexpr (OUTK == 0) {
@@ -415,6 +438,15 @@
             if (res) y += p.out_bf16 ? (float)((const __bf16*)p.ep_res)[idx + j] : ((const float*)p.ep_res)[idx + j];
             if (relu) y = fmaxf(y, 0.f);
             if (relu6) y = fminf(y, 6.f);
+            if constexpr (SIGNX) {
+              if (sn.on && p.out_bf16 && relu) {
+                const uint32_t io = idx + (uint32_t)j;
+                const uint32_t sb = (btx_sign_word(io >> 5, sn.ka, sn.kb) >> btx_sign_bitpos(io & 31u)) & 1u;
+                const uint16_t yb = __builtin_bit_cast(uint16_t, (__bf16)y);
+                ((uint16_t*)p.out)[io] = (uint16_t)((yb & 0x7fffu) | (sb << 15));
+                continue;
+              }
+            }
             if (p.out_bf16) ((__bf16*)p.out)[idx + j] = (__bf16)y;
             else ((float*)p.out)[idx + j] = y;
           }
@@ -424,14 +456,15 @@
   }
 }
 
-template <int KIND, int NW, bool RES_PRE = false>
+template <int KIND, int NW, bool RES_PRE = false, bool SIGNX = false>
 __device__ __forceinline__ void staged_epilogue(const ContractParams& p, const RngLive& rl, const f32x16 (&accm)[2][2],
                                                 const f32x16 (&accd)[2][2], unsigned char* smem, int tid, int wave,
                                                 int lane, int ntile, int group, int split, uint32_t m0, int nvalid,
-                                                int pwave = -1, bool first = true, float* ba_ext = nullptr) {
+                                                int pwave = -1, bool first = true, float* ba_ext = nullptr,
+                                                const SignNext sn = SignNext{0u, 0u, 0u}) {
   const PixContig pm = {m0, nvalid};
-  staged_epilogue_pm<KIND, NW, PixContig, RES_PRE>(p, rl, accm, accd, smem, tid, wave, lane, ntile, group, split, pm, pwave, first,
-                                                   ba_ext);
-}
-
-}
+  staged_epilogue_pm<KIND, NW, PixContig, RES_PRE, EpNoHook, SIGNX>(p, rl, accm, accd, smem, tid, wave, lane, ntile, group, split, pm,
+                                                                    pwave, first, ba_ext, EpNoHook{}, nullptr, sn);
+}
+
+}
diff --git a/bayesian_torch_amd/csrc/btx_mma.h b/bayesian_torch_amd/csrc/btx_mma.h
--- a/bayesian_torch_amd/csrc/btx_mma.h
+++ b/bayesian_torch_amd/csrc/btx_mma.h
@@ -47,10 +47,39 @@
   }
 }
 
-template <int PREC, int KIND, int MI = 2, int MIA = MI, bool ZERO = false, bool MASK = true>
+template <int PREC, int KIND, int MI = 2, int MIA = MI, bool ZERO = false, bool MASK = true, bool XSGN = false>
 __device__ __forceinline__ void stage_mma(StageFragT<MI>& f, const DeltaFrag& dfrag, f32x16 (&accm)[MI][2],
                                           f32x16 (&accd)[MI][2], int l31, int h) {
     const u32x4 (&wd)[NG / 2][2] = dfrag.w;
+    if constexpr (XSGN) {
+      static_assert(PREC == 1 && KIND == 1 && MASK, "signed input: bf16 Flipout");
+#pragma unroll
+      for (int kk = 0; kk < NG / 2; ++kk)
+#pragma unroll
+        for (int mi = 0; mi < MIA; ++mi)
+#pragma unroll
+          for (int ni = 0; ni < 2; ++ni) {
+            const f32x16 zc = {0.f, 0.f, 0.f, 0.f, 0.f, 0.f, 0.f, 0.f, 0.f, 0.f, 0.f, 0.f, 0.f, 0.f, 0.f, 0.f};
+            accd[mi][ni] = __builtin_amdgcn_mfma_f32_32x32x16_bf16(
+                __builtin_bit_cast(bf16x8, wd[kk][ni]), __builtin_bit_cast(bf16x8, f.a[kk][mi]), (ZERO && kk == 0) ? zc : accd[mi][ni], 0, 0, 0);
+          }
+#pragma unroll
+      for (int kk = 0; kk < NG / 2; ++kk) {
+#pragma unroll
+        for (int mi = 0; mi < MIA; ++mi)
+#pragma unroll
+          for (int d = 0; d < 4; ++d) f.a[kk][mi][d] &= 0x7fff7fffu;
+#pragma unroll
+        for (int mi = 0; mi < MIA; ++mi)
+#pragma unroll
+          for (int ni = 0; ni < 2; ++ni) {
+            const f32x16 zc = {0.f, 0.f, 0.f, 0.f, 0.f, 0.f, 0.f, 0.f, 0.f, 0.f, 0.f, 0.f, 0.f, 0.f, 0.f, 0.f};
+            accm[mi][ni] = __builtin_amdgcn_mfma_f32_32x32x16_bf16(
+                __builtin_bit_cast(bf16x8, f.wm[kk][ni]), __builtin_bit_cast(bf16x8, f.a[kk][mi]), (ZERO && kk == 0) ? zc : accm[mi][ni], 0, 0, 0);
+          }
+      }
+      return;
+    }
     if constexpr (PREC == 2) {
       static_assert(NG == 4, "split-bf16: one 32x32x16 K-step per 16-k stage");
       u32x4 ah[MI], al[MI];
diff --git a/bayesian_torch_amd/csrc/btx_patch_presign.hip b/bayesian_torch_amd/csrc/btx_patch_presign.hip
--- /dev/null
+++ b/bayesian_torch_amd/csrc/btx_patch_presign.hip
@@ -0,0 +1,33 @@
+#include "../../include/btx.h"
+#include "btx_contract_taps.h"
+#include "btx_contract_taps2.h"
+namespace btx {
+int launch_contract_taps_presign_bf16(const ContractParams& p, int nwg, hipStream_t st) {
+#define BTX_LAUNCH_PS(KFN)                                                                                        \
+  do {                                                                                                            \
+    auto kfn = KFN;                                                                                               \
+    static bool attr_done = false;                                                                                \
+    if (!attr_done) {                                                                                             \
+      hipError_t e = hipFuncSetAttribute((const void*)kfn, hipFuncAttributeMaxDynamicSharedMemorySize, 163840);   \
+      if (e != hipSuccess) return (int)e;                                                                         \
+      attr_done = true;                                                                                           \
+    }                                                                                                             \
+    hipLaunchKernelGGL(kfn, dim3(nwg), dim3(256), p.pt_lds, st, p);                                               \
+  } while (0)
+  const int ps = (p.x_signed ? 1 : 0) | (p.sign_next ? 2 : 0);
+  if (p.pt_kg != 1 || ps == 0) return BTX_E_UNSUPPORTED;
+  if (p.pt_taps == 33) {
+    if (ps == 1) BTX_LAUNCH_PS((contract_taps_kernel<1, 1, 3, 3, 1, false, 1>));
+    else if (ps == 2) BTX_LAUNCH_PS((contract_taps_kernel<1, 1, 3, 3, 1, false, 2>));
+    else BTX_LAUNCH_PS((contract_taps_kernel<1, 1, 3, 3, 1, false, 3>));
+  } else if (p.pt_taps == 332) {
+    if (ps == 1) BTX_LAUNCH_PS((contract_taps2_kernel<1, 1, false, 1>));
+    else if (ps == 2) BTX_LAUNCH_PS((contract_taps2_kernel<1, 1, false, 2>));
+    else BTX_LAUNCH_PS((contract_taps2_kernel<1, 1, false, 3>));
+  } else {
+    return BTX_E_UNSUPPORTED;
+  }
+#undef BTX_LAUNCH_PS
+  return (int)hipGetLastError();
+}
+}
diff --git a/bayesian_torch_amd/csrc/btx_plan.cpp b/bayesian_torch_amd/csrc/btx_plan.cpp
--- a/bayesian_torch_amd/csrc/btx_plan.cpp
+++ b/bayesian_torch_amd/csrc/btx_plan.cpp
@@ -128,12 +128,12 @@
   if (!dma_shape_ok(g, act_dtype, prec, *pl)) return false;
   return g->D == 1 && g->KD == 1 && pl->Do == 1;
 }
-static bool patch_lds(PatchPlan* pt, int slots, int wd, int max_ni) {
+static bool patch_lds(PatchPlan* pt, int slots, int wd, int max_ni, bool sign_slots = true) {
   const int pieces = (pt->PP + 15) / 16;
   pt->NI = (pieces + pt->nw - 1) / pt->nw;
   if (pt->NI > max_ni) return false;
   pt->astage = pieces * 1024;
-  int lds = slots * pt->astage + slots * (pt->astage / 16) + wd * 8192 + 1024;
+  int lds = slots * pt->astage + (sign_slots ? slots * (pt->astage / 16) : 0) + wd * 8192 + 1024;
   const int ep = pt->nw * PT_EP_WAVE + 1024;
   if (lds < ep) lds = ep;
   if (lds > (pt->nw == 4 ? 81920 : 163840)) return false;
@@ -195,6 +195,8 @@
             2 * pt->lds_g <= 163840) ? 2 : 1;
   if (!patch_split_k(g, prec, flags, T, pl, *pt)) return false;
   if (pt->kg == 2) pt->lds = 2 * pt->lds_g;
+  if ((flags & BTX_FLAG_X_SIGNED) && kind == BTX_KIND_FLIPOUT && pt->taps == 33 && pt->kg == 1 && !patch_lds(pt, 2, PT_WD, PT_MAXNI, false))
+    return false;
   return true;
 }
 
@@ -211,7 +213,9 @@
   wide_tile(g, kind, act_dtype, prec, flags, *pl, pt);
   pt->taps = 332;
   pt->kg = 1;
-  return patch_split_k(g, prec, flags, 9, pl, *pt);
+  if (!patch_split_k(g, prec, flags, 9, pl, *pt)) return false;
+  if ((flags & BTX_FLAG_X_SIGNED) && kind == BTX_KIND_FLIPOUT && !patch_lds(pt, 3, 3, 5, false)) return false;
+  return true;
 }
 
 static bool make_stem_plan(const BtxGeom* g, int act_dtype, int prec, const Plan& pl, StemPlan* st) {
@@ -288,7 +292,7 @@
 }
 
 int select_fwd(int kind, const BtxGeom* g, int act_dtype, int prec, uint32_t flags, bool unaligned, const BtxNoise* noise,
-               const BtxEpilogue* ep, FwdSel* s) {
+               const BtxEpilogue* ep, FwdSel* s, int sign_next) {
   if (kind != BTX_KIND_REPARAM && kind != BTX_KIND_FLIPOUT) return BTX_E_UNSUPPORTED;
   if (act_dtype != BTX_ACT_F32 && act_dtype != BTX_ACT_BF16) return BTX_E_DTYPE;
   memset(s, 0, sizeof(*s));
@@ -418,6 +422,17 @@
   if (dma && patch) s->pt = pt;
   else s->pt.kg = 1;
   s->need = need; s->wt_off = wt_off; s->wt_one = wt_one; s->wt_all = wt_all;
+  if (flags & BTX_FLAG_X_SIGNED) {
+    if (kind != BTX_KIND_FLIPOUT || prec != BTX_PREC_BF16 || act_dtype != BTX_ACT_BF16 || (s->family != BTX_FAMILY_TAPS && s->family != BTX_FAMILY_TAPS2) || pt.kg != 1 ||
+        (flags & BTX_FLAG_SWAP_SIGNS) || (noise && noise->sign_in))
+      return BTX_E_UNSUPPORTED;
+  }
+  if (sign_next) {
+    if (kind != BTX_KIND_FLIPOUT || prec != BTX_PREC_BF16 || !out_bf16 || !ep || (ep->relu != 1 && ep->relu != 2) || ep->pool ||
+        (s->family != BTX_FAMILY_TAPS && s->family != BTX_FAMILY_TAPS2) || pt.kg != 1 || pl.ksplits != 1 || g->groups != 1 ||
+        (flags & BTX_FLAG_SWAP_SIGNS))
+      return BTX_E_UNSUPPORTED;
+  }
   return 0;
 }
 
@@ -485,13 +500,14 @@
   return wa;
 }
 
-int btx_contract_plan_info(int kind, const BtxGeom* g, int act_dtype, int prec, uint32_t flags, const BtxEpilogue* ep,
-                           BtxPlanInfo* out) {
+static int plan_info_impl(int kind, const BtxGeom* g, int act_dtype, int prec, uint32_t flags, const BtxEpilogue* ep, int sign_next,
+                          BtxPlanInfo* out, int32_t* lds) {
   if (!g || !out) return BTX_E_NULL;
   memset(out, 0, sizeof(*out));
   FwdSel s;
-  const int rc = select_fwd(kind, g, act_dtype, prec, flags, false, nullptr, ep, &s);
+  const int rc = select_fwd(kind, g, act_dtype, prec, flags, false, nullptr, ep, &s, sign_next);
   if (rc) return rc;
+  if (lds) *lds = (s.family == BTX_FAMILY_PATCH || s.family == BTX_FAMILY_TAPS || s.family == BTX_FAMILY_TAPS2) ? s.pt.lds : 0;
   out->family = s.family;
   out->ksplits = s.pl.ksplits;
   out->kper = s.pl.kper;
@@ -506,6 +522,20 @@
   return 0;
 }
 
+int btx_contract_plan_info(int kind, const BtxGeom* g, int act_dtype, int prec, uint32_t flags, const BtxEpilogue* ep,
+                           BtxPlanInfo* out) {
+  return plan_info_impl(kind, g, act_dtype, prec, flags, ep, 0, out, nullptr);
+}
+
+int btx_contract_plan_info2(int kind, const BtxGeom* g, int act_dtype, int prec, uint32_t flags, const BtxEpilogue2* ep2,
+                            BtxPlanInfo2* out) {
+  if (!out) return BTX_E_NULL;
+  memset(out, 0, sizeof(*out));
+  if (ep2 && ep2->sign_next > 1u) return BTX_E_UNSUPPORTED;
+  return plan_info_impl(kind, g, act_dtype, prec, flags, ep2 ? &ep2->base : nullptr, ep2 ? (int)ep2->sign_next : 0, &out->info,
+                        &out->lds_bytes);
+}
+
 size_t btx_sampled_w_bytes(const BtxGeom* g, int kind, int prec) { return btx_sampled_w_bytes_lanes(g, kind, prec, 1); }
 
 size_t btx_sampled_w_bytes_lanes(const BtxGeom* g, int kind, int prec, int lanes) {
diff --git a/bayesian_torch_amd/csrc/btx_plan.h b/bayesian_torch_amd/csrc/btx_plan.h
--- a/bayesian_torch_amd/csrc/btx_plan.h
+++ b/bayesian_torch_amd/csrc/btx_plan.h
@@ -52,7 +52,7 @@
 static inline bool uses_tiles(int family) { return family >= BTX_FAMILY_DMA; }
 
 int select_fwd(int kind, const BtxGeom* g, int act_dtype, int prec, uint32_t flags, bool unaligned, const BtxNoise* noise,
-               const BtxEpilogue* ep, FwdSel* s);
+               const BtxEpilogue* ep, FwdSel* s, int sign_next = 0);
 
 int make_plan(const BtxGeom* g, int prec, uint32_t flags, int bm, Plan* pl);
 size_t plan_ws(const Plan& pl, const BtxGeom* g, int lanes = 1);
diff --git a/bayesian_torch_amd/functional.py b/bayesian_torch_amd/functional.py
--- a/bayesian_torch_amd/functional.py
+++ b/bayesian_torch_amd/functional.py
@@ -256,6 +256,42 @@
         hit = _REFUSED_CACHE[key] = (rc == _lib.E_UNSUPPORTED and
                                      L.btx_contract_plan_info(kind, ctypes.byref(g), act, prec_c, flags & ~_lib.FLAG_LANES_MASK,
                                                               None, ctypes.byref(info)) == 0, op)
+    return hit[0]
+
+
+_PRESIGN_CACHE = {}
+
+
+def presign_plan(kind, op, nb, spatial, dtype, prec, lanes=1, x_signed=False, sign_next=None, relu=0, extra_flags=0):
+    prec_c = _lib.PREC_CODE[prec or _PRECISION]
+    flags = (_lib.FLAG_TRANSPOSED if op.transposed else 0) | extra_flags | (_lib.FLAG_CONCURRENT if _CONCURRENT else 0)
+    if x_signed:
+        flags |= _lib.FLAG_X_SIGNED
+    if lanes > 1:
+        flags |= lanes << _lib.FLAG_LANES_SHIFT
+    act = _lib.ACT_BF16 if dtype == torch.bfloat16 else _lib.ACT_F32
+    key = (id(op), nb, tuple(spatial), kind, act, prec_c, flags, sign_next is not None, int(relu))
+    hit = _PRESIGN_CACHE.get(key)
+    if hit is None or hit[1] is not op:
+        L = _lib.lib()
+        g = _lib.Geom()
+        g.NB, (g.D, g.H, g.W), g.C, g.N = nb, spatial, op.in_channels, op.out_channels
+        g.KD, g.KH, g.KW = op.kernel
+        g.sd, g.sh, g.sw = op.stride
+        g.pd, g.ph, g.pw = op.padding
+        g.dd, g.dh, g.dw = op.dilation
+        g.od, g.oh, g.ow = op.output_padding
+        g.groups = op.groups
+        ep2 = _lib.Epilogue2()
+        ep2.base.relu = int(relu)
+        ep2.sign_next = 1 if sign_next is not None else 0
+        info = _lib.PlanInfo2()
+        rc = L.btx_contract_plan_info2(kind, ctypes.byref(g), act, prec_c, flags, ctypes.byref(ep2), ctypes.byref(info))
+        if rc not in (0, _lib.E_UNSUPPORTED):
+            _lib.check(rc)
+        if len(_PRESIGN_CACHE) > 4096:
+            _PRESIGN_CACHE.clear()
+        hit = _PRESIGN_CACHE[key] = (info if rc == 0 else None, op)
     return hit[0]
 
 
@@ -421,6 +457,12 @@
             ep.residual = rp.data_ptr()
         ep.relu = act_code(epilogue.get("relu"))
         ep.pool = 1 if epilogue.get("pool") else 0
+    sign_next = epilogue.get("sign_next") if epilogue is not None else None
+    ep2 = None
+    if sign_next is not None:
+        ep2 = _lib.Epilogue2()
+        ep2.base = ep
+        ep2.sign_next_layer, ep2.sign_next = int(sign_next) & 0xFFFFFFFF, 1
     args = (kind, ctypes.byref(g), xp.data_ptr(), mu_p.data_ptr(), rho_p.data_ptr(),
             mu_b.data_ptr() if mu_b is not None else None, rho_b.data_ptr() if rho_b is not None else None,
             out.data_ptr(), ctypes.byref(r), ctypes.byref(nz) if nz is not None else None,
@@ -432,10 +474,11 @@
         ln.x_stride = 0 if x_shared else (xp.numel() // lanes) * xp.element_size()
         ln.out_stride = (out.numel() // lanes) * out.element_size()
         ln.res_stride = ln.out_stride
-        rc = L.btx_contract_fwd_lanes(*args, ctypes.byref(ln))
+        rc = (L.btx_contract_fwd2(*args[:-1], ctypes.byref(ep2), ctypes.byref(ln)) if ep2 is not None
+              else L.btx_contract_fwd_lanes(*args, ctypes.byref(ln)))
     else:
-        rc = L.btx_contract_fwd_ex(*args)
-    if rc == _lib.E_UNSUPPORTED and ep is not None and ep.relu == 2:
+        rc = L.btx_contract_fwd2(*args[:-1], ctypes.byref(ep2), None) if ep2 is not None else L.btx_contract_fwd_ex(*args)
+    if rc == _lib.E_UNSUPPORTED and ep is not None and ep.relu == 2 and ep2 is None:
         ep.relu = 1
         rc = L.btx_contract_fwd_lanes(*args, ctypes.byref(ln)) if lanes > 1 else L.btx_contract_fwd_ex(*args)
         _lib.check(rc)
diff --git a/bayesian_torch_amd/layers/base_variational_layer.py b/bayesian_torch_amd/layers/base_variational_layer.py
--- a/bayesian_torch_amd/layers/base_variational_layer.py
+++ b/bayesian_torch_amd/layers/base_variational_layer.py
@@ -320,11 +320,11 @@
             return pre[1]
         return None
 
-    def _forward_hip(self, x, noise=None, sample_idx=None, epilogue=None, gather=False):
+    def _forward_hip(self, x, noise=None, sample_idx=None, epilogue=None, gather=False, x_signed=False):
         if self._op.nd > 0 and x.dim() == self._op.nd + 1:
             if epilogue is not None and epilogue.get("residual") is not None:
                 epilogue = dict(epilogue, residual=epilogue["residual"].unsqueeze(0))
-            return self._forward_hip(x.unsqueeze(0), noise, sample_idx, epilogue, gather).squeeze(0)
+            return self._forward_hip(x.unsqueeze(0), noise, sample_idx, epilogue, gather, x_signed).squeeze(0)
         mu, rho = self._w()
         mu_p, rho_p = BF.gemm_major_view(mu, self._op), BF.gemm_major_view(rho, self._op)
         lanes, lane_batch = self._lanes()
@@ -339,6 +339,8 @@
         op = self._op
         self.__dict__["_btx_last_xshape"] = tuple(x.shape)
         plan = self._rowfuse_plan(x) if noise is None else None
+        if x_signed and (plan is not None or noise is not None or self._btx_cpad is not None or gather):
+            raise _lib.BtxError("x_signed: a plain bf16 tap-kernel launch with generated noise only (presign_request)")
         if plan is not None:
             prec = self.precision or BF.get_precision()
             pre = self._take_presampled(sample_idx, prec, ("rowfuse", plan["cp"], plan["kwp"]))
@@ -370,7 +372,8 @@
         return BF.contract_hip(kind, x, mu_p, rho_p, mb, rb, op, _rng.seed(), sample_idx,
                                self._btx_layer_id, prec=self.precision, noise=noise, epilogue=epilogue, sampled_w=pre,
                                sample_dev=getattr(self, "_btx_sample_dev", None),
-                               extra_flags=_lib.FLAG_GATHER if gather else 0, lanes=lanes, lane_batch=lane_batch)
+                               extra_flags=(_lib.FLAG_GATHER if gather else 0) | (_lib.FLAG_X_SIGNED if x_signed else 0),
+                               lanes=lanes, lane_batch=lane_batch)
 
     def _rowfuse_packed(self, x, plan, dtype):
         store = self.__dict__.get("_btx_static_x")
@@ -404,10 +407,28 @@
         return BF.contract_pool_ok(plan["op"], x.shape[0], (1, plan["Hp"], plan["Wp"]), torch.bfloat16, "bf16",
                                    _lib.FLAG_ROWFUSE)
 
-    def forward_fused(self, x, scale=None, shift=None, residual=None, relu=False, pool=False, act=None):
+    def presign_request(self, x_shape, dtype, x_signed=False, sign_next=False, relu=1):
+        op = self._op
+        if (self._family != "flipout" or op.nd != 2 or dtype != torch.bfloat16 or (self.precision or BF.get_precision()) != "bf16"
+                or self._btx_cpad is not None or op.in_channels <= 4 or len(x_shape) != 4):
+            return False
+        lanes, lane_batch = self._lanes()
+        nb = int(lane_batch) if lanes > 1 else int(x_shape[0])
+        if lanes > 1 and int(x_shape[0]) != nb * lanes:
+            return False
+        return BF.presign_plan(_lib.KIND_FLIPOUT, op, nb, (1, int(x_shape[2]), int(x_shape[3])), dtype, "bf16", lanes=lanes,
+                               x_signed=x_signed, sign_next=(0 if sign_next else None), relu=relu) is not None
+
+    def forward_fused(self, x, scale=None, shift=None, residual=None, relu=False, pool=False, act=None, sign_next=None,
+                      x_signed=False):
         relu = BF.act_code(act if act is not None else relu)
         if self._use_hip(x) and not self._needs_grad(x):
-            return self._forward_hip(x, epilogue=dict(scale=scale, shift=shift, residual=residual, relu=relu, pool=pool))
+            ep = dict(scale=scale, shift=shift, residual=residual, relu=relu, pool=pool)
+            if sign_next is not None:
+                ep["sign_next"] = sign_next._btx_layer_id
+            return self._forward_hip(x, epilogue=ep, x_signed=x_signed)
+        if sign_next is not None or x_signed:
+            raise _lib.BtxError("forward_fused(sign_next= / x_signed=) is an inference-only GPU path (presign_request)")
         if pool:
             raise _lib.BtxError("forward_fused(pool=True) is an inference-only GPU path (pool_fusable)")
         out = self.forward(x, return_kl=False) if self._use_hip(x) else self._forward_aten(x, False)
diff --git a/bayesian_torch_amd/models/fuse.py b/bayesian_torch_amd/models/fuse.py
--- a/bayesian_torch_amd/models/fuse.py
+++ b/bayesian_torch_amd/models/fuse.py
@@ -5,6 +5,7 @@
 
 
 STEM_POOL_FUSION = True
+PRESIGN = True
 
 
 def fold_bn(bn):
@@ -137,10 +138,31 @@
     return x if self.downsample is None else self.downsample(x)
 
 
+def _presign_pair(prod, cons, x, mods):
+    if not PRESIGN or torch.is_grad_enabled() or not x.is_cuda or x.dtype != torch.bfloat16 or x.dim() != 4:
+        return False
+    if any(m.training or _hooked(m) for m in mods):
+        return False
+    if not (hasattr(prod, "presign_request") and hasattr(cons, "presign_request")):
+        return False
+    if (prod._btx_sample != cons._btx_sample or prod.__dict__.get("_btx_sample_dev") is not cons.__dict__.get("_btx_sample_dev")
+            or prod._lanes() != cons._lanes() or not prod._use_hip(x)):
+        return False
+    op = prod._op
+    sp = op.out_spatial((1, int(x.shape[2]), int(x.shape[3])))
+    mid = (int(x.shape[0]), op.out_channels, sp[1], sp[2])
+    return (prod.presign_request(tuple(x.shape), x.dtype, sign_next=True, relu=1)
+            and cons.presign_request(mid, x.dtype, x_signed=True))
+
+
 def _basic_forward(self, x):
     idt = _downsample(self, x)
-    y = self._f1(x, None, True)
-    return self._f2(y, idt, True)
+    f1, f2 = self._f1, self._f2
+    if _presign_pair(f1.conv, f2.conv, x, (f1.conv, f1.bn, f2.conv, f2.bn)):
+        y = f1.conv.forward_fused(x, *f1._scale_shift(), None, True, sign_next=f2.conv)
+        return f2.conv.forward_fused(y, *f2._scale_shift(), idt, True, x_signed=True)
+    y = f1(x, None, True)
+    return f2(y, idt, True)
 
 
 def _bottleneck_forward(self, x):
diff --git a/include/btx.h b/include/btx.h
--- a/include/btx.h
+++ b/include/btx.h
@@ -33,6 +33,8 @@
 #define BTX_FLAG_CONCURRENT 128u
 #define BTX_FLAG_REVERSE    256u
 #define BTX_FLAG_GATHER      32u
+
+#define BTX_FLAG_X_SIGNED   512u
 
 #define BTX_FLAG_LANES_SHIFT 16
 #define BTX_FLAG_LANES_MASK  (0xffu << BTX_FLAG_LANES_SHIFT)
@@ -156,6 +158,27 @@
 int btx_contract_plan_info(int kind, const BtxGeom* g, int act_dtype, int prec, uint32_t flags,
                            const BtxEpilogue* ep , BtxPlanInfo* out);
 
+typedef struct BtxEpilogue2 {
+  BtxEpilogue base;
+  uint32_t    sign_next_layer;
+  uint32_t    sign_next;
+} BtxEpilogue2;
+int btx_contract_fwd2(int kind, const BtxGeom* g,
+                      const void* x, const float* mu_w, const float* rho_w,
+                      const float* mu_b, const float* rho_b,
+                      void* out,
+                      const BtxRng* rng, const BtxNoise* noise ,
+                      int act_dtype, int prec, uint32_t flags,
+                      void* ws, size_t ws_bytes, void* stream,
+                      const BtxEpilogue2* ep2 , const BtxLanes* lanes );
+typedef struct BtxPlanInfo2 {
+  BtxPlanInfo info;
+  int32_t     lds_bytes;
+  int32_t     reserved;
+} BtxPlanInfo2;
+int btx_contract_plan_info2(int kind, const BtxGeom* g, int act_dtype, int prec, uint32_t flags,
+                            const BtxEpilogue2* ep2 , BtxPlanInfo2* out);
+
 int btx_contract_wgrad(int kind, const BtxGeom* g, const void* x, const void* dy, float* dw_mu, float* dw_delta,
                        float* db_mu, float* db_delta, const BtxRng* rng, const BtxNoise* noise ,
                        int act_dtype, uint32_t flags, void* stream);
```

After: 1998 (median of 4 runs). Within noise of the previous version (+1.1%).
